# jdhuang-csm/hybrid-drt

Hardware: AMD Instinct MI355X
Metric: DRT fits/sec (256 freq x 512 tau, batched) (higher is better)
Workload: dtype f64

## Files before the change

### hybrid-drt_amd/_ffi.py

```python
from __future__ import annotations

import ctypes as C
import os
import sys
import threading

import numpy as np

_HERE = os.path.dirname(os.path.abspath(__file__))
LIB_PATH = os.environ.get("HIPDRT_LIB", os.path.join(_HERE, "libhipdrt.so"))

MODE_INTERP, MODE_TRAPZ = 0, 1
RESPONSE_POT, RESPONSE_EXPDECAY = 0, 1
QP_OPTIMAL, QP_MAXITER, QP_SINGULAR_LATE, QP_SINGULAR, QP_ABORTED = 0, 1, 2, -1, -2
PREDICT_NOT_PD = -3


class HipDrtError(RuntimeError):
    pass


class QpOpts(C.Structure):
    _fields_ = [("abstol", C.c_double), ("reltol", C.c_double), ("feastol", C.c_double), ("maxiters", C.c_int)]

# ... 148 lines not shown


SIGNATURES = {
    "hipdrt_create": [C.c_int, C.POINTER(_vp)],
    "hipdrt_destroy": [_vp],
    "hipdrt_last_error": [],
    "hipdrt_stream": [_vp],
    "hipdrt_synchronize": [_vp],
    "hipdrt_device_info": [_vp, C.c_char_p, C.c_int, _ip, C.POINTER(C.c_longlong)],
    "hipdrt_impedance_lookup": [_vp, C.c_double, C.c_int, C.c_int, _dp, _dp, _dp, _dp],
    "hipdrt_impedance_matrix": [_vp, C.c_int, C.c_int, _dp, C.c_int, _dp, C.c_int, C.c_int, C.c_int, C.c_double,
                                C.c_int, _dp, _dp, _dp, _dp, C.c_int, _dp, _dp],
    "hipdrt_impedance_matrix_dev": [_vp, C.c_int, C.c_int, _dp, C.c_int, _dp, C.c_int, C.c_int, C.c_int, C.c_double,
                                    C.c_int, _dp, _dp, _dp, _dp, C.c_int, _vp, _vp, C.c_int, C.POINTER(C.c_float)],
    "hipdrt_phasor_z_matrix": [_vp, _dp, C.c_int, _dp, C.c_int, C.c_double, _dp, _dp],
    "hipdrt_phasor_v_matrix": [_vp, _dp, C.c_int, _dp, C.c_int, C.c_double, _dp, _dp, C.c_int, _dp, _dp],
    "hipdrt_chrono_var_matrix": [_vp, _dp, C.c_int, _ip, C.c_int, C.c_double, C.c_int, _dp],
    "hipdrt_response_lookup": [_vp, C.c_double, C.c_int, C.c_int, _dp, _dp],
    "hipdrt_response_matrix": [_vp, _dp, C.c_int, _dp, C.c_int, _dp, _dp, C.c_int, C.c_int, C.c_double, C.c_int, _dp, _dp,
                               C.c_int, _dp, _dp],
    "hipdrt_plan_bytes_per_spectrum": [C.c_int, C.c_int, C.c_int, C.POINTER(C.c_longlong)],
    "hipdrt_response_matrix_variant": [_vp, _dp, C.c_int, _dp, C.c_int, _dp, _dp, _dp, C.c_int, C.c_int, C.c_double, C.c_int,
                                       _dp, _dp],
    "hipdrt_nonuniform_gaussian_filter1d": [_vp, _dp, C.c_int, _dp, _ip, C.c_int, _ip, _dp, C.c_int, _dp, _dp, C.c_longlong,
                                            _ip, _ip, _dp],
    "hipdrt_penalty_matrices": [_vp, _dp, C.c_int, C.c_double, C.c_int, _dp, _dp, _dp],
    "hipdrt_eis_var_matrix": [_vp, _dp, C.c_int, C.c_double, C.c_double, C.c_int, _dp],
    "hipdrt_qp_batch": [_vp, C.c_int, C.c_int, C.c_int, _dp, _dp, C.c_int, _dp, C.POINTER(QpOpts), _dp, _ip, _dp, _ip],
    "hipdrt_qp_profile": [_vp, C.POINTER(C.c_ulonglong), C.c_int, C.c_int],
    "hipdrt_debug_qp_occupancy": [_vp, C.c_int, C.c_int],
    "hipdrt_debug_qp_group": [_vp, C.c_int],
    "hipdrt_debug_exact_zero_shortcuts": [_vp, C.c_int],
    "hipdrt_debug_qp_waves": [_vp, C.c_int],
    "hipdrt_debug_stream_pool": [_vp, C.c_int, C.POINTER(C.c_void_p), _ip, _ip, _ip],
    "hipdrt_debug_gram_l2": [_vp, C.POINTER(DebugGramArgs)],
    "hipdrt_debug_pack_p": [_vp, C.c_int, C.c_int, _dp, C.c_int, _dp],
    "hipdrt_debug_hyper_step": [_vp, C.POINTER(DebugHyperArgs)],
    "hipdrt_debug_hyper_form": [_vp, C.c_int, C.c_int, C.c_int, C.c_int, C.c_int, _ip, C.POINTER(C.c_longlong)],
    "hipdrt_debug_kk_stats": [_vp, C.c_int, C.c_int, _dp, _dp, _dp, C.POINTER(KkOpts), _dp, _ip, _dp, _ip, _ip],
    "hipdrt_default_kk_opts": [C.POINTER(KkOpts)],
    "hipdrt_plan_kk_screen": [_vp, C.POINTER(KkOpts), C.c_int, _dp, _dp, _dp, _dp, _dp, _ip, _dp, _ip, _ip],
    "hipdrt_func_eval_matrix": [_vp, _dp, C.c_int, _dp, C.c_int, C.c_double, C.c_int, _dp],
    "hipdrt_plan_set_tau_basis": [_vp, _dp, C.c_int, C.c_double],
    "hipdrt_plan_predict_drt": [_vp, _dp, C.c_int, C.c_int, C.c_int, C.c_int, C.c_double, C.c_double, _dp, _dp, _dp, _ip],
    "hipdrt_plan_predict_z": [_vp, _dp, C.c_int, C.c_int, _dp, _dp, _ip],
    "hipdrt_plan_predict_resistances": [_vp, _dp, _dp, _dp, C.c_int],
    "hipdrt_plan_set_predict_desc": [_vp, C.POINTER(PredictDesc)],
    "hipdrt_plan_predict_response": [_vp, C.POINTER(ResponseArgs), _dp, _ip],
    "hipdrt_plan_predict_z_model": [_vp, C.POINTER(ZModelArgs), _dp, _dp, _ip],
    "hipdrt_plan_predict_dop": [_vp, _dp, C.c_int, _dp, C.c_double, _dp, C.c_double, C.c_int, _dp, _ip],
    "hipdrt_debug_response": [_vp, C.POINTER(DebugResponseArgs)],
    "hipdrt_peak_opts_default": [C.POINTER(PeakOpts)],
    "hipdrt_plan_find_peaks": [_vp, _dp, C.c_int, C.POINTER(PeakOpts), _dp, _ip, _ip, _dp, _dp, _dp, _ip, _ip, _ip, _dp, _dp, _dp,
                               _ip],
    "hipdrt_debug_find_peaks": [_vp, C.c_int, C.c_int, _dp, _dp, _dp, _dp, C.POINTER(PeakOpts), _ip, _ip, _dp, _dp, _dp, _ip, _ip,
                                _ip, _dp, _dp, _dp],
    "hipdrt_peak_resolve_opts_default": [C.POINTER(PeakResolveOpts)],
    "hipdrt_plan_resolve_peaks": [_vp, C.POINTER(PeakResolveIn), C.POINTER(PeakResolveOpts), C.POINTER(PeakResolveOut)],
    "hipdrt_plan_integrate_drt": [_vp, _dp, C.c_int, C.c_int, C.c_int, C.c_int, _dp, _ip, _ip, C.c_int, _dp, _ip],
    "hipdrt_debug_peak_resolve": [_vp, C.POINTER(DebugPeakResolveArgs)],
    "hipdrt_plan_score_candidates": [_vp, C.POINTER(CandidatesIn), C.POINTER(CandidatesOut)],
    "hipdrt_debug_candidate_llh": [_vp, C.c_int, C.c_int, C.c_int, C.c_int, _dp, C.c_int, _dp, _dp, _dp, _dp, _dp, _dp],
    "hipdrt_debug_candidate_form": [_vp, C.c_int],
    "hipdrt_plan_pfrt_bytes_per_spectrum": [C.c_int, C.c_int, C.POINTER(C.c_longlong)],
    "hipdrt_plan_pfrt_begin": [_vp, C.c_int],
    "hipdrt_plan_pfrt_record": [_vp],
# ... 431 lines not shown
        opts = opts if opts is not None else default_fit_opts()
        B, nf, ntau = z.shape[0], freq.size, tau.size
        n = ntau + int(opts.fit_ohmic) + int(opts.fit_inductance)
        out = {"x": np.empty((B, n)), "fit_x": np.empty((B, ntau)), "R_inf": np.empty(B), "inductance": np.empty(B),
               "weights": np.empty((B, 2 * nf)), "coefficient_scale": np.empty(B), "rho": np.empty((B, 3)),
               "q_vector": np.empty((B, n)), "outer_iters": np.empty(B, dtype=np.int32),
               "status": np.empty(B, dtype=np.int32)}
        _check(self._lib.hipdrt_fit_eis_batch(self._h, B, _p(freq), nf, _p(z_re), _p(z_im), _p(tau), ntau, float(epsilon),
                                              MODE_INTERP, int(bool(toeplitz_a)), int(bool(toeplitz_m)), wt_re.size,
                                              int(ny), _p(wt_re), _p(wt_im), _p(lre), _p(lim), C.byref(opts),
                                              _p(out["x"]), _p(out["fit_x"]), _p(out["R_inf"]), _p(out["inductance"]),
                                              _p(out["weights"]), _p(out["coefficient_scale"]), _p(out["rho"]),
                                              _p(out["q_vector"]), _pi(out["outer_iters"]), _pi(out["status"])))
        return out

    def device_alloc(self, nbytes):
        ptr = _vp()
        _check(self._lib.hipdrt_device_alloc(self._h, int(nbytes), C.byref(ptr)))
        return ptr.value

    def device_free(self, ptr):
        _check(self._lib.hipdrt_device_free(self._h, _vp(ptr)))

    def device_synchronize(self):
        _check(self._lib.hipdrt_device_synchronize(self._h))

    def debug_qp_group(self, members):
        _check(self._lib.hipdrt_debug_qp_group(self._h, int(members)))
        self._qp_group_override = int(members)

    def debug_qp_waves(self, waves):
        _check(self._lib.hipdrt_debug_qp_waves(self._h, int(waves)))

    def debug_stream_pool(self):
        size = C.c_int(0)
        _check(self._lib.hipdrt_debug_stream_pool(self._h, 0, None, None, None, C.byref(size)))
        n = size.value
        st, ho, ru = (C.c_void_p * n)(), (C.c_int * n)(), (C.c_int * n)()
        _check(self._lib.hipdrt_debug_stream_pool(self._h, n, st, ho, ru, C.byref(size)))
        return [st[i] for i in range(n)], [ho[i] for i in range(n)], [ru[i] for i in range(n)]

    def debug_exact_zero_shortcuts(self, on):
        _check(self._lib.hipdrt_debug_exact_zero_shortcuts(self._h, int(bool(on))))

    def debug_gram_l2(self, A, w, y=None, l1=None, l1_scalar=0.0, l2=None, mk=None, s=None, rho=None, dfac=(0.0, 0.0, 0.0),
                      ns=0, sym=False, toep=False, toep_maxd=-1, spec_zero=False, dop_start=0, dop_size=0, dop_rho=None,
                      dop_dfac=(0.0, 0.0, 0.0), active=None, n=None, P=None, Ppk=None, q=None):
        A, w = _f64(A), _f64(w)
        B, m = w.shape
        a = DebugGramArgs()
        a.B, a.m, a.lda = B, m, A.shape[-1]
        a.n = n = A.shape[-1] if n is None else int(n)
        a.a_batched = int(A.ndim == 3)
        if A.shape[-2] != m or (A.ndim == 3 and A.shape[0] != B):
            raise ValueError("A does not match w")
        keep = [A, w]

        def arr(v, shape, what):
            if v is None:
                return None
            v = _f64(v)
            if v.shape != tuple(shape):
                raise ValueError(f"{what}: shape {v.shape}, expected {tuple(shape)}")
            keep.append(v)
            return _p(v)

# ... 958 lines not shown
```

### hybrid-drt_amd/csrc/common.hpp

```cpp
#pragma once
#include <hip/hip_runtime.h>

#include <cstdio>
#include <string>
#include <vector>

#include "../../include/hipdrt.h"
#include "../../include/hipdrt_debug.h"

namespace hipdrt {

void set_error(const std::string& msg);

#define HIPDRT_CHECK(expr)                                                                     \
    do {                                                                                       \
        hipError_t _e = (expr);                                                                \
        if (_e != hipSuccess) {                                                                \
            hipdrt::set_error(std::string(#expr) + ": " + hipGetErrorString(_e) + " (" +       \
                              __FILE__ + ":" + std::to_string(__LINE__) + ")");                \
            return HIPDRT_E_HIP;                                                               \
        }                                                                                      \
    } while (0)

#define HIPDRT_REQUIRE(cond, msg)                                                              \
// ... 30 lines not shown
        if (!src.p) return;
        p = static_cast<char*>(src.p) + offset;
        bytes = n;
        own = false;
    }
    template <class T>
    T* as() const { return static_cast<T*>(p); }
    double* d() const { return static_cast<double*>(p); }
    int* i() const { return static_cast<int*>(p); }
};

inline int round_up(int v, int m) { return (v + m - 1) / m * m; }

inline int set_lds_limit(const void* f, size_t bytes, const char* what) {
    const hipError_t e = hipFuncSetAttribute(f, hipFuncAttributeMaxDynamicSharedMemorySize, (int)bytes);
    if (e != hipSuccess) { set_error(std::string("hipFuncSetAttribute(") + what + "): " + hipGetErrorString(e)); return HIPDRT_E_HIP; }
    return HIPDRT_OK;
}

}

struct hipdrt_ctx {
    int device = 0;
    hipStream_t stream = nullptr;
    int pool_idx = -1;
    int num_cu = 0;
    size_t hbm_bytes = 0;
    std::string arch;
    int plans = 0;
    bool released = false;
    int qp_force_group = -1;
    int zero_shortcuts = 1;
    int qp_waves = -1;
    int cand_form = -1;
    float predict_ms[2] = {0.f, 0.f};
};

namespace hipdrt {

void ensure_stream_pool(int device);

void launch_lookup(hipStream_t st, double eps, int ngrid, int ny, const double* wt_re, const double* wt_im,
                   double* z_re, double* z_im);
void launch_lookup_slopes(hipStream_t st, int ngrid, const double* xp, const double* fp, double* slopes);
void launch_impedance_matrix(hipStream_t st, int B, int freq_batched, const double* freq, int nf, const double* tau,
                             int ntau, int mode, int toeplitz, double eps, int ngrid, const double* lut6, int ny,
                             double* a_re, double* a_im, double* cr_scratch);
void launch_phasor_z(hipStream_t st, const double* freq, int nf, const double* nu, int nnu, double eps, double* zre,
                     double* zim);
void launch_phasor_v(hipStream_t st, const double* times, int nt, const double* nu, int nnu, double eps,
                     const double* step_times, const double* step_sizes, int nsteps, double* rm, double* layered);
void launch_chrono_vmm(hipStream_t st, const double* tt, int nt, const int* seg, int nseg, double eps, int uniform,
                       double* vmm);
void launch_response_lookup(hipStream_t st, double eps, int ngrid, int ny, const double* td, double* v);
void launch_response_matrix(hipStream_t st, const double* times, int nt, const double* tau, int ntau,
                            const double* step_times, const double* step_sizes, int nsteps, int mode, double eps,
                            int ngrid, const double* lut3, int ny, double* a, double* layered);
void launch_response_variant(hipStream_t st, const double* times, int nt, const double* tau, int ntau,
                             const double* step_times, const double* step_sizes, const double* tau_rise, int nsteps,
                             int variant, double eps, int ny, double* a, double* layered);
void launch_nonuniform_gauss(hipStream_t st, const double* y, int n, const double* sigma, const int* seg_of, const int* seg,
                             const double* nodes, int K, const double* node_delta, const double* weights, const int* woff,
                             const int* radius, double* out);
void launch_penalty(hipStream_t st, const double* ln_tau, int n, double eps, int toeplitz, double* m0, double* m1,
                    double* m2, int ld, int pad);
void launch_eis_vmm(hipStream_t st, const double* freq, int nf, double vmm_eps, double reim_cor, int uniform,
// ... 282 lines not shown
    int* status;
};
void launch_cand_compact(hipStream_t st, const CandPeakArgs& a);

struct QpArgs {
    int B, n;
    const double* P;
    long long p_stride;
    int ldp;
    const double* Ppk;
    long long ppk_stride;
    int nchp;
    const double* q;
    const double* h;
    long long h_stride;
    double* L;
    int ldl;
    long long l_stride;
    double* x;
    int* iters;
    double* pcost;
    int* status;
    const int* active;
    const int* order = nullptr;
    int* iters_accum;
    double* state;
    int state_ld;
    long long state_stride;
    hipdrt_qp_opts opts;
    int G = 0;
    int* gsync = nullptr;
    int redo_aborted = 0;
    int waves = 0;
};
int launch_qp(hipStream_t st, const QpArgs& a);
int qp_group_size(int B, int n, int force = -1);
size_t qp_gsync_ints();
int launch_dist_var(hipStream_t st, int B, int n, const double* Ppk, long long ppk_stride, const double* Bex, int nex,
                    double* L, long long l_stride, double* out, long long out_stride, int* status);
size_t dist_var_scratch_doubles(int n, int nex);
void launch_rows_outer(hipStream_t st, const double* Y, int nch, int ncol, int nex, int nrow, double scale, double* out, int ld);
void launch_pack_rows(hipStream_t st, int nrow, int ncol, int col_offset, const double* M, int ldm, int ntile_rows,
                      double* tiles, int nchp);
void launch_lpt_order(hipStream_t st, int B, const int* iters, const int* active, int* order);
size_t qp_scratch_ld(int n);
size_t qp_scratch_doubles(int n, int G = 0);
inline int qp_state_ld(int n) { return round_up(n, 32) + 32; }
inline size_t qp_state_doubles(int n) { return (size_t)17 * qp_state_ld(n); }
int qp_profile_read(unsigned long long* out, int n, int reset);
int hyper_profile_read(unsigned long long* out, int n, int reset);
int qp_occupancy(int threads, int n);

}
```

### hybrid-drt_amd/csrc/debug.hip

```cpp
#include <cmath>
#include <cstring>

#include "plan.hpp"

namespace {
struct Guarded {
    static constexpr size_t G = 128;
    static constexpr unsigned char MARK = 0xA5;
    DevBuf buf;
    void* host = nullptr;
    size_t bytes = 0;
    const char* name = "";
    std::vector<unsigned char> stage;
    int up(const char* what, void* h, size_t nbytes, hipStream_t st) {
        name = what; host = h; bytes = nbytes;
        stage.assign(nbytes + 2 * G, MARK);
        if (h) std::memcpy(stage.data() + G, h, nbytes);
        HIPDRT_CHECK(buf.alloc(stage.size()));
        HIPDRT_CHECK(hipMemcpyAsync(buf.p, stage.data(), stage.size(), hipMemcpyHostToDevice, st));
        return 0;
    }
    double* dd() const { return reinterpret_cast<double*>(static_cast<unsigned char*>(buf.p) + G); }
    int fetch(hipStream_t st) { HIPDRT_CHECK(hipMemcpyAsync(stage.data(), buf.p, stage.size(), hipMemcpyDeviceToHost, st)); return 0; }
    int check() {
// ... 9 lines not shown
struct GuardedOuts {
    static constexpr int MAX = 17;
    Guarded g[MAX];
    int n = 0;
    template <class T>
    int want(const char* name, T* host, size_t count, T*& field, hipStream_t st) {
        if (!host) return 0;
        HIPDRT_REQUIRE(n < MAX, "internal: more outputs than GuardedOuts holds");
        TRY(g[n].up(name, host, count * sizeof(T), st));
        field = reinterpret_cast<T*>(g[n++].dd());
        return 0;
    }
    int back(hipStream_t st) {
        for (int i = 0; i < n; ++i) TRY(g[i].fetch(st));
        HIPDRT_CHECK(hipStreamSynchronize(st));
        for (int i = 0; i < n; ++i) TRY(g[i].check());
        return 0;
    }
};
}

extern "C" {

int hipdrt_debug_qp_group(hipdrt_ctx* ctx, int members) try {
    HIPDRT_REQUIRE(ctx, "NULL pointer");
    ctx->qp_force_group = members;
    return HIPDRT_OK;
} HIPDRT_CATCH

int hipdrt_debug_qp_waves(hipdrt_ctx* ctx, int waves) try {
    HIPDRT_REQUIRE(ctx, "NULL pointer");
    HIPDRT_REQUIRE(waves == -1 || waves == 4 || waves == 8, "waves: 4, 8 or -1");
    ctx->qp_waves = waves;
    return HIPDRT_OK;
} HIPDRT_CATCH

int hipdrt_debug_exact_zero_shortcuts(hipdrt_ctx* ctx, int on) try {
    HIPDRT_REQUIRE(ctx, "NULL pointer");
    ctx->zero_shortcuts = on ? 1 : 0;
    return HIPDRT_OK;
} HIPDRT_CATCH

int hipdrt_debug_qp_occupancy(hipdrt_ctx* ctx, int threads, int n) try {
    if (!ctx || hipSetDevice(ctx->device) != hipSuccess) return -1;
    return qp_occupancy(threads, n);
} HIPDRT_CATCH

int hipdrt_qp_profile(hipdrt_ctx* ctx, unsigned long long* cycles, int n, int reset) try {
    HIPDRT_REQUIRE(ctx && cycles, "NULL pointer");
    TRY(enter(ctx));
    HIPDRT_CHECK(hipStreamSynchronize(ctx->stream));
    return qp_profile_read(cycles, n, reset) < 0 ? HIPDRT_E_HIP : HIPDRT_OK;
} HIPDRT_CATCH

int hipdrt_debug_gram_l2(hipdrt_ctx* ctx, const hipdrt_debug_gram_args* a) try {
    HIPDRT_REQUIRE(ctx && a && a->A && a->w, "NULL pointer");
    const int B = a->B, m = a->m, n = a->n;
    HIPDRT_REQUIRE(B >= 1 && B <= 4096 && m >= 1 && m <= 8192 && n >= 1 && n <= 4096, "1 <= B <= 4096, 1 <= m <= 8192, 1 <= n <= 4096");
    HIPDRT_REQUIRE(a->lda >= n, "lda >= n");
    HIPDRT_REQUIRE(a->P || a->Ppk, "at least one of P / Ppk");
    HIPDRT_REQUIRE(!a->P || a->ldp >= n, "ldp >= n");
    HIPDRT_REQUIRE(!a->y || a->q, "y without q");
    const bool hyper = a->s != nullptr;
    if (hyper) {
        HIPDRT_REQUIRE(a->mk[0] && a->mk[1] && a->mk[2], "hyper-parameter form: three penalty matrices");
        HIPDRT_REQUIRE(a->ldm >= n, "ldm >= n");
// ... 501 lines not shown
```

### hybrid-drt_amd/csrc/operators.hip

```cpp
#include <cmath>

#include "plan.hpp"

namespace hipdrt {
hipdrt_qp_opts default_qp_opts() { return hipdrt_qp_opts{1e-7, 1e-6, 1e-7, 100}; }

int func_eval_dev(hipStream_t st, const double* basis_dev, int nb, const double* ev_dev, int ne, double eps, int order, double fac,
                  double* out_dev, int ld) {
    const double c1 = -2.0 * std::pow(eps, 2.0), c2 = 4.0 * std::pow(eps, 4.0);
    launch_func_eval(st, basis_dev, nb, ev_dev, ne, eps, order, c1, c2, fac, out_dev, ld);
    LAUNCH_OK();
    return HIPDRT_OK;
}
}

extern "C" {

int hipdrt_impedance_lookup(hipdrt_ctx* ctx, double epsilon, int ngrid, int ny, const double* wt_re,
                            const double* wt_im, double* z_re, double* z_im) try {
    HIPDRT_REQUIRE(ctx && wt_re && wt_im && z_re && z_im, "NULL pointer");
    HIPDRT_REQUIRE(ngrid >= 2 && ny >= 2 && ny <= 6000, "ngrid >= 2, 2 <= ny <= 6000");
    hipStream_t st; TRY(enter(ctx, &st));
    DevBuf dwr, dwi, dzr, dzi;
    const size_t gb = (size_t)ngrid * sizeof(double);
// ... 271 lines not shown

int hipdrt_eis_var_matrix(hipdrt_ctx* ctx, const double* freq, int nf, double vmm_epsilon, double reim_cor,
                          int uniform, double* vmm) try {
    HIPDRT_REQUIRE(ctx && freq && vmm, "NULL pointer");
    HIPDRT_REQUIRE(nf >= 1, "nf >= 1");
    hipStream_t st; TRY(enter(ctx, &st));
    DevBuf df, dv;
    const size_t bytes = (size_t)4 * nf * nf * sizeof(double);
    TRY(upload(df, freq, (size_t)nf * sizeof(double), st));
    HIPDRT_CHECK(dv.alloc(bytes));
    launch_eis_vmm(st, df.d(), nf, vmm_epsilon, reim_cor, uniform, dv.d());
    LAUNCH_OK();
    HIPDRT_CHECK(hipMemcpyAsync(vmm, dv.p, bytes, hipMemcpyDeviceToHost, st));
    HIPDRT_CHECK(hipStreamSynchronize(st));
    return HIPDRT_OK;
} HIPDRT_CATCH

int hipdrt_qp_batch(hipdrt_ctx* ctx, int B, int n, int p_batched, const double* P, const double* q, int h_batched,
                    const double* h, const hipdrt_qp_opts* opts, double* x, int* iters, double* pcost, int* status) try {
    HIPDRT_REQUIRE(ctx && P && q && h && x && status, "NULL pointer");
    HIPDRT_REQUIRE(B >= 1 && n >= 1 && n <= 4096, "B >= 1, 1 <= n <= 4096");
    hipStream_t st; TRY(enter(ctx, &st));
    DevBuf dP, dq, dh, dL, dx, dit, dpc, dst, dstate, dPpk, dgs;
    const int ldl = (int)qp_scratch_ld(n);
    const int G = qp_group_size(B, n, ctx->qp_force_group);
    const int ldp = round_up(n, 2);
    const size_t nmat = (size_t)(p_batched ? B : 1);
    HIPDRT_CHECK(dP.alloc(nmat * n * ldp * sizeof(double)));
    if (ldp != n) HIPDRT_CHECK(hipMemsetAsync(dP.p, 0, dP.bytes, st));
    HIPDRT_CHECK(hipMemcpy2DAsync(dP.p, (size_t)ldp * sizeof(double), P, (size_t)n * sizeof(double),
                                  (size_t)n * sizeof(double), nmat * n, hipMemcpyHostToDevice, st));
    TRY(upload(dq, q, (size_t)B * n * sizeof(double), st));
    TRY(upload(dh, h, (size_t)(h_batched ? B : 1) * n * sizeof(double), st));
    HIPDRT_CHECK(dL.alloc((size_t)B * qp_scratch_doubles(n, G) * sizeof(double)));
    HIPDRT_CHECK(dx.alloc((size_t)B * n * sizeof(double)));
    HIPDRT_CHECK(dit.alloc((size_t)B * sizeof(int)));
    HIPDRT_CHECK(dpc.alloc((size_t)B * sizeof(double)));
    HIPDRT_CHECK(dst.alloc((size_t)B * sizeof(int)));
    QpArgs a{};
    a.B = B; a.n = n; a.P = dP.d(); a.p_stride = p_batched ? (long long)n * ldp : 0; a.ldp = ldp;
    a.q = dq.d(); a.h = dh.d(); a.h_stride = h_batched ? n : 0;
    a.L = dL.d(); a.ldl = ldl; a.l_stride = (long long)qp_scratch_doubles(n, G);
    a.x = dx.d(); a.iters = dit.i(); a.pcost = dpc.d(); a.status = dst.i();
    a.active = nullptr; a.iters_accum = nullptr;
    a.G = G;
    a.waves = ctx->qp_waves;
    if (G >= 1) {
        HIPDRT_CHECK(dgs.alloc((size_t)B * qp_gsync_ints() * sizeof(int)));
        a.gsync = dgs.i();
    }
    HIPDRT_CHECK(dPpk.alloc(nmat * qp_ppk_doubles(n) * sizeof(double)));
    launch_pack_p(st, (int)nmat, n, dP.d(), ldp, (long long)n * ldp, dPpk.d(), (long long)qp_ppk_doubles(n), qp_nchp(n));
    a.Ppk = dPpk.d(); a.ppk_stride = p_batched ? (long long)qp_ppk_doubles(n) : 0; a.nchp = qp_nchp(n);
    HIPDRT_CHECK(dstate.alloc((size_t)B * (G > 1 ? G : 1) * qp_state_doubles(n) * sizeof(double)));
    a.state = dstate.d(); a.state_ld = qp_state_ld(n); a.state_stride = (long long)qp_state_doubles(n);
    a.opts = opts ? *opts : default_qp_opts();
    TRY(launch_qp(st, a));
    HIPDRT_CHECK(hipMemcpyAsync(x, dx.p, (size_t)B * n * sizeof(double), hipMemcpyDeviceToHost, st));
    if (iters) HIPDRT_CHECK(hipMemcpyAsync(iters, dit.p, (size_t)B * sizeof(int), hipMemcpyDeviceToHost, st));
    if (pcost) HIPDRT_CHECK(hipMemcpyAsync(pcost, dpc.p, (size_t)B * sizeof(double), hipMemcpyDeviceToHost, st));
    HIPDRT_CHECK(hipMemcpyAsync(status, dst.p, (size_t)B * sizeof(int), hipMemcpyDeviceToHost, st));
    HIPDRT_CHECK(hipStreamSynchronize(st));
    return HIPDRT_OK;
} HIPDRT_CATCH

int hipdrt_weighted_gram(hipdrt_ctx* ctx, int B, int m, int n, const double* A, const double* w, const double* b,
                         int l2_batched, const double* l2, const double* l1, double* P, double* q) try {
    HIPDRT_REQUIRE(ctx && A && w && b && P && q, "NULL pointer");
    HIPDRT_REQUIRE(B >= 1 && m >= 1 && n >= 1, "B, m, n >= 1");
    hipStream_t st; TRY(enter(ctx, &st));
    DevBuf dA, dw, db, dl2, dl1, dP, dq;
    TRY(upload(dA, A, (size_t)m * n * sizeof(double), st));
    TRY(upload(dw, w, (size_t)B * m * sizeof(double), st));
    TRY(upload(db, b, (size_t)B * m * sizeof(double), st));
    if (l2) TRY(upload(dl2, l2, (size_t)(l2_batched ? B : 1) * n * n * sizeof(double), st));
    if (l1) TRY(upload(dl1, l1, (size_t)n * sizeof(double), st));
    HIPDRT_CHECK(dP.alloc((size_t)B * n * n * sizeof(double)));
    HIPDRT_CHECK(dq.alloc((size_t)B * n * sizeof(double)));
    launch_weighted_gram(st, B, m, n, dA.d(), n, dw.d(), db.d(), l2 ? dl2.d() : nullptr,
// ... 27 lines not shown
```

### hybrid-drt_amd/csrc/plan.hip

```cpp
#include <cmath>
#include <cstring>

#include "plan.hpp"

struct SpecDims { size_t n, m, nf; int qp_G; };
struct PerSpectrumBuf {
    DevBuf hipdrt_plan::*buf;
    size_t (*bytes)(const SpecDims&);
    bool lazy;
};
static const PerSpectrumBuf kPerSpectrum[] = {
    {&hipdrt_plan::z_re, [](const SpecDims& d) { return d.nf * sizeof(double); }},
    {&hipdrt_plan::z_im, [](const SpecDims& d) { return d.nf * sizeof(double); }},
    {&hipdrt_plan::rv, [](const SpecDims& d) { return d.m * sizeof(double); }},
    {&hipdrt_plan::w, [](const SpecDims& d) { return d.m * sizeof(double); }},
    {&hipdrt_plan::est_w, [](const SpecDims& d) { return d.m * sizeof(double); }},
    {&hipdrt_plan::x, [](const SpecDims& d) { return d.n * sizeof(double); }},
    {&hipdrt_plan::x_in, [](const SpecDims& d) { return d.n * sizeof(double); }},
    {&hipdrt_plan::q, [](const SpecDims& d) { return d.n * sizeof(double); }},
    {&hipdrt_plan::s, [](const SpecDims& d) { return 3 * d.n * sizeof(double); }},
    {&hipdrt_plan::rho, [](const SpecDims&) { return 3 * sizeof(double); }},
    {&hipdrt_plan::xmx, [](const SpecDims&) { return 3 * sizeof(double); }},
    {&hipdrt_plan::coef_scale, [](const SpecDims&) { return sizeof(double); }},
    {&hipdrt_plan::var_floor, [](const SpecDims&) { return sizeof(double); }},
    {&hipdrt_plan::pcost, [](const SpecDims&) { return sizeof(double); }},
    {&hipdrt_plan::active, [](const SpecDims&) { return sizeof(int); }},
    {&hipdrt_plan::outer_iters, [](const SpecDims&) { return sizeof(int); }},
    {&hipdrt_plan::fit_status, [](const SpecDims&) { return sizeof(int); }},
    {&hipdrt_plan::qp_iters_total, [](const SpecDims&) { return sizeof(int); }},
    {&hipdrt_plan::qp_status, [](const SpecDims&) { return sizeof(int); }},
    {&hipdrt_plan::qp_iters, [](const SpecDims&) { return sizeof(int); }},
    {&hipdrt_plan::L, [](const SpecDims& d) { return qp_scratch_doubles((int)d.n, d.qp_G) * sizeof(double); }},
    {&hipdrt_plan::qpstate, [](const SpecDims& d) { return (d.qp_G > 1 ? d.qp_G : 1) * qp_state_doubles((int)d.n) * sizeof(double); }},
    {&hipdrt_plan::gsync, [](const SpecDims&) { return qp_gsync_ints() * sizeof(int); }},
    {&hipdrt_plan::Ppk, [](const SpecDims& d) { return qp_ppk_doubles((int)d.n) * sizeof(double); }},
    {&hipdrt_plan::order, [](const SpecDims&) { return sizeof(int); }},
    {&hipdrt_plan::premv, [](const SpecDims& d) { return 3 * d.m * sizeof(double); }, true},
};

static SpecDims spec_dims(const hipdrt_plan* p) {
    return {(size_t)p->n, (size_t)p->m, (size_t)(p->nf > 0 ? p->nf : 1), p->qp_G};
}

namespace hipdrt {
int make_view(hipdrt_plan* p, hipdrt_subfit& sf, int idx, int b0, int nb) {
    hipdrt_plan& v = sf.view;
    sf.ctx = *p->ctx;
    sf.ctx.plans = 0; sf.ctx.released = false; sf.ctx.pool_idx = -1;
    v.ctx = &sf.ctx;
    static_cast<PlanShape&>(v) = *p;
    v.capacity = nb; v.B = nb; v.subbatches = 1;
    auto whole = [](DevBuf& d, const DevBuf& s_) { d.alias(s_, 0, s_.bytes); };
    whole(v.freq, p->freq); whole(v.tau, p->tau); whole(v.ln_tau, p->ln_tau); whole(v.wt_re, p->wt_re); whole(v.wt_im, p->wt_im);
    whole(v.lut6, p->lut6); whole(v.a_re, p->a_re); whole(v.a_im, p->a_im); whole(v.cr, p->cr); whole(v.rm, p->rm);
    for (int k = 0; k < 3; ++k) whole(v.mk[k], p->mk[k]);
    whole(v.vmm, p->vmm); whole(v.h, p->h); whole(v.l1, p->l1); whole(v.h_init, p->h_init); whole(v.vmm_base, p->vmm_base);
    whole(v.Ptmp, p->Ptmp);
    const SpecDims d = spec_dims(p);
    for (const PerSpectrumBuf& e : kPerSpectrum) {
        const size_t per = e.bytes(d);
        (v.*e.buf).alias(p->*e.buf, (size_t)b0 * per, (size_t)nb * per);
    }
    v.n_active.alias(p->n_active_sub, (size_t)idx * sizeof(int), sizeof(int));
    return HIPDRT_OK;
}

int plan_hist_reserve(hipdrt_plan* p, int rows) {
    if (rows < 1) rows = 1;
    if (p->hist_b >= 0 && p->hist_cap < rows) {
        p->hist_cap = rows;
        HIPDRT_CHECK(p->hist_x.alloc((size_t)p->hist_cap * p->n * sizeof(double)));
        HIPDRT_CHECK(p->hist_w.alloc((size_t)p->hist_cap * p->m * sizeof(double)));
        HIPDRT_CHECK(p->hist_rho.alloc((size_t)p->hist_cap * 3 * sizeof(double)));
        HIPDRT_CHECK(p->hist_qp.alloc((size_t)(p->hist_cap + 1) * sizeof(int)));
// ... 20 lines not shown
    o->eis_vmm_epsilon = 0.25; o->eis_reim_cor = 0.25;
    o->xtol = 1e-2; o->max_iter = 50; o->nonneg = 1; o->scale_data = 1; o->fit_ohmic = 1; o->fit_inductance = 1;
    o->update_scale = 0; o->eff_hp = 1;
    o->eis_error_uniform = 0;
    o->outlier_p = -1.0; o->iw_alpha = -1.0; o->iw_beta = -1.0;
    o->qp = default_qp_opts();
}

static int plan_build_matrices(hipdrt_plan* p, bool build_lookup) {
    hipStream_t st = p->ctx->stream;
    if (p->mode == HIPDRT_MODE_INTERP && build_lookup) {
        double* base = p->lut6.d();
        launch_lookup(st, p->eps, p->ngrid, p->ny, p->wt_re.d(), p->wt_im.d(), base + p->ngrid, base + 4 * (size_t)p->ngrid);
        LAUNCH_OK();
    }
    if (p->mode == HIPDRT_MODE_INTERP) {
        double* base = p->lut6.d();
        launch_lookup_slopes(st, p->ngrid, base, base + p->ngrid, base + 2 * (size_t)p->ngrid);
        launch_lookup_slopes(st, p->ngrid, base + 3 * (size_t)p->ngrid, base + 4 * (size_t)p->ngrid, base + 5 * (size_t)p->ngrid);
    }
    launch_impedance_matrix(st, 1, 0, p->freq.d(), p->nf, p->tau.d(), p->ntau, p->mode, p->toeplitz_a, p->eps, p->ngrid,
                            p->lut6.d(), p->ny, p->a_re.d(), p->a_im.d(), p->cr.d());
    LAUNCH_OK();
    FitState fs = p->state();
    launch_assemble_rm(st, fs, p->a_re.d(), p->a_im.d(), p->freq.d(), p->rm.d(), p->idx_rinf, p->idx_induc);
    LAUNCH_OK();
    return 0;
}

static int plan_alloc_batch(hipdrt_plan* p) {
    const size_t cap = (size_t)p->capacity;
    const int n = p->n, m = p->m;
    p->qp_G = qp_group_size(p->capacity, n, p->ctx->qp_force_group);
    HIPDRT_REQUIRE(p->qp_G >= 0, "n too large for the QP kernels");
    const SpecDims d = spec_dims(p);
    for (const PerSpectrumBuf& e : kPerSpectrum)
        if (!e.lazy) HIPDRT_CHECK((p->*e.buf).alloc(cap * e.bytes(d)));
    HIPDRT_CHECK(p->n_active.alloc(sizeof(int)));
    HIPDRT_CHECK(p->Ptmp.alloc((size_t)n * p->ldp * sizeof(double)));
    if (p->opts.outlier_p > 0.0) {
        HIPDRT_CHECK(p->vmm_base.alloc((size_t)m * m * sizeof(double)));
        HIPDRT_CHECK(p->outlier_t.alloc(cap * m * sizeof(double)));
    }
    HIPDRT_CHECK(p->hist_rows.alloc(sizeof(int)));
    return 0;
}

static int plan_toep_reach(hipdrt_plan* p) {
    p->toep_maxd = -1;
    if (!p->toeplitz_m) return HIPDRT_OK;
    const int nd = p->n - p->ns;
    std::vector<double> row(nd);
    int reach = 0;
    for (int k = 0; k < 3; ++k) {
        HIPDRT_CHECK(hipMemcpy(row.data(), p->mk[k].d() + (size_t)p->ns * p->ldm + p->ns, (size_t)nd * sizeof(double), hipMemcpyDeviceToHost));
        for (int d = nd - 1; d > reach; --d)
            if (row[d] != 0.0) { reach = d; break; }
    }
    p->toep_maxd = reach;
    p->spec_zero = 1;
    if (p->ns > 0) {
        std::vector<double> cols((size_t)nd * p->ns), rows((size_t)p->ns * nd);
        for (int k = 0; k < 3 && p->spec_zero; ++k) {
            HIPDRT_CHECK(hipMemcpy2D(cols.data(), (size_t)p->ns * sizeof(double), p->mk[k].d() + (size_t)p->ns * p->ldm,
                                     (size_t)p->ldm * sizeof(double), (size_t)p->ns * sizeof(double), nd, hipMemcpyDeviceToHost));
            HIPDRT_CHECK(hipMemcpy2D(rows.data(), (size_t)nd * sizeof(double), p->mk[k].d() + p->ns, (size_t)p->ldm * sizeof(double),
// ... 369 lines not shown
```

### hybrid-drt_amd/csrc/plan.hpp

```cpp
#pragma once
#include <memory>
#include <mutex>
#include <new>
#include <stdexcept>

#include "common.hpp"
#include "pfrt_store.hpp"

using namespace hipdrt;

#define TRY(expr) do { int _rc = (expr); if (_rc) return _rc; } while (0)
#define LAUNCH_OK() HIPDRT_CHECK(hipGetLastError())

#define HIPDRT_CATCH                                                                                              \
    catch (const std::bad_alloc&) { hipdrt::set_error("out of host memory"); return HIPDRT_E_HIP; }                \
    catch (const std::exception& e) { hipdrt::set_error(std::string("internal error: ") + e.what()); return HIPDRT_E_HIP; } \
    catch (...) { hipdrt::set_error("internal error"); return HIPDRT_E_HIP; }

inline int enter(hipdrt_ctx* ctx, hipStream_t* st = nullptr) {
    HIPDRT_CHECK(hipSetDevice(ctx->device)); (void)hipGetLastError();
    if (st) *st = ctx->stream;
    return HIPDRT_OK;
}

// ... 34 lines not shown
    if (nf < 2) return 1;
    const int dir = f[0] > f[1] ? 1 : -1;
    for (int i = 0; i + 1 < nf; ++i)
        if (!(dir > 0 ? f[i] > f[i + 1] : f[i] < f[i + 1])) return 0;
    return dir;
}

namespace hipdrt {
void pool_borrow(int device, int k, int* idx, hipStream_t* st);
void pool_return(int device, int k, const int* idx);
int pool_size(int device);
struct LoopOnContextStream {
    hipdrt_ctx* c;
    explicit LoopOnContextStream(hipdrt_ctx* c_);
    ~LoopOnContextStream();
};
extern std::mutex g_life;
void free_ctx(hipdrt_ctx* ctx);

hipdrt_qp_opts default_qp_opts();
int func_eval_dev(hipStream_t st, const double* basis_dev, int nb, const double* ev_dev, int ne, double eps, int order,
                  double fac, double* out_dev, int ld);
}

struct PlanShape {
    int nf = 0, ntau = 0, n = 0, m = 0, ns = 0, ngrid = 0, ny = 0, mode = 0, toeplitz_a = 0, toeplitz_m = 0;
    int idx_rinf = -1, idx_induc = -1;
    int ldrm = 0, ldm = 0, ldp = 0, ldl = 0;
    double eps = 0;
    hipdrt_fit_opts opts{};
    int toep_maxd = -1;
    int spec_zero = 0;
    int qp_G = 0;
};

struct hipdrt_plan : PlanShape {
    hipdrt_ctx* ctx = nullptr;
    int freq_order = 0;
    int capacity = 0, B = 0;
    int prepared = 0;
    int prepped = 0;
    hipdrt_prepared_desc desc{};
    long long rm_stride = 0;
    DevBuf vz_strength, dop_rho, dop_xmx, hist_dop_rho, outlier_t, vz_entry;
    double weight_factor = 1.0;
    int wrow_batched = 0;
    int wrow_late = 0;
    DevBuf wrow, w_eff, h_init, wfac;
    bool has_weight_factors() const { return weight_factor != 1.0 || wrow.p != nullptr; }
    DevBuf freq, tau, ln_tau, wt_re, wt_im, lut6, a_re, a_im, cr, rm, mk[3], vmm, h, l1;
    DevBuf z_re, z_im, rv, w, est_w, x, x_in, q, s, rho, xmx, coef_scale, var_floor;
    DevBuf active, outer_iters, fit_status, qp_iters_total, qp_status, qp_iters, n_active, pcost;
    DevBuf premv;
    DevBuf L, Ptmp, qpstate, Ppk, order, vmm_base, gsync;
    DevBuf basis_ln_tau;
    int basis_nb = 0;
    double basis_eps = 0;
    int pd_set = 0, pd_idx_rinf = -1, pd_idx_induc = -1, pd_idx_cinv = -1;
    double pd_inductance_scale = 0, pd_capacitance_scale = 0;
    DevBuf pd_dop_scale, pd_vb_scale, pd_cs, pd_rss, pd_sro;
    void qp_layout(int B, QpArgs& qa) const {
        int G = qp_group_size(B, n, ctx ? ctx->qp_force_group : -1);
        const size_t have_l = L.bytes / sizeof(double), have_s = qpstate.bytes / sizeof(double);
        if (G >= 1 && G != qp_G) {
            const bool fits = gsync.p && (size_t)B * qp_scratch_doubles(n, G) <= have_l &&
                              (size_t)B * G * qp_state_doubles(n) <= have_s && (size_t)B * qp_gsync_ints() * sizeof(int) <= gsync.bytes;
            if (!fits) G = qp_G;
        } else if (G < 1) {
            G = qp_G;
        }
        qa.G = G; qa.gsync = gsync.i(); qa.l_stride = (long long)qp_scratch_doubles(n, G);
        qa.waves = ctx ? ctx->qp_waves : -1;
    }
    int hist_b = -1, hist_cap = 0;
    DevBuf hist_x, hist_w, hist_rho, hist_qp, hist_rows;
    int pf_max = 0, pf_steps = 0;
    DevBuf pf_x, pf_rho, pf_dop_rho, pf_s, pf_rss, pf_slw, pf_status;
    hipdrt::PfrtStoreLayout pf_layout() const { return {(size_t)capacity, (size_t)n}; }
    float t_ms[5] = {0, 0, 0, 0, 0};
    int launches[5] = {0, 0, 0, 0, 0};
    int subbatches = 0;
    std::vector<std::unique_ptr<struct hipdrt_subfit>> subs;
    DevBuf n_active_sub;
    hipdrt_plan() = default;
    ~hipdrt_plan();

    FitState state() const {
        FitState st{};
        st.nf = nf; st.m = m; st.n = n; st.ns = ns; st.ldrm = ldrm; st.ldm = ldm; st.toeplitz_m = toeplitz_m;
        st.toep_reach = (toeplitz_m && !(ctx && !ctx->zero_shortcuts)) ? toep_maxd : -1;
        st.opts = opts; st.continue_mode = 0; st.min_iter = 1;
        st.basis_area = prepared ? desc.basis_area : (eps > 0 ? 1.7724538509055159 / eps : 0.0);
        st.prepared = prepared; st.desc = desc; st.rm_stride = rm_stride; st.rm_rw = rm.d();
        st.vz_strength = vz_strength.d(); st.vz_entry = nullptr; st.dop_rho = dop_rho.d(); st.dop_xmx = dop_xmx.d();
        st.hist_dop_rho = hist_dop_rho.d(); st.outlier_t = outlier_t.d();
        st.rm = rm.d(); st.vmm = vmm.d(); st.vmm_iw = vmm_base.p ? vmm_base.d() : vmm.d();
        for (int k = 0; k < 3; ++k) st.mk[k] = mk[k].d();
        st.z_re = z_re.d(); st.z_im = z_im.d();
        st.rv = rv.d(); st.w = w.d(); st.est_w = est_w.d();
        st.x = x.d(); st.x_in = x_in.d(); st.s = s.d(); st.rho = rho.d(); st.xmx = xmx.d();
        st.coef_scale = coef_scale.d(); st.var_floor = var_floor.d();
        st.active = active.i(); st.outer_iters = outer_iters.i(); st.fit_status = fit_status.i();
        st.qp_iters_total = qp_iters_total.i(); st.qp_status = qp_status.i(); st.qp_iters = qp_iters.i();
        st.n_active = n_active.i();
// ... 55 lines not shown
```

### hybrid-drt_amd/csrc/qp.hip

```cpp
#include <atomic>
#include <mutex>
#include <cstdlib>
#include <cstdio>

#include "qp_common.hpp"
#include "qp_resident.hpp"
#include "qp_group.hpp"

namespace hipdrt {

size_t qp_scratch_ld(int n) { return (size_t)round_up(n, 16); }

size_t qp_scratch_doubles(int n, int G) {
    if (G >= 1) return group_scratch_doubles(n, G);
    return n <= RNP_MAX ? resident_l_doubles(n) : resident_gu_doubles(n);
}
size_t qp_gsync_ints() { return GRP_WORDS; }

int device_cus() {
    static const int cus = [] {
        int dev = 0, v = 0;
        if (hipGetDevice(&dev) != hipSuccess ||
            hipDeviceGetAttribute(&v, hipDeviceAttributeMultiprocessorCount, dev) != hipSuccess || v <= 0) v = 256;
        return v;
    }();
    return cus;
}

int qp_group_size(int B, int n, int force) {
    if (n > GRP_NMAX) return -1;
    if (force == 0 && n <= 2048) return 0;
    if (force >= 1) {
        int G = force;
        const int ntr = (n + 15) / 16, rounds = (B + 7) / 8;
        if (G > 32 / rounds) G = 32 / rounds;
        if (G > ntr / 2) G = ntr / 2;
        return G >= 1 ? G : 1;
    }
    const bool few = B * 16 <= device_cus();
    if (n <= 2048 && !(few && n > 256)) return 0;
    const int ntr = (n + 15) / 16, rounds = (B + 7) / 8;
    int G = ntr / 4;
    if (G > 32 / rounds) G = 32 / rounds;
    if (G > GRP_MAXG) G = GRP_MAXG;
    return G >= 2 ? G : 1;
}

#ifdef HIPDRT_GRP_TIMELINE
// ... 32 lines not shown
    for (int i = threadIdx.x; i < B; i += blockDim.x) keys[i] = (active && !active[i]) ? -1 : iters[i];
    __syncthreads();
    const int t = blockIdx.x * blockDim.x + threadIdx.x, b = t >> 4, part = t & 15;
    int rank = 0;
    if (b < B) {
        const int kb = keys[b];
        for (int j = part; j < B; j += 16) {
            const int kj = keys[j];
            rank += (kj > kb) || (kj == kb && j < b);
        }
    }
#pragma unroll
    for (int o = 8; o >= 1; o >>= 1) rank += __shfl_xor(rank, o, 16);
    if (b < B && part == 0) order[rank] = b;
}

void launch_lpt_order(hipStream_t st, int B, const int* iters, const int* active, int* order) {
    const int blocks = (B * 16 + 255) / 256;
    hipLaunchKernelGGL(lpt_order_kernel, dim3(blocks), dim3(256), (size_t)B * sizeof(int), st, B, iters, active, order);
}

template <typename K, typename... A>
static int launch_lds(K kernel, const char* what, dim3 grid, dim3 block, size_t lds, hipStream_t st, A... args) {
    if (int rc = set_lds_limit(reinterpret_cast<const void*>(kernel), lds, what)) return rc;
    hipLaunchKernelGGL(kernel, grid, block, lds, st, args...);
    const hipError_t e = hipGetLastError();
    if (e != hipSuccess) { set_error(std::string(what) + " launch: " + hipGetErrorString(e)); return HIPDRT_E_HIP; }
    return HIPDRT_OK;
}

static int launch_qp_resident(hipStream_t st, const QpArgs& a) {
    const int NP = round_up(a.n, 32);
    if (!a.Ppk) { set_error("qp resident: packed copy of P missing"); return HIPDRT_E_INVALID; }
    const bool gu = a.n > RNP_MAX;
    if (!gu && a.waves == 4)
        return launch_lds(qp_kernel_resident<false, 256, 1, 2>, "qp fat", dim3(a.B), dim3(256), qp_resident_lds_bytes<false, 256, 2>(NP),
                          st, a, NP);
    if (gu) return launch_lds(qp_kernel_resident<true>, "qp resident", dim3(a.B), dim3(RT), qp_resident_lds_bytes<true>(NP), st, a, NP);
    return launch_lds(qp_kernel_resident<false>, "qp resident", dim3(a.B), dim3(RT), qp_resident_lds_bytes<false>(NP), st, a, NP);
}

int launch_dist_var(hipStream_t st, int B, int n, const double* Ppk, long long ppk_stride, const double* Bex, int nex,
                    double* L, long long l_stride, double* out, long long out_stride, int* status) {
    if (n > GRP_NMAX) { set_error("posterior variance: n > 4096 not supported"); return HIPDRT_E_INVALID; }
    const int NP = round_up(n, 32);
    CovArgs a;
    a.B = B; a.n = n; a.Ppk = Ppk; a.ppk_stride = ppk_stride; a.nchp = qp_nchp(n); a.Bex = Bex; a.nex = nex;
    a.L = L; a.l_stride = l_stride; a.out = out; a.out_stride = out_stride; a.status = status;
    if (n > RNP_MAX) return launch_lds(cov_kernel_resident<true>, "cov", dim3(B), dim3(RT), cov_lds_bytes<true>(NP), st, a, NP);
    return launch_lds(cov_kernel_resident<false>, "cov", dim3(B), dim3(RT), cov_lds_bytes<false>(NP), st, a, NP);
}

size_t dist_var_scratch_doubles(int n, int nex) {
    const size_t nch = (size_t)round_up(n, 32) / 16;
    return (nch + (size_t)nex) * nch * TSZ + (n > RNP_MAX ? (size_t)round_up(n, 32) * PLD : 0);
}

int qp_occupancy(int threads, int n) {
    const int NP = round_up(n, 32);
    int nb = -1;
    hipError_t e;
    if (threads != 512) return -1;
    if (n > RNP_MAX) {
        e = hipOccupancyMaxActiveBlocksPerMultiprocessor(&nb, qp_kernel_resident<true, 512>, 512, qp_resident_lds_bytes<true>(NP));
    } else {
        (void)hipFuncSetAttribute(reinterpret_cast<const void*>(qp_kernel_resident<false, 512>), hipFuncAttributeMaxDynamicSharedMemorySize, (int)qp_resident_lds_bytes<false>(NP));
        e = hipOccupancyMaxActiveBlocksPerMultiprocessor(&nb, qp_kernel_resident<false, 512>, 512, qp_resident_lds_bytes<false>(NP));
    }
    return e == hipSuccess ? nb : -1;
}

static int launch_qp_group(hipStream_t st, const QpArgs& a, int G) {
    const int NP = round_up(a.n, 32);
    if (!a.Ppk || !a.gsync) { set_error("qp group: packed copy of P or sync words missing"); return HIPDRT_E_INVALID; }
    hipError_t e = hipMemsetAsync(a.gsync, 0, (size_t)a.B * GRP_WORDS * sizeof(int), st);
    if (e != hipSuccess) { set_error(std::string("qp group sync reset: ") + hipGetErrorString(e)); return HIPDRT_E_HIP; }
    const int blocks = 8 * G * ((a.B + 7) / 8);
    static std::mutex mtx;
    static hipEvent_t last[64] = {};
    int dev = 0;
    (void)hipGetDevice(&dev);
    std::lock_guard<std::mutex> lock(mtx);
    hipEvent_t& ev = last[dev & 63];
    if (G > 1) {
        if (ev) {
            e = hipStreamWaitEvent(st, ev, 0);
            if (e != hipSuccess) { set_error(std::string("qp group chain: ") + hipGetErrorString(e)); return HIPDRT_E_HIP; }
        } else {
            e = hipEventCreateWithFlags(&ev, hipEventDisableTiming);
            if (e != hipSuccess) { ev = nullptr; set_error(std::string("qp group event: ") + hipGetErrorString(e)); return HIPDRT_E_HIP; }
        }
    }
    if (int rc = launch_lds(qp_kernel_group, "qp group", dim3(blocks), dim3(512), group_lds_bytes(NP), st, a, NP, G)) return rc;
    if (G > 1) {
        e = hipEventRecord(ev, st);
        if (e != hipSuccess) { set_error(std::string("qp group record: ") + hipGetErrorString(e)); return HIPDRT_E_HIP; }
    }
    return HIPDRT_OK;
}

static std::atomic<bool> g_group_spread[64];

// ... 40 lines not shown
```

### hybrid-drt_amd/csrc/qp_common.hpp

```cpp
#pragma once
#include "common.hpp"

namespace hipdrt {

typedef double v4d __attribute__((ext_vector_type(4)));

#ifdef HIPDRT_QP_PROFILE
static constexpr int QP_PROF_SLOTS = 48;
__device__ unsigned long long g_qp_prof[QP_PROF_SLOTS];
static constexpr int QP_TL_J = 16, QP_TL_K = 8;
__device__ unsigned long long g_qp_tl[8 * QP_TL_J * QP_TL_K];
__device__ unsigned long long g_qp_tl_sum[8 * QP_TL_J * QP_TL_K + 1];
__device__ unsigned long long g_qp_tl_ref;
#define TL_START() do { if (blockIdx.x == 0) { g_qp_tl_ref = __builtin_amdgcn_s_memtime(); atomicAdd(&g_qp_tl_sum[8 * QP_TL_J * QP_TL_K], 1ull); } } while (0)
#define TL(w, J, k) do { if ((threadIdx.x & 63) == 0 && blockIdx.x == 0 && (J) < QP_TL_J) { \
    const unsigned long long _tn = __builtin_amdgcn_s_memtime(); \
    g_qp_tl[((w) * QP_TL_J + (J)) * QP_TL_K + (k)] = _tn; \
    atomicAdd(&g_qp_tl_sum[((w) * QP_TL_J + (J)) * QP_TL_K + (k)], _tn - g_qp_tl_ref); } } while (0)
#define PROF_DECL unsigned long long _pt = __builtin_amdgcn_s_memtime();
#define PROF(slot) do { if (threadIdx.x == 0 && blockIdx.x == 0) { unsigned long long _n = __builtin_amdgcn_s_memtime(); \
    atomicAdd(&g_qp_prof[slot], _n - _pt); _pt = _n; } else { _pt = 0; } } while (0)
#define PROF2(slot, slot2) do { if (threadIdx.x == 0 && blockIdx.x == 0) { unsigned long long _n = __builtin_amdgcn_s_memtime(); \
    atomicAdd(&g_qp_prof[slot], _n - _pt); atomicAdd(&g_qp_prof[slot2], _n - _pt); _pt = _n; } else { _pt = 0; } } while (0)
#define PROFW(slot) do { if ((threadIdx.x & 63) == 0 && blockIdx.x == 0) { unsigned long long _n = __builtin_amdgcn_s_memtime(); \
    atomicAdd(&g_qp_prof[slot], _n - _pt); _pt = _n; } else { _pt = 0; } } while (0)
#else
static constexpr int QP_PROF_SLOTS = 48;
#define PROF_DECL
#define PROF(slot)
#define PROF2(slot, slot2)
#define PROFW(slot)
#define TL(w, J, k)
#define TL_START()
#endif

static constexpr int NB = 32;
static constexpr int PLD = 33;

__device__ __forceinline__ unsigned opaque_u32(unsigned v) {
    asm volatile("" : "+v"(v));
    return v;
}

__device__ __forceinline__ void lds_barrier() {
    asm volatile("s_waitcnt lgkmcnt(0)\n\ts_barrier" ::: "memory");
}

static __device__ __forceinline__ int lds_peek32(const void* p) {
    int v;
    asm volatile("ds_read_b32 %0, %1\n\ts_waitcnt lgkmcnt(0)" : "=v"(v) : "v"((unsigned)(size_t)p) : "memory");
    return __builtin_amdgcn_readfirstlane(v);
}
static __device__ __forceinline__ int lds_peek8(const void* p) {
    int v;
    asm volatile("ds_read_u8 %0, %1\n\ts_waitcnt lgkmcnt(0)" : "=v"(v) : "v"((unsigned)(size_t)p) : "memory");
    return __builtin_amdgcn_readfirstlane(v);
}

typedef double v2d __attribute__((ext_vector_type(2)));

static __device__ __forceinline__ v2d gload16(const char* sbase, unsigned voff) {
    v2d d;
    asm volatile("global_load_dwordx4 %0, %1, %2" : "=v"(d) : "v"(voff), "s"(sbase) : "memory");
    return d;
}
template <int OFF>
static __device__ __forceinline__ v2d gload16v(const void* p) {
    v2d d;
    asm volatile("global_load_dwordx4 %0, %1, off offset:%2" : "=v"(d) : "v"(p), "n"(OFF) : "memory");
    return d;
// ... 54 lines not shown

__device__ __forceinline__ double uni(double v) {
    int lo = __double2loint(v), hi = __double2hiint(v);
    lo = __builtin_amdgcn_readfirstlane(lo);
    hi = __builtin_amdgcn_readfirstlane(hi);
    return __hiloint2double(hi, lo);
}

__device__ __forceinline__ double wsum(double v) {
    v += dpp_mov_d<0xB1>(v);
    v += dpp_mov_d<0x4E>(v);
    v += dpp_mov_d<0x124>(v);
    v += dpp_mov_d<0x128>(v);
    return (bcast_lane(v, 0) + bcast_lane(v, 16)) + (bcast_lane(v, 32) + bcast_lane(v, 48));
}
__device__ __forceinline__ double wmax(double v) {
    v = fmax(v, dpp_mov_d<0xB1>(v));
    v = fmax(v, dpp_mov_d<0x4E>(v));
    v = fmax(v, dpp_mov_d<0x124>(v));
    v = fmax(v, dpp_mov_d<0x128>(v));
    return fmax(fmax(bcast_lane(v, 0), bcast_lane(v, 16)), fmax(bcast_lane(v, 32), bcast_lane(v, 48)));
}

template <int NW, int SLOTS = 4, int VT = 1>
struct Reducer {
    static_assert(SLOTS == 2 || SLOTS == 4, "");
    static constexpr int NWV = NW * VT;
    double* buf;
    int slot;
    __device__ Reducer(double* b) : buf(b), slot(0) {}
    template <int N>
    __device__ __forceinline__ void sum(double (&v)[VT][N]) {
        static_assert(N <= 4, "");
        double* s = buf + (slot & (SLOTS - 1)) * NWV * 4;
        ++slot;
#pragma unroll
        for (int t = 0; t < VT; ++t)
#pragma unroll
            for (int i = 0; i < N; ++i) v[t][i] = wsum(v[t][i]);
        if ((threadIdx.x & 63) == 0) {
#pragma unroll
            for (int t = 0; t < VT; ++t)
#pragma unroll
                for (int i = 0; i < N; ++i) s[((threadIdx.x >> 6) + NW * t) * 4 + i] = v[t][i];
        }
        __syncthreads();
#pragma unroll
        for (int i = 0; i < N; ++i) {
            double t = 0.0;
#pragma unroll
            for (int w = 0; w < NWV; ++w) t += s[w * 4 + i];
            v[0][i] = t;
        }
    }
    template <int N>
    __device__ __forceinline__ void max(double (&v)[VT][N]) {
        static_assert(N <= 4, "");
        double* s = buf + (slot & (SLOTS - 1)) * NWV * 4;
        ++slot;
#pragma unroll
        for (int t = 0; t < VT; ++t)
#pragma unroll
            for (int i = 0; i < N; ++i) v[t][i] = wmax(v[t][i]);
        if ((threadIdx.x & 63) == 0) {
#pragma unroll
            for (int t = 0; t < VT; ++t)
#pragma unroll
                for (int i = 0; i < N; ++i) s[((threadIdx.x >> 6) + NW * t) * 4 + i] = v[t][i];
        }
        __syncthreads();
#pragma unroll
        for (int i = 0; i < N; ++i) {
            double t = s[i];
#pragma unroll
            for (int w = 1; w < NWV; ++w) t = fmax(t, s[w * 4 + i]);
            v[0][i] = t;
        }
    }
};


struct IpmSmem {
    double* vec;
    double* dvec;
    double* red;
};

template <int THREADS, int EPT, class Ops, int VT = 1>
__device__ __forceinline__ void ipm_solve(const QpArgs& a, int b, Ops& ops, const IpmSmem& sm, int slot = -1,
                                          bool leader = true) {
    constexpr int NW = THREADS / 64;
    constexpr int EUNR = EPT <= 4 ? EPT : 2;
    const int n = a.n;
    const unsigned tid = threadIdx.x;
    const double* qg = a.q + (size_t)b * n;
    const double* hg = a.h + (size_t)b * a.h_stride;
    Reducer<NW, Ops::kRedSlots, VT> red(sm.red);
#ifdef HIPDRT_QP_MATVEC
    constexpr bool kRecurPx = false;
#else
    constexpr bool kRecurPx = true;
#endif
    constexpr double kDriftTol = 8.0;
    constexpr double kCancUlps = 64.0;
    double drift = 0.0, canc = 0.0;
    bool refresh = false;

    double* const S_ = a.state + (size_t)(slot >= 0 ? slot : b) * a.state_stride;
    const int sld = a.state_ld;
#define SV(k) (S_ + (size_t)(k) * sld)
    double* const x = SV(0); double* const z = SV(1); double* const s = SV(2); double* const d = SV(3);
    double* const di = SV(4); double* const lm = SV(5); double* const qv = SV(6); double* const hv = SV(7);
    double* const rx = SV(8); double* const rz = SV(9); double* const dx = SV(10); double* const ds = SV(11);
    double* const dz = SV(12); double* const ws3 = SV(13); double* const zz = SV(14); double* const sv = SV(15);
    double* const px = SV(16);
#define FOR_E _Pragma("unroll") for (unsigned v_ = 0; v_ < (unsigned)VT; ++v_) \
        _Pragma("unroll EUNR") for (unsigned e_ = 0, i = opaque_u32(tid) + v_ * THREADS; e_ < (unsigned)EPT; ++e_, i += THREADS * VT)
#define VALID (i < (unsigned)n)
    FOR_E if (VALID) { qv[i] = qg[i]; hv[i] = hg[i]; x[i] = z[i] = 0.0; s[i] = lm[i] = 1.0; d[i] = di[i] = 1.0; }

    double nq[VT][2] = {};
    FOR_E if (VALID) { nq[v_][0] += qv[i] * qv[i]; nq[v_][1] += hv[i] * hv[i]; }
    red.sum(nq);
    const double resx0 = uni(fmax(1.0, sqrt(nq[0][0])));
    const double resz0 = uni(fmax(1.0, sqrt(nq[0][1])));

    PROF_DECL
#ifdef HIPDRT_QP_PROFILE
    const unsigned long long _rt0 = __builtin_amdgcn_s_memrealtime();
#endif
    int status = HIPDRT_QP_MAXITER, iters = 0;
    double pcost = 0.0, gap = 0.0;

    bool start = true;
    for (;;) {
        if (!start) {
            const bool direct = !kRecurPx || refresh;
            if (direct) {
                __syncthreads();
                FOR_E if (VALID) sm.vec[i] = x[i];
                __syncthreads();
                { PROF_DECL
                ops.matvec();
                __syncthreads();
                PROF(9); }
                if (kRecurPx) {
                    FOR_E if (VALID) px[i] = sm.dvec[i];
                    refresh = false;
                    canc = 0.0;
                }
            }
            double t4[VT][4] = {}, zr[VT][1] = {};
            FOR_E {
                if (VALID) {
                    const double px_ = kRecurPx ? px[i] : sm.dvec[i], q_ = qv[i], x_ = x[i], z_ = z[i], s_ = s[i], h_ = hv[i];
                    double r = px_ + q_;
                    t4[v_][0] += x_ * r;
                    t4[v_][1] += x_ * q_;
                    r -= z_;
                    t4[v_][2] += r * r;
                    const double rzz = s_ - h_ - x_;
                    t4[v_][3] += rzz * rzz;
                    zr[v_][0] += z_ * rzz;
                    rx[i] = r;
                    rz[i] = rzz;
                }
            }
            red.sum(t4);
            red.sum(zr);
            const double f0 = 0.5 * (t4[0][0] + t4[0][1]);
            const double resx = sqrt(t4[0][2]), resz = sqrt(t4[0][3]);
            pcost = uni(f0);
            const double dcost = f0 + zr[0][0] - gap;
            bool has_rel = false;
            double relgap = 0.0;
            if (pcost < 0.0) { relgap = gap / -pcost; has_rel = true; }
            else if (dcost > 0.0) { relgap = gap / dcost; has_rel = true; }
// ... 7 lines not shown
            }
            if (conv) { status = HIPDRT_QP_OPTIMAL; break; }
            if (iters == a.opts.maxiters) { status = HIPDRT_QP_MAXITER; break; }
            if (iters == 0) {
                FOR_E if (VALID) { const double s_ = s[i], z_ = z[i], d_ = sqrt(s_ / z_); d[i] = d_; di[i] = 1.0 / d_; lm[i] = sqrt(s_ * z_); }
            }
        }
        const double mu = uni(gap / (double)n);
        double sigma = 0.0, step = 1.0;
        const int nsolve = start ? 1 : 2;
        auto set_rhs = [&](int pc) {
            FOR_E {
                if (VALID) {
                    if (start) {
                        sm.vec[i] = -qv[i] - hv[i];
                    } else {
                        const double lm_ = lm[i], rz_ = rz[i], d_ = d[i], di_ = di[i], rx_ = rx[i];
                        double t = (pc == 1) ? (-ws3[i] - lm_ * lm_) : (-(lm_ * lm_));
                        t += sigma * mu;
                        const double sv_ = t / lm_;
                        const double bz = -rz_ - d_ * sv_;
                        const double zz_ = bz * di_;
                        sv[i] = sv_;
                        zz[i] = zz_;
                        sm.vec[i] = -rx_ - di_ * zz_;
                    }
                }
            }
        };
        __syncthreads();
        FOR_E if (VALID) sm.dvec[i] = di[i] * di[i];
        set_rhs(0);
        __syncthreads();
        if (!ops.factor()) {
            status = (start || iters == 0) ? HIPDRT_QP_SINGULAR : HIPDRT_QP_SINGULAR_LATE;
            break;
        }

#pragma nounroll
        for (int pc = 0; pc < nsolve; ++pc) {
            if (pc == 0) {
                ops.backward();
            } else {
                set_rhs(pc);
                __syncthreads();
                ops.solve();
            }
            if (start) {
                double st[VT][2] = {}, mx[VT][2];
                for (int t_ = 0; t_ < VT; ++t_) mx[t_][0] = mx[t_][1] = -INFINITY;
                FOR_E {
                    if (VALID) {
                        const double x_ = sm.vec[i], q_ = qv[i], h_ = hv[i];
                        const double z_ = -x_ - h_, s_ = -z_;
                        st[v_][0] += s_ * s_; st[v_][1] += z_ * z_;
                        mx[v_][0] = fmax(mx[v_][0], -s_); mx[v_][1] = fmax(mx[v_][1], -z_);
                        x[i] = x_;
                        if (kRecurPx) px[i] = (-q_ - h_) - x_;
                        z[i] = z_;
                        s[i] = s_;
                    }
                }
                red.sum(st);
                red.max(mx);
                if (kRecurPx) {
                    double mm[VT][2] = {};
                    FOR_E if (VALID) { const double ax = fabs(x[i]); mm[v_][0] = fmax(mm[v_][0], ax); mm[v_][1] = fmax(mm[v_][1], fabs(qv[i] + hv[i]) + ax); }
                    red.max(mm);
                    drift = uni(mm[0][0]);
                    canc = uni(mm[0][1]);
                }
                const double nrms = sqrt(st[0][0]), nrmz = sqrt(st[0][1]);
                if (mx[0][0] >= -1e-8 * fmax(nrms, 1.0)) {
                    FOR_E if (VALID) s[i] += 1.0 + mx[0][0];
                }
                if (mx[0][1] >= -1e-8 * fmax(nrmz, 1.0)) {
                    FOR_E if (VALID) z[i] += 1.0 + mx[0][1];
                }
                double gp[VT][1] = {};
// ... 62 lines not shown
                s[i] = lmn * dn;
                z[i] = lmn * din;
            }
        }
        red.sum(g2);
        gap = uni(g2[0][0]);
        if (kRecurPx) {
            red.max(mm);
            drift = uni(drift + mm[0][0]);
            canc = uni(canc + mm[0][2]);
            if (drift > kDriftTol * mm[0][1]) { refresh = true; drift = uni(mm[0][1]); }
        }
        ++iters;
    }

    PROF(10);
#ifdef HIPDRT_QP_PROFILE
    if (threadIdx.x == 0 && blockIdx.x == 0) atomicAdd(&g_qp_prof[13], __builtin_amdgcn_s_memrealtime() - _rt0);
#endif
    if (leader) {
        FOR_E if (VALID) a.x[(size_t)b * n + i] = x[i];
    }
    if (tid == 0 && leader) {
#ifdef HIPDRT_QP_PROFILE
        if (blockIdx.x == 0) atomicAdd(&g_qp_prof[11], (unsigned long long)(iters + 1));
#endif
        if (a.iters) a.iters[b] = iters;
        if (a.pcost) a.pcost[b] = pcost;
        a.status[b] = status;
        if (a.iters_accum) a.iters_accum[b] += iters;
    }
#undef FOR_E
#undef VALID
#undef SV
}

}
```

### hybrid-drt_amd/csrc/qp_group.hpp

```cpp
#pragma once
#include "qp_resident.hpp"

namespace hipdrt {

#ifdef HIPDRT_GRP_TIMELINE
__device__ unsigned long long g_grp_tl[32 * 8 * 10 + 32];
#define TS_DECL unsigned long long ts_[10] = {0, 0, 0, 0, 0, 0, 0, 0, 0, 0}; const bool ts_on_ = (fidx == 3 && jb == HIPDRT_GRP_TIMELINE);
#define TS(e) do { if (ts_on_) ts_[e] = __builtin_amdgcn_s_memtime(); } while (0)
#define TS_PRINT() do { if (ts_on_ && (threadIdx.x & 63) == 0 && g < 32) { const int w_ = threadIdx.x >> 6; for (int e_ = 0; e_ < 10; ++e_) g_grp_tl[(g * 8 + w_) * 10 + e_] = ts_[e_]; if (w_ == 1) g_grp_tl[2560 + g] = la_owner(jb); } } while (0)
#else
#define TS_DECL
#define TS(e)
#define TS_PRINT()
#endif

static constexpr int GRP_NMAX = 4096;
static constexpr int GRP_OWN = 512;
static constexpr int GRP_MAXG = 32;
#ifndef HIPDRT_GRP_LA_RING
#define HIPDRT_GRP_LA_RING 4
#endif
#ifndef HIPDRT_GRP_ROW_RING
#define HIPDRT_GRP_ROW_RING 4
#endif
// ... 340 lines not shown
            const v4d d22 = init_tile(1, 1, ntr, fo, li, kq);
            stage_dsc(d11);
            img21[lane] = d21;
            img21[64 + lane] = d22;
        }
        __syncthreads();
        bool ok;
        if (wv == 0) ok = factor_chain();
        else if (wv == 1) ok = factor_lookahead();
        else ok = factor_rows(wv);
        if (ok) group_sync();
        return ok;
    }

    __device__ __forceinline__ bool factor_chain() {
        const int lane = fresh_lane(), li = lane & 15, kq = lane >> 4;
        const int fo = li * 4 + kq;
        const int nblk = (n + NB - 1) / NB;
        double* U = sm.U;
        v4d* const img21 = reinterpret_cast<v4d*>(sm.img);
        v4d* const img22 = img21 + 64;
        for (int jb = 0; jb < nblk; ++jb) {
            const int j0 = jb * NB;
            PROF_DECL
            TS_DECL
            TS(0);
            for (int spins = 0; lds_peek32(&sm.flag[1]) < jb;) {
                __builtin_amdgcn_s_sleep(1);
                trap_if(++spins > kSpinLimit);
            }
            asm volatile("" ::: "memory");
            PROF(2);
            TS(1);
            bool ok = cholinv16_dsc(j0, 0);
            TS(2);
            const v4d d21 = img21[lane];
            v4d d22 = img22[lane];
            v4d x21 = (v4d){0, 0, 0, 0};
#pragma unroll
            for (int s_ = 0; s_ < 4; ++s_)
                x21 = __builtin_amdgcn_mfma_f64_16x16x4f64(-U[(size_t)(j0 + li) * PLD + 4 * s_ + kq], d21[s_], x21, 0, 0, 0);
#pragma unroll
            for (int rg = 0; rg < 4; ++rg) sm.t21[li * DLD + kq + 4 * rg] = x21[rg];
            {
                double2* d0 = const_cast<double2*>(tile2(2 * jb + 1, 2 * jb)) + fo;
                d0[0] = make_double2(x21[0], x21[1]);
                d0[64] = make_double2(x21[2], x21[3]);
            }
            __builtin_amdgcn_wave_barrier();
#pragma unroll
            for (int s_ = 0; s_ < 4; ++s_)
                d22 = __builtin_amdgcn_mfma_f64_16x16x4f64(sm.t21[li * DLD + 4 * s_ + kq], x21[s_], d22, 0, 0, 0);
            ok = cholinv16(d22, j0 + 16, 16) && ok;
            PROF(12);
            TS(5);
            if (lane == 0) sm.flag[0] = ok ? 0 : 1;
            __syncthreads();
            PROF(1);
            TS(6);
            if (sm.flag[0]) return false;
            v4d y = (v4d){0, 0, 0, 0};
#pragma unroll
            for (int s_ = 0; s_ < 4; ++s_)
                y = __builtin_amdgcn_mfma_f64_16x16x4f64(sm.t21[li * DLD + 4 * s_ + kq],
                                                         U[(size_t)(j0 + 4 * s_ + kq) * PLD + li], y, 0, 0, 0);
            v4d w21 = (v4d){0, 0, 0, 0};
#pragma unroll
            for (int s_ = 0; s_ < 4; ++s_)
                w21 = __builtin_amdgcn_mfma_f64_16x16x4f64(-U[(size_t)(j0 + 16 + li) * PLD + 16 + 4 * s_ + kq], y[s_], w21, 0, 0, 0);
#pragma unroll
            for (int rg = 0; rg < 4; ++rg) U[(size_t)(j0 + 16 + kq + 4 * rg) * PLD + li] = w21[rg];
            __builtin_amdgcn_wave_barrier();
            const int r = lane & 31;
            const double* Mr = U + (size_t)(j0 + r) * PLD;
            double s0 = 0.0, s1 = 0.0, s2 = 0.0, s3 = 0.0;
#pragma unroll
            for (int c = 0; c < NB; c += 4) {
                s0 += Mr[c] * sm.vec[j0 + c];
                s1 += Mr[c + 1] * sm.vec[j0 + c + 1];
                s2 += Mr[c + 2] * sm.vec[j0 + c + 2];
                s3 += Mr[c + 3] * sm.vec[j0 + c + 3];
            }
            const double yv = (s0 + s1) + (s2 + s3);
            __builtin_amdgcn_wave_barrier();
            if (lane < NB) sm.vec[j0 + lane] = yv;
            TS(8);
            lds_barrier();
            PROF(3);
            TS(7);
            TS_PRINT();
        }
        return true;
    }

    __device__ __forceinline__ bool factor_lookahead() {
        const int lane = fresh_lane(), li = lane & 15, kq = lane >> 4;
        const int fo = li * 4 + kq;
        const int nblk = (n + NB - 1) / NB;
        const int ntr = (n + 15) >> 4;
        double* U = sm.U;
        v4d* const img21 = reinterpret_cast<v4d*>(sm.img);
        v4d* const img22 = img21 + 64;
        int laown = 0;
        for (int jb = 0; jb < nblk; ++jb) {
            const int j0 = jb * NB;
            const int tb = j0 >> 4;
            const int R2 = tb + 2, R3 = tb + 3;
// ... 74 lines not shown
                        v2d t_[14];
#pragma unroll
                        for (int q = 0; q < 7; ++q) {
                            t_[2 * q] = gload16_sc1(src + q * 2048, vo);
                            t_[2 * q + 1] = gload16_sc1(src + q * 2048 + 16, vo);
                        }
                        vm_wait<0>();
#pragma unroll
                        for (int q = 0; q < 14; ++q) asm volatile("" : "+v"(t_[q]));
                        auto cat = [&](int q) { return (v4d){t_[2 * q].x, t_[2 * q].y, t_[2 * q + 1].x, t_[2 * q + 1].y}; };
                        p20 = cat(0); p21 = cat(1); p30 = cat(2); p31 = cat(3); e11 = cat(4); e21 = cat(5); e22 = cat(6);
                        if (lane < 32) {
                            unsigned long long* rp_ = reinterpret_cast<unsigned long long*>(labuf + (size_t)jb * GRP_LA_SLOT + 7 * 256 + lane);
                            const unsigned long long bits = __hip_atomic_load(rp_, __ATOMIC_RELAXED, __HIP_MEMORY_SCOPE_AGENT);
                            sm.vec[R2 * 16 + lane] = __longlong_as_double((long long)bits);
                        }
                        TS(4);
                    }
                    if (!v3) {
                        p30 = (v4d){0, 0, 0, 0}; p31 = (v4d){0, 0, 0, 0}; e21 = (v4d){0, 0, 0, 0};
                        e22 = init_tile(R3, R3, ntr, fo, li, kq);
                    }
                }
            }
            TS(5);
            __syncthreads();
            PROFW(23);
            TS(6);
            if (sm.flag[0]) return false;
            if (v2) {
                double wn1[4], l21[4], wn2[4];
#pragma unroll
                for (int s_ = 0; s_ < 4; ++s_) {
                    wn1[s_] = -U[(size_t)(j0 + li) * PLD + 4 * s_ + kq];
                    l21[s_] = sm.t21[li * DLD + 4 * s_ + kq];
                    wn2[s_] = -U[(size_t)(j0 + 16 + li) * PLD + 16 + 4 * s_ + kq];
                }
                v4d x20 = (v4d){0, 0, 0, 0}, x30 = x20, x21_ = x20, x31 = x20;
#pragma unroll
                for (int s_ = 0; s_ < 4; ++s_) {
                    x20 = __builtin_amdgcn_mfma_f64_16x16x4f64(wn1[s_], p20[s_], x20, 0, 0, 0);
                    x30 = __builtin_amdgcn_mfma_f64_16x16x4f64(wn1[s_], p30[s_], x30, 0, 0, 0);
                }
#pragma unroll
                for (int s_ = 0; s_ < 4; ++s_) {
                    p21 = __builtin_amdgcn_mfma_f64_16x16x4f64(l21[s_], x20[s_], p21, 0, 0, 0);
                    p31 = __builtin_amdgcn_mfma_f64_16x16x4f64(l21[s_], x30[s_], p31, 0, 0, 0);
                }
#pragma unroll
                for (int s_ = 0; s_ < 4; ++s_) {
                    x21_ = __builtin_amdgcn_mfma_f64_16x16x4f64(wn2[s_], p21[s_], x21_, 0, 0, 0);
                    x31 = __builtin_amdgcn_mfma_f64_16x16x4f64(wn2[s_], p31[s_], x31, 0, 0, 0);
                }
                {
                    double2* d0 = const_cast<double2*>(tile2(R2, 2 * jb)) + fo;
                    d0[0] = make_double2(x20[0], x20[1]);   d0[64] = make_double2(x20[2], x20[3]);
                    d0[128] = make_double2(x21_[0], x21_[1]); d0[192] = make_double2(x21_[2], x21_[3]);
                }
                if (v3) {
                    double2* d0 = const_cast<double2*>(tile2(R3, 2 * jb)) + fo;
                    d0[0] = make_double2(x30[0], x30[1]);   d0[64] = make_double2(x30[2], x30[3]);
                    d0[128] = make_double2(x31[0], x31[1]); d0[192] = make_double2(x31[2], x31[3]);
                }
#pragma unroll
                for (int s_ = 0; s_ < 4; ++s_) {
                    e11 = __builtin_amdgcn_mfma_f64_16x16x4f64(x20[s_], x20[s_], e11, 0, 0, 0);
                    e21 = __builtin_amdgcn_mfma_f64_16x16x4f64(x20[s_], x30[s_], e21, 0, 0, 0);
                    e22 = __builtin_amdgcn_mfma_f64_16x16x4f64(x30[s_], x30[s_], e22, 0, 0, 0);
                }
// ... 61 lines not shown
#pragma unroll 1
            for (int ps = 0; ps < npass; ++ps) {
                int T[GRP_RMAXT];
                bool act[GRP_RMAXT];
#pragma unroll
                for (int u = 0; u < GRP_RMAXT; ++u) {
                    const int t_ = pop_row(mask, tb);
                    T[u] = t_ >= 0 ? t_ : nch;
                    act[u] = t_ >= 0;
                }
                v4d acc[GRP_RMAXT][2];
#pragma unroll
                for (int u = 0; u < GRP_RMAXT; ++u)
#pragma unroll
                    for (int ct = 0; ct < 2; ++ct)
                        acc[u][ct] = act[u] ? init_tile(T[u], tb + ct, ntr, fo, li, kq) : (v4d){0, 0, 0, 0};
                TS(9);
                if (jb > 0 && act[0]) {
                    if (act[GRP_RMAXT - 1]) ring_rows<GRP_RMAXT>(jb, ntr, lane, T, act, acc);
                    else ring_rows<1>(jb, ntr, lane, T, act, acc);
                }
                if (ps == 0) {
                    if (wv == 2) PROFW(28);
                    TS(5);
                    __syncthreads();
                    if (wv == 2) PROFW(29);
                    TS(6);
                    if (sm.flag[0]) return false;
                }
                if (act[0]) {
                    double wn1[4], l21[4], wn2[4];
#pragma unroll
                    for (int s_ = 0; s_ < 4; ++s_) {
                        wn1[s_] = -U[(size_t)(j0 + li) * PLD + 4 * s_ + kq];
                        wn2[s_] = -U[(size_t)(j0 + 16 + li) * PLD + 16 + 4 * s_ + kq];
                    }
                    if (ps == 0) {
#pragma unroll
                        for (int s_ = 0; s_ < 4; ++s_) l21[s_] = sm.t21[li * DLD + 4 * s_ + kq];
                    } else {
                        const double2* t_ = tile2(tb + 1, 2 * jb) + fo;
                        const double2 h0 = t_[0], h1 = t_[64];
                        l21[0] = h0.x; l21[1] = h0.y; l21[2] = h1.x; l21[3] = h1.y;
                    }
                    v4d x1[GRP_RMAXT], x2[GRP_RMAXT];
#pragma unroll
                    for (int u = 0; u < GRP_RMAXT; ++u) { x1[u] = (v4d){0, 0, 0, 0}; x2[u] = (v4d){0, 0, 0, 0}; }
#pragma unroll
                    for (int s_ = 0; s_ < 4; ++s_)
#pragma unroll
                        for (int u = 0; u < GRP_RMAXT; ++u)
                            x1[u] = __builtin_amdgcn_mfma_f64_16x16x4f64(wn1[s_], acc[u][0][s_], x1[u], 0, 0, 0);
#pragma unroll
                    for (int s_ = 0; s_ < 4; ++s_)
#pragma unroll
                        for (int u = 0; u < GRP_RMAXT; ++u)
                            acc[u][1] = __builtin_amdgcn_mfma_f64_16x16x4f64(l21[s_], x1[u][s_], acc[u][1], 0, 0, 0);
#pragma unroll
                    for (int s_ = 0; s_ < 4; ++s_)
#pragma unroll
                        for (int u = 0; u < GRP_RMAXT; ++u)
                            x2[u] = __builtin_amdgcn_mfma_f64_16x16x4f64(wn2[s_], acc[u][1][s_], x2[u], 0, 0, 0);
#pragma unroll
                    for (int u = 0; u < GRP_RMAXT; ++u) {
                        if (act[u]) {
                            double2* d0 = const_cast<double2*>(tile2(T[u], 2 * jb)) + fo;
                            d0[0] = make_double2(x1[u][0], x1[u][1]);
                            d0[64] = make_double2(x1[u][2], x1[u][3]);
                            d0[128] = make_double2(x2[u][0], x2[u][1]);
                            d0[192] = make_double2(x2[u][2], x2[u][3]);
                        }
                    }
                    if (ps == 0) lds_barrier();
#pragma unroll
                    for (int u = 0; u < GRP_RMAXT; ++u)
                        if (act[u] && T[u] < nch) fwd_update(x1[u], x2[u], T[u], j0, li, kq);
                } else if (ps == 0) {
                    lds_barrier();
                }
            }
            if (wv == 2) PROFW(30);
            TS(7);
            TS_PRINT();
        }
        return true;
    }
};

static constexpr int GRP_FIXED = 4 * 8 * 4 + 2 * 16 * 17 + 8 + 512 + 2 * GRP_OWN / 8 + 7 * 256 + 8;
static size_t group_lds_bytes(int NP) { return (size_t)(GRP_FIXED + 2 * (NP + 64)) * sizeof(double); }

static size_t group_scratch_doubles(int n, int G) {
    const size_t NP = (size_t)round_up(n, 32);
    return NP * NP + (size_t)G * NP * PLD + (NP / NB) * (size_t)GRP_LA_SLOT;
}

__global__ __launch_bounds__(512, 2) void qp_kernel_group(QpArgs a, int NP, int G) {
    constexpr int RT = 512;
    const int s_ = blockIdx.x & 7, rg = blockIdx.x >> 3;
    const int b = 8 * (rg / G) + s_, g = rg % G;
    if (b >= a.B) return;
    if (a.active && !a.active[b]) return;
    if (a.redo_aborted && a.status[b] != HIPDRT_QP_ABORTED) return;
    extern __shared__ double smem[];
    OpsGroup ops;
    ops.G = G; ops.g = g;
    ops.gs = a.gsync + (size_t)b * GRP_WORDS;
    ops.abort_status = a.status + b;
    ops.L = a.L + (size_t)b * a.l_stride; ops.nch = NP / 16; ops.n = a.n;
    ops.Ppk = a.Ppk + (size_t)b * a.ppk_stride; ops.nchp = a.nchp;
    ops.sm.red = smem;
    ops.sm.t21 = ops.sm.red + 4 * 8 * 4;
    ops.sm.dsc = ops.sm.t21 + 16 * 17;
    ops.sm.flag = reinterpret_cast<int*>(ops.sm.dsc + 16 * 17);
    ops.sm.img = ops.sm.dsc + 16 * 17 + 8;
    ops.owner = reinterpret_cast<unsigned char*>(ops.sm.img + 512);
    ops.rowdone = ops.owner + GRP_OWN;
    ops.latile = ops.sm.img + 512 + 2 * GRP_OWN / 8;
    ops.lacnt = reinterpret_cast<int*>(ops.latile + 7 * 256);
    ops.sm.vec = ops.latile + 7 * 256 + 8;
    ops.sm.dvec = ops.sm.vec + NP + 64;
    ops.sm.U = ops.L + (size_t)NP * NP + (size_t)g * NP * PLD;
    ops.labuf = ops.L + (size_t)NP * NP + (size_t)G * NP * PLD;
    ops.build_owner();
    for (int i = threadIdx.x; i < NP * PLD; i += RT) ops.sm.U[i] = 0.0;
    for (int i = threadIdx.x; i < NP + 64; i += RT) { ops.sm.vec[i] = 0.0; ops.sm.dvec[i] = 0.0; }
    if (G > 1) {
        int& xcc_mask = ops.sm.flag[2];
        if (threadIdx.x == 0) {
            const unsigned xcc = __builtin_amdgcn_s_getreg(20 | (0 << 6) | ((4 - 1) << 11)) & 15u;
            __hip_atomic_fetch_or(&ops.gs[1], 1 << xcc, __ATOMIC_RELAXED, __HIP_MEMORY_SCOPE_AGENT);
            int seen = __hip_atomic_fetch_add(&ops.gs[0], 1, __ATOMIC_ACQ_REL, __HIP_MEMORY_SCOPE_AGENT) + 1;
            int spins = 0;
            while (!(seen & kNotResident) && seen < G) {
                __builtin_amdgcn_s_sleep(2);
                if (++spins > OpsGroup::kRendezvousLimit) {
                    int expected = seen;
                    if (__hip_atomic_compare_exchange_strong(&ops.gs[0], &expected, seen | kNotResident, __ATOMIC_RELAXED,
                                                             __ATOMIC_RELAXED, __HIP_MEMORY_SCOPE_AGENT)) {
                        seen |= kNotResident;
                        break;
                    }
                    seen = expected;
                    continue;
                }
                seen = __hip_atomic_load(&ops.gs[0], __ATOMIC_ACQUIRE, __HIP_MEMORY_SCOPE_AGENT);
            }
            xcc_mask = (seen & kNotResident) ? kNotResident
                                             : __hip_atomic_load(&ops.gs[1], __ATOMIC_RELAXED, __HIP_MEMORY_SCOPE_AGENT);
        }
        __syncthreads();
        if (__builtin_popcount(xcc_mask) != 1 || (xcc_mask & kNotResident)) {
            if (g == 0 && threadIdx.x == 0) {
                a.status[b] = HIPDRT_QP_ABORTED;
                ops.gs[4] = (xcc_mask & kNotResident) ? 2 : 1;
            }
            return;
        }
// ... 8 lines not shown
```

### hybrid-drt_amd/csrc/qp_resident.hpp

```cpp
#pragma once
#include "qp_common.hpp"


namespace hipdrt {

static constexpr int RT = 512;
static constexpr int RNW = RT / 64;
static constexpr int RMAXT = 4;
static constexpr int kSweepCap = 5;
static constexpr int kLa1Load = 14;
static constexpr int kLa2Load = 22;
static constexpr int RNP_MAX = 528;
static constexpr int TSZ = 256;
static constexpr int DLD = 17;

template <bool GU, int RTT = 512, bool P64 = false, int VT = 1>
struct ResSmemT {
    double* U;
    double* vec;
    double* dvec;
    double* red;
    double* t21;
    double* dsc;
    double* img;
    int* flag;
    unsigned char* sched;

    static constexpr int VEC = GU ? (P64 ? 2048 + 32 + 32 : 4096 + 32 + 32) : 528 + 16 + 32;
    static constexpr int DVEC = P64 ? VEC - 32 : VEC;
    static constexpr int SROW = GU ? 128 : 32;
    static constexpr int SCHED = GU ? 64 * 128 / 8 : (P64 ? 9 * 32 / 8 : 17 * 32 / 8 + 4);
    static constexpr int RED = (P64 ? 2 : 4) * (RTT / 64) * VT * 4;
    static constexpr int T21 = P64 ? 2 * 256 : 16 * 17;
    static constexpr int FIXED = RED + T21 + 16 * 17 + 8 + 512 + SCHED + VEC + DVEC;
    __device__ __forceinline__ void carve(double* smem) {
        red = smem;
        t21 = red + RED;
        dsc = t21 + T21;
        flag = reinterpret_cast<int*>(dsc + 16 * 17);
        img = dsc + 16 * 17 + 8;
        sched = reinterpret_cast<unsigned char*>(img + 512);
        vec = img + 512 + SCHED;
        dvec = vec + VEC;
        U = dvec + DVEC;
    }
};
static_assert((ResSmemT<false, 512, true>::FIXED + 544 * 33) * 8 <= 160 * 1024, "n = 514 must fit one CU's LDS");
static_assert((ResSmemT<false, 256, true, 2>::FIXED + 544 * 33) * 8 <= 160 * 1024, "n = 514 must fit one CU's LDS (fat form)");
static_assert((ResSmemT<false, 512, true>::RED + ResSmemT<false, 512, true>::T21 + 16 * 17 + 8) % 4 == 0, "img must be 32-byte aligned");

template <bool GU, int RTT = 512, bool P64 = false, int VT = 1>
struct OpsResidentT {
    static constexpr int RT = RTT, RNW = RTT / 64;
    static_assert(!P64 || RTT == 512 || RTT == 256, "factor64 is written for eight wavefronts, or four fat ones");
    using Smem = ResSmemT<GU, RTT, P64, VT>;
    static constexpr int kVT = VT;
    static constexpr int kRedSlots = P64 ? 2 : 4;
    double* L; int nch; int n; Smem sm;
    const double* Ppk; int nchp;
    int nex = 0; const double* Bex = nullptr;

    __device__ __forceinline__ const double2* tile2(int t, int c) const {
        return reinterpret_cast<const double2*>(L) + (size_t)((t * nch + c) * (TSZ / 2));
    }

    static __device__ __forceinline__ int fresh_lane() {
        int l;
        asm volatile("v_mbcnt_lo_u32_b32 %0, -1, 0\n\tv_mbcnt_hi_u32_b32 %0, -1, %0" : "=v"(l));
        return l;
    }

    __device__ __forceinline__ void stage_dsc(const v4d& at) const {
        const int lane = fresh_lane(), li = lane & 15, kq = lane >> 4;
#pragma unroll
        for (int rg = 0; rg < 4; ++rg) sm.dsc[li * DLD + kq + 4 * rg] = -at[rg];
    }
    __device__ __forceinline__ bool cholinv16(const v4d& at, int r0, int c0) const {
        stage_dsc(at);
        __builtin_amdgcn_wave_barrier();
        return cholinv16_dsc(r0, c0);
    }
    __device__ __forceinline__ bool cholinv16_dsc(int r0, int c0) const { return cholinv16_blocked(r0, c0); }
    static __device__ __forceinline__ double rsq_pivot(double x) {
        const double y0 = __builtin_amdgcn_rsq(x);
        const double e = __builtin_fma(y0 * -x, y0, 1.0);
        return __builtin_fma(y0 * e, __builtin_fma(e, 0.375, 0.5), y0);
    }
    __device__ __forceinline__ bool cholinv16_blocked(int r0, int c0) const {
        const int lane = fresh_lane(), li = lane & 15, kq = lane >> 4;
        const double* D = sm.dsc;
        v4d aA, aW;
#pragma unroll
        for (int rg = 0; rg < 4; ++rg) {
            const int i = kq + 4 * rg;
            aA[rg] = D[(i > li ? i : li) * DLD + (i > li ? li : i)];
            aW[rg] = (i == li) ? 1.0 : 0.0;
        }
        double pmin = 1.0, plast = 0.0;
#pragma unroll
        for (int k = 0; k < 4; ++k) {
            const double tA = aA[k], tW = aW[k];
            auto dg = [&](int a_, int b_) { return bcast_lane(tA, 4 * k + b_ + 16 * a_); };
            const double d00 = dg(0, 0), d10 = dg(1, 0), d20 = dg(2, 0), d30 = dg(3, 0);
            const double d11 = dg(1, 1), d21 = dg(2, 1), d31 = dg(3, 1), d22 = dg(2, 2), d32 = dg(3, 2), d33 = dg(3, 3);
            const double i0 = rsq_pivot(d00);
            const double l10 = d10 * i0, l20 = d20 * i0, l30 = d30 * i0;
            const double p1 = d11 - l10 * l10;
            const double i1 = rsq_pivot(p1);
            const double l21 = (d21 - l20 * l10) * i1, l31 = (d31 - l30 * l10) * i1;
            const double p2 = d22 - l20 * l20 - l21 * l21;
            const double i2 = rsq_pivot(p2);
            const double l32 = (d32 - l30 * l20 - l31 * l21) * i2;
            const double p3 = d33 - l30 * l30 - l31 * l31 - l32 * l32;
            const double i3 = rsq_pivot(p3);
            pmin = fmin(fmin(pmin, fmin(d00, p1)), fmin(p2, p3));
            plast = p3;
            const double w10 = -(l10 * i0) * i1;
            const double w21 = -(l21 * i1) * i2, w20 = -(l20 * i0 + l21 * w10) * i2;
            const double w32 = -(l32 * i2) * i3, w31 = -(l31 * i1 + l32 * w21) * i3, w30 = -(l30 * i0 + l31 * w10 + l32 * w20) * i3;
            const double c0_ = li == 0 ? i0 : li == 1 ? w10 : li == 2 ? w20 : w30;
            const double c1_ = li == 1 ? i1 : li == 2 ? w21 : w31;
            const double c2_ = li == 2 ? i2 : w32;
            double wsel = kq == 0 ? c0_ : kq == 1 ? c1_ : kq == 2 ? c2_ : i3;
            wsel = (li < 4 && kq <= li) ? wsel : 0.0;
            const v4d z4 = (v4d){0, 0, 0, 0};
            const v4d X = __builtin_amdgcn_mfma_f64_16x16x4f64(wsel, tA, z4, 0, 0, 0);
            const v4d Y = __builtin_amdgcn_mfma_f64_16x16x4f64(wsel, tW, z4, 0, 0, 0);
            sm.U[(size_t)(r0 + 4 * k + kq) * PLD + c0 + li] = (li <= 4 * k + kq) ? Y[0] : 0.0;
            if (k < 3) {
                const double pan = (li > 4 * k + 3) ? -X[0] : 0.0;
                aA = __builtin_amdgcn_mfma_f64_16x16x4f64(pan, X[0], aA, 0, 0, 0);
                aW = __builtin_amdgcn_mfma_f64_16x16x4f64(pan, Y[0], aW, 0, 0, 0);
            }
        }
        __builtin_amdgcn_wave_barrier();
        return pmin > 0.0 && plast == plast;
    }

    struct TileSrc { double2 d0, d1; };
    __device__ __forceinline__ TileSrc tile_src(int T, int Cc, int ntr, int fo) const {
        TileSrc r_;
        r_.d0 = make_double2(0.0, 0.0); r_.d1 = r_.d0;
        if (T >= nch) {
            const double2* tile = reinterpret_cast<const double2*>(Bex + ((size_t)(T - nch) * nchp + Cc) * 256);
            r_.d0 = tile[fo]; r_.d1 = tile[64 + fo];
        } else if (T < ntr) {
            const double2* tile = reinterpret_cast<const double2*>(Ppk + ((size_t)T * nchp + Cc) * 256);
            r_.d0 = tile[fo]; r_.d1 = tile[64 + fo];
        }
        return r_;
    }
    __device__ __forceinline__ v4d tile_image(const TileSrc& r_, int T, int Cc, int li, int kq) const {
        v4d a_ = (v4d){-r_.d0.x, -r_.d0.y, -r_.d1.x, -r_.d1.y};
        if (T == Cc) {
            const int row = T * 16 + li;
            const double dg = row < n ? sm.dvec[row] : 1.0;
#pragma unroll
            for (int rg = 0; rg < 4; ++rg)
                if (kq + 4 * rg == li) a_[rg] -= dg;
        }
        return a_;
// ... 24 lines not shown
            default: vm_wait<28>(); break;
        }
    }

    __device__ __forceinline__ bool factor() {
        if constexpr (P64) return factor64();
        const int tid = opaque_u32(threadIdx.x), lane = tid & 63, wv = __builtin_amdgcn_readfirstlane(tid >> 6);
        const int ntr = (n + 15) >> 4;
        if (wv == 1) {
            const int li = lane & 15, kq = lane >> 4, fo = li * 4 + kq;
            v4d* const img21 = reinterpret_cast<v4d*>(sm.img);
            const v4d d11 = init_tile(0, 0, ntr, fo, li, kq);
            const v4d d21 = init_tile(1, 0, ntr, fo, li, kq);
            const v4d d22 = init_tile(1, 1, ntr, fo, li, kq);
            stage_dsc(d11);
            img21[lane] = d21;
            img21[64 + lane] = d22;
        }
        __syncthreads();
        if (wv == 0) return factor_chain();
        if (wv == 1) return factor_lookahead();
        return factor_rows(wv);
    }

    __device__ __forceinline__ bool factor_chain() {
        const int lane = fresh_lane(), li = lane & 15, kq = lane >> 4;
        const int nblk = (n + NB - 1) / NB;
        double* U = sm.U;
        v4d* const img21 = reinterpret_cast<v4d*>(sm.img);
        v4d* const img22 = img21 + 64;
        for (int jb = 0; jb < nblk; ++jb) {
            const int j0 = jb * NB;
            PROF_DECL
            bool ok = cholinv16_dsc(j0, 0);
            PROF(12);
            const v4d d21 = img21[lane];
            v4d d22 = img22[lane];
            v4d x21 = (v4d){0, 0, 0, 0};
#pragma unroll
            for (int s_ = 0; s_ < 4; ++s_)
                x21 = __builtin_amdgcn_mfma_f64_16x16x4f64(-U[(size_t)(j0 + li) * PLD + 4 * s_ + kq], d21[s_], x21, 0, 0, 0);
#pragma unroll
            for (int rg = 0; rg < 4; ++rg) sm.t21[li * DLD + kq + 4 * rg] = x21[rg];
            __builtin_amdgcn_wave_barrier();
#pragma unroll
            for (int s_ = 0; s_ < 4; ++s_)
                d22 = __builtin_amdgcn_mfma_f64_16x16x4f64(sm.t21[li * DLD + 4 * s_ + kq], x21[s_], d22, 0, 0, 0);
            PROF(14);
            ok = cholinv16(d22, j0 + 16, 16) && ok;
            PROF(15);
            if (lane == 0) sm.flag[0] = ok ? 0 : 1;
            __syncthreads();
            PROF2(1, 16 + (jb < 31 ? jb : 31));
            if (sm.flag[0]) return false;
            v4d y = (v4d){0, 0, 0, 0};
#pragma unroll
            for (int s_ = 0; s_ < 4; ++s_)
                y = __builtin_amdgcn_mfma_f64_16x16x4f64(sm.t21[li * DLD + 4 * s_ + kq],
                                                         U[(size_t)(j0 + 4 * s_ + kq) * PLD + li], y, 0, 0, 0);
            v4d w21 = (v4d){0, 0, 0, 0};
#pragma unroll
            for (int s_ = 0; s_ < 4; ++s_)
                w21 = __builtin_amdgcn_mfma_f64_16x16x4f64(-U[(size_t)(j0 + 16 + li) * PLD + 16 + 4 * s_ + kq], y[s_], w21, 0, 0, 0);
#pragma unroll
            for (int rg = 0; rg < 4; ++rg) U[(size_t)(j0 + 16 + kq + 4 * rg) * PLD + li] = w21[rg];
            PROF(3);
            __syncthreads();
            PROF(4);
        }
        return true;
    }

    __device__ __forceinline__ bool factor_lookahead() {
        const int lane = fresh_lane(), li = lane & 15, kq = lane >> 4;
        const int fo = li * 4 + kq;
        const int nblk = (n + NB - 1) / NB;
        const int ntr = (n + 15) >> 4;
        double* U = sm.U;
        v4d* const img21 = reinterpret_cast<v4d*>(sm.img);
        v4d* const img22 = img21 + 64;
        TileSrc pre[7];
        bool have_pre = false;
        for (int jb = 0; jb < nblk; ++jb) {
            const int j0 = jb * NB;
            const int tb = j0 >> 4;
            const int nc = 2 * jb;
            const int R2 = tb + 2, R3 = tb + 3;
            const bool v2 = R2 < ntr, v3 = R3 < ntr;
            v4d p20, p21, p30, p31, e11, e21, e22;
            if (v2) {
                if (have_pre) {
                    p20 = tile_image(pre[0], R2, tb, li, kq);      p21 = tile_image(pre[1], R2, tb + 1, li, kq);
                    p30 = tile_image(pre[2], R3, tb, li, kq);      p31 = tile_image(pre[3], R3, tb + 1, li, kq);
                    e11 = tile_image(pre[4], R2, R2, li, kq);      e21 = tile_image(pre[5], R3, R2, li, kq);
                    e22 = tile_image(pre[6], R3, R3, li, kq);
                } else {
                    p20 = init_tile(R2, tb, ntr, fo, li, kq);      p21 = init_tile(R2, tb + 1, ntr, fo, li, kq);
                    p30 = init_tile(R3, tb, ntr, fo, li, kq);      p31 = init_tile(R3, tb + 1, ntr, fo, li, kq);
// ... 23 lines not shown
                        e21 = __builtin_amdgcn_mfma_f64_16x16x4f64(A2, A3, e21, 0, 0, 0);           \
                        e22 = __builtin_amdgcn_mfma_f64_16x16x4f64(A3, A3, e22, 0, 0, 0);           \
                    }
                    auto multf = [&](const Frag& f_) {
                        HIPDRT_STEP7(f_.b0.x, f_.b1.x, f_.a2.x, f_.a3.x)
                        HIPDRT_STEP7(f_.b0.y, f_.b1.y, f_.a2.y, f_.a3.y)
                        __builtin_amdgcn_sched_barrier(0);
                    };
#undef HIPDRT_STEP7
                    asm volatile("s_waitcnt vmcnt(0)" ::: "memory");
                    __builtin_amdgcn_sched_barrier(0);
                    Frag f0, f1, f2, f3;
                    loadf(f0, 0); loadf(f1, 1); loadf(f2, 2);
                    for (int k2 = 0; k2 < nk2; k2 += 4) {
                        loadf(f3, k2 + 3); vm_wait<12>(); multf(f0);
                        loadf(f0, k2 + 4); vm_wait<12>(); multf(f1);
                        loadf(f1, k2 + 5); vm_wait<12>(); multf(f2);
                        loadf(f2, k2 + 6); vm_wait<12>(); multf(f3);
                    }
                    vm_wait<0>();
                    if (!v3) {
                        p30 = (v4d){0, 0, 0, 0}; p31 = (v4d){0, 0, 0, 0}; e21 = (v4d){0, 0, 0, 0};
                        e22 = init_tile(R3, R3, ntr, fo, li, kq);
                    }
                }
            }
            __syncthreads();
            if (sm.flag[0]) return false;
            have_pre = false;
            if (v2) {
                double wn1[4], l21[4], wn2[4];
#pragma unroll
                for (int s_ = 0; s_ < 4; ++s_) {
                    wn1[s_] = -U[(size_t)(j0 + li) * PLD + 4 * s_ + kq];
                    l21[s_] = sm.t21[li * DLD + 4 * s_ + kq];
                    wn2[s_] = -U[(size_t)(j0 + 16 + li) * PLD + 16 + 4 * s_ + kq];
                }
                v4d x20 = (v4d){0, 0, 0, 0}, x30 = x20, x21_ = x20, x31 = x20;
#pragma unroll
                for (int s_ = 0; s_ < 4; ++s_) {
                    x20 = __builtin_amdgcn_mfma_f64_16x16x4f64(wn1[s_], p20[s_], x20, 0, 0, 0);
                    x30 = __builtin_amdgcn_mfma_f64_16x16x4f64(wn1[s_], p30[s_], x30, 0, 0, 0);
                }
#pragma unroll
                for (int s_ = 0; s_ < 4; ++s_) {
                    p21 = __builtin_amdgcn_mfma_f64_16x16x4f64(l21[s_], x20[s_], p21, 0, 0, 0);
                    p31 = __builtin_amdgcn_mfma_f64_16x16x4f64(l21[s_], x30[s_], p31, 0, 0, 0);
                }
#pragma unroll
                for (int s_ = 0; s_ < 4; ++s_) {
                    x21_ = __builtin_amdgcn_mfma_f64_16x16x4f64(wn2[s_], p21[s_], x21_, 0, 0, 0);
                    x31 = __builtin_amdgcn_mfma_f64_16x16x4f64(wn2[s_], p31[s_], x31, 0, 0, 0);
                }
                {
                    double2* d0 = const_cast<double2*>(tile2(R2, 2 * jb)) + fo;
                    d0[0] = make_double2(x20[0], x20[1]);   d0[64] = make_double2(x20[2], x20[3]);
                    d0[128] = make_double2(x21_[0], x21_[1]); d0[192] = make_double2(x21_[2], x21_[3]);
                }
                if (v3) {
                    double2* d0 = const_cast<double2*>(tile2(R3, 2 * jb)) + fo;
                    d0[0] = make_double2(x30[0], x30[1]);   d0[64] = make_double2(x30[2], x30[3]);
                    d0[128] = make_double2(x31[0], x31[1]); d0[192] = make_double2(x31[2], x31[3]);
                }
                if (R2 + 2 < ntr) {
                    const int N2 = R2 + 2, N3 = R3 + 2;
                    pre[0] = tile_src(N2, R2, ntr, fo); pre[1] = tile_src(N2, R3, ntr, fo);
                    pre[2] = tile_src(N3, R2, ntr, fo); pre[3] = tile_src(N3, R3, ntr, fo);
                    pre[4] = tile_src(N2, N2, ntr, fo); pre[5] = tile_src(N3, N2, ntr, fo);
                    pre[6] = tile_src(N3, N3, ntr, fo);
// ... 102 lines not shown
                            }
                        }
#pragma unroll
                        for (int u = 0; u < RMAXT; ++u) {
                            if (act[u]) {
                                acc[u][0] = __builtin_amdgcn_mfma_f64_16x16x4f64(b_.b0.y, a_.a[u].y, acc[u][0], 0, 0, 0);
                                if (two) acc[u][1] = __builtin_amdgcn_mfma_f64_16x16x4f64(b_.b1.y, a_.a[u].y, acc[u][1], 0, 0, 0);
                            }
                        }
                        __builtin_amdgcn_sched_barrier(0);
                    };
                    SlA a0, a1, a2, a3;
                    asm volatile("s_waitcnt vmcnt(0)" ::: "memory");
                    __builtin_amdgcn_sched_barrier(0);
                    SlB b0, b1;
                    loadB(b0, 0); loadA(a0, 0); loadA(a1, 1); loadA(a2, 2);
                    for (int k2 = 0; k2 < nk2; k2 += 4) {
                        loadB(b1, k2 + 1); loadA(a3, k2 + 3); vm_wait<2 * RMAXT + 2>(); mult(a0, b0);
                        loadB(b0, k2 + 2); loadA(a0, k2 + 4); vm_wait<2 * RMAXT + 2>(); mult(a1, b1);
                        loadB(b1, k2 + 3); loadA(a1, k2 + 5); vm_wait<2 * RMAXT + 2>(); mult(a2, b0);
                        loadB(b0, k2 + 4); loadA(a2, k2 + 6); vm_wait<2 * RMAXT + 2>(); mult(a3, b1);
                    }
                    vm_wait<0>();
                }
                if (ps == 0) {
                    __syncthreads();
                    if (sm.flag[0]) return false;
                    have_pre = false;
                }
                if (act[0]) {
                    double wn1[4], l21[4], wn2[4];
#pragma unroll
                    for (int s_ = 0; s_ < 4; ++s_) {
                        wn1[s_] = -U[(size_t)(j0 + li) * PLD + 4 * s_ + kq];
                        l21[s_] = sm.t21[li * DLD + 4 * s_ + kq];
                        wn2[s_] = -U[(size_t)(j0 + 16 + li) * PLD + 16 + 4 * s_ + kq];
                    }
                    v4d x1[RMAXT], x2[RMAXT];
#pragma unroll
                    for (int u = 0; u < RMAXT; ++u) { x1[u] = (v4d){0, 0, 0, 0}; x2[u] = (v4d){0, 0, 0, 0}; }
#pragma unroll
                    for (int s_ = 0; s_ < 4; ++s_)
#pragma unroll
                        for (int u = 0; u < RMAXT; ++u)
                            x1[u] = __builtin_amdgcn_mfma_f64_16x16x4f64(wn1[s_], acc[u][0][s_], x1[u], 0, 0, 0);
#pragma unroll
                    for (int s_ = 0; s_ < 4; ++s_)
#pragma unroll
                        for (int u = 0; u < RMAXT; ++u)
                            acc[u][1] = __builtin_amdgcn_mfma_f64_16x16x4f64(l21[s_], x1[u][s_], acc[u][1], 0, 0, 0);
#pragma unroll
                    for (int s_ = 0; s_ < 4; ++s_)
#pragma unroll
                        for (int u = 0; u < RMAXT; ++u)
                            x2[u] = __builtin_amdgcn_mfma_f64_16x16x4f64(wn2[s_], acc[u][1][s_], x2[u], 0, 0, 0);
#pragma unroll
                    for (int u = 0; u < RMAXT; ++u) {
                        if (act[u]) {
                            double2* d0 = const_cast<double2*>(tile2(T[u], 2 * jb)) + fo;
                            d0[0] = make_double2(x1[u][0], x1[u][1]);
                            d0[64] = make_double2(x1[u][2], x1[u][3]);
                            d0[128] = make_double2(x2[u][0], x2[u][1]);
                            d0[192] = make_double2(x2[u][2], x2[u][3]);
                        }
                    }
                    if (ps == npass - 1 && jb + 1 < nblk) {
                        int Tn[RMAXT];
                        bool an[RMAXT];
                        first_rows(jb + 1, wv, ntr, Tn, an);
// ... 49 lines not shown
                continue;
            }
            const int cap = RM * (nsq > 6 * RM ? (nsq + 6 * RM - 1) / (6 * RM) : 1);
            int l0 = (tA + 2 < ntr) ? kLa1Load * nk2 + 48 : 0;
            int l1 = (tA + 4 < ntr) ? kLa2Load * nk2 + 96 : 0, l2 = 0, l3 = 0;
            int c2 = 0, c3 = 0, c4 = 0, c5 = 0, c6 = 0, c7 = 0;
            for (int r = 0; r < nsq; ++r) {
                const int w2 = c2 <= c6 ? 2 : 6, n2 = c2 <= c6 ? c2 : c6;
                const int w3 = c3 <= c7 ? 3 : 7, n3 = c3 <= c7 ? c3 : c7;
                int best = -1, bl = 0x7fffffff;
                if (c4 < cap && l0 < bl) { best = 4; bl = l0; }
                if (n2 < cap && l2 < bl) { best = w2; bl = l2; }
                if (n3 < cap && l3 < bl) { best = w3; bl = l3; }
                if (c5 < cap && l1 < bl) { best = 5; bl = l1; }
                sm.sched[J * SROW + r] = (unsigned char)best;
                if (best == 4) { ++c4; l0 += c; }
                else if (best == 5) { ++c5; l1 += c; }
                else if (best == 2) { ++c2; l2 += c; }
                else if (best == 6) { ++c6; l2 += c; }
                else if (best == 3) { ++c3; l3 += c; }
                else { ++c7; l3 += c; }
            }
        }
    }

    __device__ __forceinline__ void load_l21(double (&l21)[4], int which, int lane) const {
#pragma unroll
        for (int s_ = 0; s_ < 4; ++s_) l21[s_] = sm.t21[which * 256 + s_ * 64 + lane];
    }
    __device__ __forceinline__ void load_wn(double (&wn1)[4], double (&wn2)[4], int j0, int li, int kq) const {
        const double* U = sm.U;
#pragma unroll
        for (int s_ = 0; s_ < 4; ++s_) {
            wn1[s_] = -U[(size_t)(j0 + li) * PLD + 4 * s_ + kq];
            wn2[s_] = -U[(size_t)(j0 + 16 + li) * PLD + 16 + 4 * s_ + kq];
        }
    }
    __device__ __forceinline__ void wait_y(int word) const {
        int spins = 0;
        while (lds_peek32(&sm.flag[2]) < word) {
            __builtin_amdgcn_s_sleep(1);
            if (++spins > (1 << 22)) __builtin_trap();
        }
    }
    __device__ __forceinline__ void publish_a(int J_, int lane) {
        if (lane == 0) __hip_atomic_store(&sm.flag[1], J_ + 1, __ATOMIC_RELEASE, __HIP_MEMORY_SCOPE_WORKGROUP);
    }
    __device__ __forceinline__ void wait_a(int J_) const {
        int spins = 0;
        while (lds_peek32(&sm.flag[1]) < J_ + 1) {
            __builtin_amdgcn_s_sleep(1);
            if (++spins > (1 << 22)) __builtin_trap();
        }
    }
    __device__ __forceinline__ void arrive_b(int lane) {
        if (lane == 0) __hip_atomic_fetch_add(&sm.flag[3], 1, __ATOMIC_RELEASE, __HIP_MEMORY_SCOPE_WORKGROUP);
    }
    __device__ __forceinline__ void wait_b(int J_) const {
        int spins = 0;
        while (lds_peek32(&sm.flag[3]) < NARR * (J_ + 1)) {
            __builtin_amdgcn_s_sleep(1);
            if (++spins > (1 << 22)) __builtin_trap();
        }
    }
    struct BFrag { v2d f[2][2][2]; };
    __device__ __forceinline__ void load_bfrag(BFrag& b_, int tA, bool v3, int fo) const {
#pragma unroll
        for (int r = 0; r < 2; ++r)
#pragma unroll
            for (int k = 0; k < 2; ++k) {
                const double2* p = tile2((r == 1 && !v3) ? tA + 2 : tA + 2 + r, tA + k) + fo;
                const double2 d0 = p[0], d1 = p[64];
                b_.f[r][k][0] = (v2d){d0.x, d0.y};
                b_.f[r][k][1] = (v2d){d1.x, d1.y};
            }
    }
    static __device__ __forceinline__ void upd_b_step(v4d& acc, const BFrag& b_, int r, const v4d& xa, const v4d& xb, int st) {
        const int k = st >> 2, h = (st >> 1) & 1;
        const double bo = (st & 1) ? b_.f[r][k][h].y : b_.f[r][k][h].x;
        const double xo = k ? xb[st & 3] : xa[st & 3];
        acc = __builtin_amdgcn_mfma_f64_16x16x4f64(bo, xo, acc, 0, 0, 0);
    }
    __device__ __forceinline__ void store_pair(int T, int c, const v4d& x1, const v4d& x2, int fo) const {
        double2* d0 = const_cast<double2*>(tile2(T, c)) + fo;
        d0[0] = make_double2(x1[0], x1[1]);   d0[64] = make_double2(x1[2], x1[3]);
        d0[128] = make_double2(x2[0], x2[1]); d0[192] = make_double2(x2[2], x2[3]);
    }
    __device__ __forceinline__ void finish_block(const v4d& x21, int j0, int lane, int li, int kq) {
        double* U = sm.U;
        v4d y = (v4d){0, 0, 0, 0};
#pragma unroll
        for (int s_ = 0; s_ < 4; ++s_)
            y = __builtin_amdgcn_mfma_f64_16x16x4f64(x21[s_], U[(size_t)(j0 + 4 * s_ + kq) * PLD + li], y, 0, 0, 0);
        v4d w21 = (v4d){0, 0, 0, 0};
#pragma unroll
        for (int s_ = 0; s_ < 4; ++s_)
            w21 = __builtin_amdgcn_mfma_f64_16x16x4f64(-U[(size_t)(j0 + 16 + li) * PLD + 16 + 4 * s_ + kq], y[s_], w21, 0, 0, 0);
#pragma unroll
        for (int rg = 0; rg < 4; ++rg) U[(size_t)(j0 + 16 + kq + 4 * rg) * PLD + li] = w21[rg];
        __builtin_amdgcn_wave_barrier();
        const int r = lane & 31;
        const double* Mr = U + (size_t)(j0 + r) * PLD;
        double s0 = 0.0, s1 = 0.0, s2 = 0.0, s3 = 0.0;
#pragma unroll
        for (int c = 0; c < NB; c += 4) {
            s0 += Mr[c] * sm.vec[j0 + c];
            s1 += Mr[c + 1] * sm.vec[j0 + c + 1];
            s2 += Mr[c + 2] * sm.vec[j0 + c + 2];
            s3 += Mr[c + 3] * sm.vec[j0 + c + 3];
        }
        const double yv = (s0 + s1) + (s2 + s3);
        __builtin_amdgcn_wave_barrier();
        if (lane < NB) sm.vec[j0 + lane] = yv;
        __builtin_amdgcn_wave_barrier();
    }

    __device__ __forceinline__ bool factor64() {
        const int tid = opaque_u32(threadIdx.x), lane = tid & 63, wv = __builtin_amdgcn_readfirstlane(tid >> 6);
        const int ntr = (n + 15) >> 4;
        if (wv == 1) {
            const int li = lane & 15, kq = lane >> 4, fo = li * 4 + kq;
            v4d* const img21 = reinterpret_cast<v4d*>(sm.img);
            const v4d d11 = init_tile(0, 0, ntr, fo, li, kq);
            const v4d d21 = init_tile(1, 0, ntr, fo, li, kq);
            const v4d d22 = init_tile(1, 1, ntr, fo, li, kq);
            stage_dsc(d11);
            img21[lane] = d21;
            img21[64 + lane] = d22;
            if (lane == 0) { sm.flag[1] = 0; sm.flag[2] = 0; sm.flag[3] = 0; TL_START(); }
        }
        __syncthreads();
        const bool ok = wv == 0 ? f64_chain() : (wv == 1 ? f64_look2() : f64_rows(wv));
        __syncthreads();
        return ok;
    }

    __device__ __forceinline__ bool f64_chain() {
        const int lane = fresh_lane(), li = lane & 15, kq = lane >> 4;
        const int fo = li * 4 + kq;
        const int nblk = (n + NB - 1) / NB, nsup = (nblk + 1) >> 1;
        const int ntr = (n + 15) >> 4;
        double* U = sm.U;
// ... 28 lines not shown
                e22 = __builtin_amdgcn_mfma_f64_16x16x4f64(A3, A3, e22, 0, 0, 0);                   \
            }
            auto multf = [&](const Frag& f_) {
                HIPDRT_STEP7(f_.b0.x, f_.b1.x, f_.a2.x, f_.a3.x)
                HIPDRT_STEP7(f_.b0.y, f_.b1.y, f_.a2.y, f_.a3.y)
                __builtin_amdgcn_sched_barrier(0);
            };
#undef HIPDRT_STEP7
            asm volatile("s_waitcnt vmcnt(0)" ::: "memory");
            __builtin_amdgcn_sched_barrier(0);
            Frag f0, f1, f2, f3;
            loadf(f0, k_lo); loadf(f1, k_lo + 1); loadf(f2, k_lo + 2);
            int k2 = k_lo;
            for (; k2 < k_hi; k2 += 4) {
                if (poll && lds_peek32(&sm.flag[3]) >= arrived) break;
                loadf(f3, k2 + 3); vm_wait<12>(); multf(f0);
                loadf(f0, k2 + 4); vm_wait<12>(); multf(f1);
                loadf(f1, k2 + 5); vm_wait<12>(); multf(f2);
                loadf(f2, k2 + 6); vm_wait<12>(); multf(f3);
            }
            vm_wait<0>();
            return k2;
        };
        for (int J = 0; J < nsup; ++J) {
            const int j0a = J * 64, j0b = j0a + NB, tA = 4 * J;
            const bool hasb = (2 * J + 1) < nblk;
            const int R2 = tA + 2, R3 = tA + 3;
            const bool v3 = R3 < ntr;
            PROF_DECL
#ifdef HIPDRT_QP_PROFILE
            const unsigned long long _jt0 = __builtin_amdgcn_s_memtime();
#endif
            TL(0, J, 0);
            bool ok = cholinv16_dsc(j0a, 0);
            PROF(12);
            {
                const v4d d21 = img21[lane];
                v4d d22 = img22[lane];
                v4d x21 = (v4d){0, 0, 0, 0};
#pragma unroll
                for (int s_ = 0; s_ < 4; ++s_)
                    x21 = __builtin_amdgcn_mfma_f64_16x16x4f64(-U[(size_t)(j0a + li) * PLD + 4 * s_ + kq], d21[s_], x21, 0, 0, 0);
#pragma unroll
                for (int rg = 0; rg < 4; ++rg) sm.t21[rg * 64 + lane] = x21[rg];
#pragma unroll
                for (int s_ = 0; s_ < 4; ++s_)
                    d22 = __builtin_amdgcn_mfma_f64_16x16x4f64(x21[s_], x21[s_], d22, 0, 0, 0);
                PROF(14);
                ok = cholinv16(d22, j0a + 16, 16) && ok;
                PROF(15);
                TL(0, J, 4);
            }
            v4d x20 = (v4d){0, 0, 0, 0}, x30 = x20, x21_ = x20, x31 = x20;
            if (hasb) {
                if (!la_ready) {
                    p20 = init_tile(R2, tA, ntr, fo, li, kq);      p21 = init_tile(R2, tA + 1, ntr, fo, li, kq);
                    p30 = init_tile(R3, tA, ntr, fo, li, kq);      p31 = init_tile(R3, tA + 1, ntr, fo, li, kq);
                    e11 = init_tile(R2, R2, ntr, fo, li, kq);      e21 = init_tile(R3, R2, ntr, fo, li, kq);
                    e22 = init_tile(R3, R3, ntr, fo, li, kq);
                    la_done = 0;
                }
                if (J > 0) {
                    if (la_done < 8 * J) la1_ring(J, la_done, 8 * J, false, 0);
                    if (!v3) {
                        p30 = (v4d){0, 0, 0, 0}; p31 = (v4d){0, 0, 0, 0}; e21 = (v4d){0, 0, 0, 0};
                        e22 = init_tile(R3, R3, ntr, fo, li, kq);
                    }
                }
                PROF(40);
                TL(0, J, 5);
                double wn1[4], l21[4], wn2[4];
                load_wn(wn1, wn2, j0a, li, kq);
                load_l21(l21, 0, lane);
#pragma unroll
                for (int s_ = 0; s_ < 4; ++s_) {
                    x20 = __builtin_amdgcn_mfma_f64_16x16x4f64(wn1[s_], p20[s_], x20, 0, 0, 0);
                    x30 = __builtin_amdgcn_mfma_f64_16x16x4f64(wn1[s_], p30[s_], x30, 0, 0, 0);
                }
#pragma unroll
                for (int s_ = 0; s_ < 4; ++s_) {
                    p21 = __builtin_amdgcn_mfma_f64_16x16x4f64(l21[s_], x20[s_], p21, 0, 0, 0);
                    p31 = __builtin_amdgcn_mfma_f64_16x16x4f64(l21[s_], x30[s_], p31, 0, 0, 0);
                }
#pragma unroll
                for (int s_ = 0; s_ < 4; ++s_) {
                    x21_ = __builtin_amdgcn_mfma_f64_16x16x4f64(wn2[s_], p21[s_], x21_, 0, 0, 0);
                    x31 = __builtin_amdgcn_mfma_f64_16x16x4f64(wn2[s_], p31[s_], x31, 0, 0, 0);
                }
                store_pair(R2, tA, x20, x21_, fo);
                if (v3) store_pair(R3, tA, x30, x31, fo);
#pragma unroll
                for (int s_ = 0; s_ < 4; ++s_) {
                    e11 = __builtin_amdgcn_mfma_f64_16x16x4f64(x20[s_], x20[s_], e11, 0, 0, 0);
                    e21 = __builtin_amdgcn_mfma_f64_16x16x4f64(x20[s_], x30[s_], e21, 0, 0, 0);
                    e22 = __builtin_amdgcn_mfma_f64_16x16x4f64(x30[s_], x30[s_], e22, 0, 0, 0);
                }
#pragma unroll
                for (int s_ = 0; s_ < 4; ++s_) {
                    e11 = __builtin_amdgcn_mfma_f64_16x16x4f64(x21_[s_], x21_[s_], e11, 0, 0, 0);
                    e21 = __builtin_amdgcn_mfma_f64_16x16x4f64(x21_[s_], x31[s_], e21, 0, 0, 0);
                    e22 = __builtin_amdgcn_mfma_f64_16x16x4f64(x31[s_], x31[s_], e22, 0, 0, 0);
                }
                PROF(41);
                TL(0, J, 6);
                ok = cholinv16(e11, j0b, 0) && ok;
                v4d xb = (v4d){0, 0, 0, 0};
#pragma unroll
                for (int s_ = 0; s_ < 4; ++s_)
                    xb = __builtin_amdgcn_mfma_f64_16x16x4f64(-U[(size_t)(j0b + li) * PLD + 4 * s_ + kq], e21[s_], xb, 0, 0, 0);
#pragma unroll
                for (int rg = 0; rg < 4; ++rg) sm.t21[256 + rg * 64 + lane] = xb[rg];
#pragma unroll
                for (int s_ = 0; s_ < 4; ++s_)
                    e22 = __builtin_amdgcn_mfma_f64_16x16x4f64(xb[s_], xb[s_], e22, 0, 0, 0);
                ok = cholinv16(e22, j0b + 16, 16) && ok;
                PROF(42);
            }
            if (lane == 0) sm.flag[0] = ok ? 0 : 1;
            TL(0, J, 1);
            if constexpr (kFat) {
                publish_a(J, lane);
                if (!ok) return false;
            } else {
                __syncthreads();
            }
            TL(0, J, 2);
            PROF(1);
#ifdef HIPDRT_QP_PROFILE
            const unsigned long long _ta = __builtin_amdgcn_s_memtime();
            unsigned long long _tarr = _ta;
#define HIPDRT_PROF_ARRIVED() do { _tarr = __builtin_amdgcn_s_memtime(); } while (0)
#else
#define HIPDRT_PROF_ARRIVED()
#endif
            if (sm.flag[0]) return false;
            {
                double l21[4];
                load_l21(l21, 0, lane);
                finish_block((v4d){l21[0], l21[1], l21[2], l21[3]}, j0a, lane, li, kq);
                if (lane == 0) sm.flag[2] = 2 * J + 1;
                if (hasb) {
                    fwd_update(x20, x21_, R2, j0a, li, kq);
                    if (v3) fwd_update(x30, x31, R3, j0a, li, kq);
                    __builtin_amdgcn_wave_barrier();
                    load_l21(l21, 1, lane);
                    finish_block((v4d){l21[0], l21[1], l21[2], l21[3]}, j0b, lane, li, kq);
                    if (lane == 0) sm.flag[2] = 2 * J + 2;
                }
// ... 479 lines not shown
    struct UrgentBuf { v2d t[2][4]; };

    __device__ __forceinline__ void fwd_tile(const v2d (&t)[4], const double (&ya)[4], const double (&yb)[4], int T, int l4, int g4) {
        double pv = 0.0;
#pragma unroll
        for (int q = 0; q < 4; ++q) pv += t[q].x * ya[q] + t[q].y * yb[q];
        pv = quad_sum(pv);
        if (l4 == 0) {
            const int row = T * 16 + g4;
            if (row < n) sm.vec[row] -= pv;
        }
    }
    __device__ __forceinline__ void bwd_chunk(const v2d (&t)[4], double x0, double x1, int c, int lane, int l4) {
        const double s0 = t[0].x * x0 + t[2].x * x1;
        const double s1 = t[0].y * x0 + t[2].y * x1;
        const double s2 = t[1].x * x0 + t[3].x * x1;
        const double s3 = t[1].y * x0 + t[3].y * x1;
        const double f = colsum4(s0, s1, s2, s3, lane);
        if ((lane & 12) == 0) sm.vec[c * 16 + l4 + 4 * (lane >> 4)] -= f;
    }

    __device__ __forceinline__ void forward() {
        const int tid = opaque_u32(threadIdx.x), lane = tid & 63, wv = __builtin_amdgcn_readfirstlane(tid >> 6);
        const int nblk = (n + NB - 1) / NB;
        const int ntr = (n + 15) >> 4;
        double* vec = sm.vec;
        const double* U = sm.U;
        PROF_DECL
        if (wv == 0) {
            const int r = lane & 31;
            double mr[NB];
            if (GU) {
#pragma unroll
                for (int c = 0; c < NB; ++c) mr[c] = U[(size_t)r * PLD + c];
            }
            const int l4 = lane & 3, g4 = lane >> 2;
            auto ucount = [&](int jb) {
                const int k = jb < nblk ? ntr - (2 * jb + 2) : 0;
                return k < 0 ? 0 : (k < 2 ? k : 2);
            };
            auto upre = [&](UrgentBuf& B_, int jb) {
                const int nv = ucount(jb);
#pragma unroll
                for (int u = 0; u < 2; ++u) {
                    if (u < nv) {
                        const double2* p = tile2(2 * jb + 2 + u, 2 * jb) + lane;
                        B_.t[u][0] = gload16v<0>(p); B_.t[u][1] = gload16v<1024>(p);
                        B_.t[u][2] = gload16v<2048>(p); B_.t[u][3] = gload16v<3072>(p);
                    }
                }
            };
            auto urgent = [&](UrgentBuf& B_, int jb) {
                const int j0 = jb * NB, nv = ucount(jb);
                vm_wait_tiles(ucount(jb + 1));
                if (nv > 0) {
                    double ya[4], yb[4];
#pragma unroll
                    for (int q = 0; q < 4; ++q) { ya[q] = vec[j0 + 8 * q + l4]; yb[q] = vec[j0 + 8 * q + l4 + 4]; }
#pragma unroll
                    for (int u = 0; u < 2; ++u)
                        if (u < nv) fwd_tile(B_.t[u], ya, yb, 2 * jb + 2 + u, l4, g4);
                }
                upre(B_, jb + 2);
            };
            UrgentBuf ua, ub;
            upre(ua, 0);
            upre(ub, 1);
            auto dstep = [&](int jb) {
                const int j0 = jb * NB;
                const double* Mr = U + (size_t)(j0 + r) * PLD;
                PROF(6);
                double s0 = 0.0, s1 = 0.0, s2 = 0.0, s3 = 0.0;
#pragma unroll
                for (int c = 0; c < NB; c += 4) {
                    s0 += (GU ? mr[c] : Mr[c]) * vec[j0 + c];
                    s1 += (GU ? mr[c + 1] : Mr[c + 1]) * vec[j0 + c + 1];
                    s2 += (GU ? mr[c + 2] : Mr[c + 2]) * vec[j0 + c + 2];
                    s3 += (GU ? mr[c + 3] : Mr[c + 3]) * vec[j0 + c + 3];
                }
                const double y = (s0 + s1) + (s2 + s3);
                __builtin_amdgcn_wave_barrier();
                if (lane < NB) vec[j0 + lane] = y;
                lds_barrier();
                PROF(5);
                if (GU && jb + 1 < nblk) {
#pragma unroll
                    for (int c = 0; c < NB; ++c) mr[c] = Mr[(size_t)NB * PLD + c];
                }
            };
            for (int jb = 0; jb < nblk; jb += 2) {
                dstep(jb);
                urgent(ua, jb);
                if (jb + 1 < nblk) { dstep(jb + 1); urgent(ub, jb + 1); }
            }
            vm_wait<0>();
            lds_barrier();
        } else {
            const int l4 = lane & 3, g4 = lane >> 2, tw_ = wv - 1;
            const unsigned voff = (unsigned)lane * 16u;
            auto fcount = [&](int jb) {
                const int tbelow = jb < nblk ? ntr - (2 * jb + 4) : 0;
                const int k = tbelow - tw_ > 0 ? (tbelow - tw_ + SW_TW - 1) / SW_TW : 0;
                return k < SW_FT ? k : SW_FT;
            };
            auto fpre1 = [&](SweepBuf& B_, int jb, int nv, int u) {
                if (u < nv) {
                    const char* p = uniform_ptr(tile2(2 * jb + 4 + tw_ + u * SW_TW, 2 * jb));
#pragma unroll
                    for (int q = 0; q < 4; ++q) B_.t[u][q] = gload16(p + q * 1024, voff);
                }
            };
            auto fpre = [&](SweepBuf& B_, int jb) {
                const int nv = fcount(jb);
#pragma unroll
                for (int u = 0; u < SW_FT; ++u) fpre1(B_, jb, nv, u);
            };
            auto fstep = [&](SweepBuf& B_, int jb) {
                const int j0 = jb * NB, tb = 2 * jb, tbelow = ntr - (tb + 4);
                PROFW(44);
                lds_barrier();
// ... 31 lines not shown
                                const int tt = tt0 + j * SW_TW;
                                if (tt < tbelow) fwd_tile(t_[j], ya, yb, tb + 4 + tt, l4, g4);
                            }
                        }
                    }
                }
            };
            {
                SweepBuf fa, fb;
                fpre(fa, 0);
                fpre(fb, 1);
                for (int jb = 0; jb < nblk; jb += 2) {
                    fstep(fa, jb);
                    if (jb + 1 < nblk) fstep(fb, jb + 1);
                }
                vm_wait<0>();
                lds_barrier();
            }
        }
    }

    __device__ __forceinline__ void backward() {
        const int tid = opaque_u32(threadIdx.x), lane = tid & 63, wv = __builtin_amdgcn_readfirstlane(tid >> 6);
        const int nblk = (n + NB - 1) / NB;
        const int ntr = (n + 15) >> 4;
        double* vec = sm.vec;
        const double* U = sm.U;
        PROF_DECL
        if (wv == 0) {
            const int r = lane & 31;
            double mc[NB];
            if (GU) {
#pragma unroll
                for (int q = 0; q < NB; ++q) mc[q] = U[((size_t)(nblk - 1) * NB + q) * PLD + r];
            }
            const int l4 = lane & 3, g4 = lane >> 2;
            auto ucount = [&](int jb) { return jb > 0 ? 2 : 0; };
            auto upre = [&](UrgentBuf& B_, int jb) {
                if (jb > 0) {
                    const int tb = 2 * jb;
                    const bool two = (tb + 1) < ntr;
#pragma unroll
                    for (int u = 0; u < 2; ++u) {
                        const int c = 2 * jb - 2 + u;
                        const double2* p0 = tile2(tb, c) + lane;
                        const double2* p1 = tile2(two ? tb + 1 : tb, c) + lane;
                        B_.t[u][0] = gload16v<0>(p0); B_.t[u][1] = gload16v<1024>(p0);
                        B_.t[u][2] = gload16v<0>(p1); B_.t[u][3] = gload16v<1024>(p1);
                    }
                }
            };
            auto urgent = [&](UrgentBuf& B_, int jb) {
                const int j0 = jb * NB, tb = 2 * jb;
                const bool two = (tb + 1) < ntr;
                vm_wait_tiles(ucount(jb - 1));
                if (jb > 0) {
                    const double x0 = vec[j0 + g4];
                    const double x1 = two ? vec[j0 + 16 + g4] : 0.0;
#pragma unroll
                    for (int u = 0; u < 2; ++u) bwd_chunk(B_.t[u], x0, x1, 2 * jb - 2 + u, lane, l4);
                }
                upre(B_, jb - 2);
            };
            UrgentBuf ua, ub;
            upre(ua, nblk - 1);
            upre(ub, nblk - 2);
            auto dstep = [&](int jb) {
                const int j0 = jb * NB;
                const double* Mc = U + (size_t)j0 * PLD + r;
                PROF(8);
                double s0 = 0.0, s1 = 0.0, s2 = 0.0, s3 = 0.0;
#pragma unroll
                for (int q = 0; q < NB; q += 4) {
                    s0 += (GU ? mc[q] : Mc[(size_t)q * PLD]) * vec[j0 + q];
                    s1 += (GU ? mc[q + 1] : Mc[(size_t)(q + 1) * PLD]) * vec[j0 + q + 1];
                    s2 += (GU ? mc[q + 2] : Mc[(size_t)(q + 2) * PLD]) * vec[j0 + q + 2];
                    s3 += (GU ? mc[q + 3] : Mc[(size_t)(q + 3) * PLD]) * vec[j0 + q + 3];
                }
                const double xv = (s0 + s1) + (s2 + s3);
                __builtin_amdgcn_wave_barrier();
                if (lane < NB) vec[j0 + lane] = xv;
                lds_barrier();
                PROF(7);
                if (GU && jb > 0) {
#pragma unroll
                    for (int q = 0; q < NB; ++q) mc[q] = U[((size_t)(j0 - NB) + q) * PLD + r];
                }
            };
            for (int jb = nblk - 1; jb >= 0; jb -= 2) {
                dstep(jb);
                urgent(ua, jb);
                if (jb - 1 >= 0) { dstep(jb - 1); urgent(ub, jb - 1); }
            }
            vm_wait<0>();
            lds_barrier();
        } else {
            const int l4 = lane & 3, g4 = lane >> 2, tw_ = wv - 1;
            const unsigned voff = (unsigned)lane * 16u;
            auto bcount = [&](int jb) {
                const int nc = jb > 0 ? 2 * jb - 2 : 0;
                const int k = nc - tw_ > 0 ? (nc - tw_ + SW_TW - 1) / SW_TW : 0;
                return k < SW_BC ? k : SW_BC;
            };
            auto bpre1 = [&](SweepBuf& B_, int jb, int nv, int u) {
                if (u < nv) {
                    const int tb = 2 * jb, c = tw_ + u * SW_TW;
                    const bool two = (tb + 1) < ntr;
                    const char* p0 = uniform_ptr(tile2(tb, c));
                    const char* p1 = uniform_ptr(tile2(two ? tb + 1 : tb, c));
                    B_.t[u][0] = gload16(p0, voff); B_.t[u][1] = gload16(p0 + 1024, voff);
                    B_.t[u][2] = gload16(p1, voff); B_.t[u][3] = gload16(p1 + 1024, voff);
                }
            };
            auto bpre = [&](SweepBuf& B_, int jb) {
                const int nv = bcount(jb);
#pragma unroll
                for (int u = 0; u < SW_BC; ++u) bpre1(B_, jb, nv, u);
            };
            auto bstep = [&](SweepBuf& B_, int jb) {
// ... 126 lines not shown
#pragma unroll
            for (int w = 0; w < RNWV; ++w) s_ += sm.U[(size_t)w * NPd + i];
            sm.dvec[i] = s_;
        }
        __syncthreads();
        for (int i = tid; i < RNWV * NPd; i += RT) sm.U[i] = 0.0;
    }
};

struct CovArgs {
    int B, n;
    const double* Ppk; long long ppk_stride; int nchp;
    const double* Bex; int nex;
    double* L; long long l_stride;
    double* out; long long out_stride;
    int* status;
};

template <bool GU>
__device__ __forceinline__ double* resident_u_ptr(double* Lb, int NP) { return Lb + (size_t)NP * NP; }

template <bool GU, int RTT = 512>
__global__ __launch_bounds__(RTT) void cov_kernel_resident(CovArgs a, int NP) {
    constexpr int RT = RTT, RNW = RTT / 64;
    const int b = blockIdx.x;
    extern __shared__ double smem[];
    OpsResidentT<GU, RTT> ops;
    ops.L = a.L + (size_t)b * a.l_stride; ops.nch = NP / 16; ops.n = a.n;
    ops.Ppk = a.Ppk + (size_t)b * a.ppk_stride; ops.nchp = a.nchp;
    ops.nex = a.nex; ops.Bex = a.Bex;
    constexpr int VEC = ResSmemT<GU, RTT>::VEC;
    ops.sm.carve(smem);
    if (GU) ops.sm.U = ops.L + (size_t)(NP / 16 + a.nex) * (NP / 16) * TSZ;
    for (int i = threadIdx.x; i < NP * PLD; i += RT) ops.sm.U[i] = 0.0;
    for (int i = threadIdx.x; i < VEC; i += RT) { ops.sm.vec[i] = 0.0; ops.sm.dvec[i] = 0.0; }
    __syncthreads();
    const bool ok = ops.factor();
    double* out = a.out + (size_t)b * a.out_stride;
    if (threadIdx.x == 0) a.status[b] = ok ? 0 : -1;
    const int lane = threadIdx.x & 63, wv = threadIdx.x >> 6, l4 = lane & 3, g4 = lane >> 2;
    const int nblk = (a.n + NB - 1) / NB;
    for (int e = wv; e < a.nex; e += RNW) {
        double s_ = 0.0;
        if (ok) {
            for (int c = 0; c < 2 * nblk; ++c) {
                const double2* t = ops.tile2(ops.nch + e, c) + lane;
                const double2 d0 = t[0], d1 = t[64];
                s_ += d0.x * d0.x + d0.y * d0.y + d1.x * d1.x + d1.y * d1.y;
            }
            s_ = quad_sum(s_);
        } else {
            s_ = __builtin_nan("");
        }
        if (l4 == 0) out[e * 16 + g4] = s_;
    }
}

template <bool GU, int RTT = 512, int WPS = 2, int VT = 1>
__global__ __launch_bounds__(RTT, WPS) void qp_kernel_resident(QpArgs a, int NP) {
    constexpr int RT = RTT;
    const int b = a.order ? a.order[blockIdx.x] : blockIdx.x;
    if (a.active && !a.active[b]) return;
    extern __shared__ double smem[];
    OpsResidentT<GU, RTT, true, VT> ops;
    ops.L = a.L + (size_t)b * a.l_stride; ops.nch = NP / 16; ops.n = a.n;
    ops.Ppk = a.Ppk ? a.Ppk + (size_t)b * a.ppk_stride : nullptr; ops.nchp = a.nchp;
    ops.sm.carve(smem);
    if (GU) ops.sm.U = resident_u_ptr<GU>(ops.L, NP);
    ops.build_schedule64();
    for (int i = threadIdx.x; i < NP * PLD; i += RT) ops.sm.U[i] = 0.0;
    for (int i = threadIdx.x; i < NP + 32; i += RT) ops.sm.vec[i] = 0.0;
    __syncthreads();
    IpmSmem is{ops.sm.vec, ops.sm.dvec, ops.sm.red};
    constexpr int VTH = RT * VT;
    ipm_solve<RT, GU ? (2048 + VTH - 1) / VTH : (RNP_MAX + VTH - 1) / VTH, decltype(ops), VT>(a, b, ops, is);
}

template <bool GU, int RTT = 512, int VT = 1>
static size_t qp_resident_lds_bytes(int NP) {
    return ((GU ? 0 : (size_t)NP * PLD) + ResSmemT<GU, RTT, true, VT>::FIXED) * sizeof(double);
}
template <bool GU>
static size_t cov_lds_bytes(int NP) {
    return ((GU ? 0 : (size_t)NP * PLD) + ResSmemT<GU, 512, false>::FIXED) * sizeof(double);
}
static size_t resident_gu_doubles(int n) {
    const size_t NP = (size_t)round_up(n, 32);
    return NP * NP + NP * PLD;
}

static size_t resident_l_doubles(int n) {
    const size_t nt = (size_t)round_up(n, 32) / 16;
    return nt * nt * TSZ;
}

}
```

### include/hipdrt_debug.h

```cpp
#ifndef HIPDRT_DEBUG_H
#define HIPDRT_DEBUG_H

#include "hipdrt.h"

#ifdef __cplusplus
extern "C" {
#endif

int hipdrt_qp_profile(hipdrt_ctx* ctx, unsigned long long* cycles, int n, int reset);
int hipdrt_debug_qp_occupancy(hipdrt_ctx* ctx, int threads, int n);
int hipdrt_debug_qp_group(hipdrt_ctx* ctx, int members);
int hipdrt_debug_qp_waves(hipdrt_ctx* ctx, int waves);
int hipdrt_debug_exact_zero_shortcuts(hipdrt_ctx* ctx, int on);
int hipdrt_debug_stream_pool(hipdrt_ctx* ctx, int cap, void** streams, int* holders, int* running, int* size);

typedef struct hipdrt_debug_gram_args {
    int B, m, n;
    const double* A;
    int a_batched, lda;
    const double* w;
    const double* y;
    const double* l1;
    double l1_scalar;
    const double* l2;
    int l2_batched, ldl2;
    const double* mk[3];
    int ldm;
    const double* s;
    const double* rho;
    double dfac[3];
    int ns, sym, toep, toep_maxd, spec_zero;
    int dop_start, dop_size;
    const double* dop_rho;
    double dop_dfac[3];
    const int* active;
    double* P;
    int ldp;
    double* Ppk;
    double* q;
} hipdrt_debug_gram_args;
int hipdrt_debug_gram_l2(hipdrt_ctx* ctx, const hipdrt_debug_gram_args* a);
int hipdrt_debug_pack_p(hipdrt_ctx* ctx, int B, int n, const double* P, int ldp, double* Ppk);

typedef struct hipdrt_debug_hyper_args {
    int B, m, n, ns, ldrm, ldm;
// ... 92 lines not shown
```

Measured before the change: 2752.

## Pack LDS-resident U factor blocks without upper-right zeros and move IPM vectors into LDS

Introduces a ULayout abstraction so that the LDS-resident Cholesky factor U stores each 32x32 block without its upper-right 16x16 zero quadrant, shrinking LDS per block. The freed LDS holds several IPM state vectors (d, di, lm, rx, rz, zz, sv, ws3), which were previously in global state memory. The triangular solves, cholinv16 and the zeroing loops are rewritten to use the new indexing. The change also adds a debug toggle to force U into global memory and some profiling spans. The aim is lower LDS footprint and fewer global-memory accesses in the QP solver, at the cost of more complex indexing.

Measured after the change: 2774, median of 6. Within noise of the previous version (+0.8%).

```diff
diff --git a/hybrid-drt_amd/_ffi.py b/hybrid-drt_amd/_ffi.py
--- a/hybrid-drt_amd/_ffi.py
+++ b/hybrid-drt_amd/_ffi.py
@@ -204,6 +204,8 @@
     "hipdrt_debug_qp_group": [_vp, C.c_int],
     "hipdrt_debug_exact_zero_shortcuts": [_vp, C.c_int],
     "hipdrt_debug_qp_waves": [_vp, C.c_int],
+    "hipdrt_debug_qp_u_outside": [_vp, C.c_int],
+    "hipdrt_debug_qp_u_layout": [_vp, C.c_int, C.c_int, _ip, C.POINTER(C.c_longlong), C.POINTER(C.c_longlong)],
     "hipdrt_debug_stream_pool": [_vp, C.c_int, C.POINTER(C.c_void_p), _ip, _ip, _ip],
     "hipdrt_debug_gram_l2": [_vp, C.POINTER(DebugGramArgs)],
     "hipdrt_debug_pack_p": [_vp, C.c_int, C.c_int, _dp, C.c_int, _dp],
@@ -701,6 +703,9 @@
     def debug_qp_waves(self, waves):
         _check(self._lib.hipdrt_debug_qp_waves(self._h, int(waves)))
 
+    def debug_qp_u_outside(self, on):
+        _check(self._lib.hipdrt_debug_qp_u_outside(self._h, int(bool(on))))
+
     def debug_stream_pool(self):
         size = C.c_int(0)
         _check(self._lib.hipdrt_debug_stream_pool(self._h, 0, None, None, None, C.byref(size)))
diff --git a/hybrid-drt_amd/csrc/common.hpp b/hybrid-drt_amd/csrc/common.hpp
--- a/hybrid-drt_amd/csrc/common.hpp
+++ b/hybrid-drt_amd/csrc/common.hpp
@@ -86,6 +86,7 @@
     int qp_force_group = -1;
     int zero_shortcuts = 1;
     int qp_waves = -1;
+    int qp_u_outside = 0;
     int cand_form = -1;
     float predict_ms[2] = {0.f, 0.f};
 };
@@ -434,6 +435,7 @@
     int* gsync = nullptr;
     int redo_aborted = 0;
     int waves = 0;
+    int u_outside = 0;
 };
 int launch_qp(hipStream_t st, const QpArgs& a);
 int qp_group_size(int B, int n, int force = -1);
@@ -446,11 +448,12 @@
                       double* tiles, int nchp);
 void launch_lpt_order(hipStream_t st, int B, const int* iters, const int* active, int* order);
 size_t qp_scratch_ld(int n);
-size_t qp_scratch_doubles(int n, int G = 0);
+size_t qp_scratch_doubles(int n, int G = 0, int u_outside = 0);
 inline int qp_state_ld(int n) { return round_up(n, 32) + 32; }
 inline size_t qp_state_doubles(int n) { return (size_t)17 * qp_state_ld(n); }
 int qp_profile_read(unsigned long long* out, int n, int reset);
 int hyper_profile_read(unsigned long long* out, int n, int reset);
 int qp_occupancy(int threads, int n);
+void qp_u_layout(int n, int u_outside, int* offsets, long long* vec_offsets, long long* info);
 
 }
diff --git a/hybrid-drt_amd/csrc/debug.hip b/hybrid-drt_amd/csrc/debug.hip
--- a/hybrid-drt_amd/csrc/debug.hip
+++ b/hybrid-drt_amd/csrc/debug.hip
@@ -65,6 +65,20 @@
     HIPDRT_REQUIRE(ctx, "NULL pointer");
     HIPDRT_REQUIRE(waves == -1 || waves == 4 || waves == 8, "waves: 4, 8 or -1");
     ctx->qp_waves = waves;
+    return HIPDRT_OK;
+} HIPDRT_CATCH
+
+int hipdrt_debug_qp_u_outside(hipdrt_ctx* ctx, int on) try {
+    HIPDRT_REQUIRE(ctx, "NULL pointer");
+    ctx->qp_u_outside = on ? 1 : 0;
+    return HIPDRT_OK;
+} HIPDRT_CATCH
+
+int hipdrt_debug_qp_u_layout(hipdrt_ctx* ctx, int n, int u_outside, int* offsets, long long* vec_offsets, long long* info) try {
+    (void)ctx;
+    HIPDRT_REQUIRE(offsets && vec_offsets && info, "NULL pointer");
+    HIPDRT_REQUIRE(n >= 1 && n <= 2048, "1 <= n <= 2048");
+    qp_u_layout(n, u_outside, offsets, vec_offsets, info);
     return HIPDRT_OK;
 } HIPDRT_CATCH
 
diff --git a/hybrid-drt_amd/csrc/operators.hip b/hybrid-drt_amd/csrc/operators.hip
--- a/hybrid-drt_amd/csrc/operators.hip
+++ b/hybrid-drt_amd/csrc/operators.hip
@@ -327,7 +327,7 @@
                                   (size_t)n * sizeof(double), nmat * n, hipMemcpyHostToDevice, st));
     TRY(upload(dq, q, (size_t)B * n * sizeof(double), st));
     TRY(upload(dh, h, (size_t)(h_batched ? B : 1) * n * sizeof(double), st));
-    HIPDRT_CHECK(dL.alloc((size_t)B * qp_scratch_doubles(n, G) * sizeof(double)));
+    HIPDRT_CHECK(dL.alloc((size_t)B * qp_scratch_doubles(n, G, ctx->qp_u_outside) * sizeof(double)));
     HIPDRT_CHECK(dx.alloc((size_t)B * n * sizeof(double)));
     HIPDRT_CHECK(dit.alloc((size_t)B * sizeof(int)));
     HIPDRT_CHECK(dpc.alloc((size_t)B * sizeof(double)));
@@ -335,11 +335,12 @@
     QpArgs a{};
     a.B = B; a.n = n; a.P = dP.d(); a.p_stride = p_batched ? (long long)n * ldp : 0; a.ldp = ldp;
     a.q = dq.d(); a.h = dh.d(); a.h_stride = h_batched ? n : 0;
-    a.L = dL.d(); a.ldl = ldl; a.l_stride = (long long)qp_scratch_doubles(n, G);
+    a.L = dL.d(); a.ldl = ldl; a.l_stride = (long long)qp_scratch_doubles(n, G, ctx->qp_u_outside);
     a.x = dx.d(); a.iters = dit.i(); a.pcost = dpc.d(); a.status = dst.i();
     a.active = nullptr; a.iters_accum = nullptr;
     a.G = G;
     a.waves = ctx->qp_waves;
+    a.u_outside = ctx->qp_u_outside;
     if (G >= 1) {
         HIPDRT_CHECK(dgs.alloc((size_t)B * qp_gsync_ints() * sizeof(int)));
         a.gsync = dgs.i();
diff --git a/hybrid-drt_amd/csrc/plan.hip b/hybrid-drt_amd/csrc/plan.hip
--- a/hybrid-drt_amd/csrc/plan.hip
+++ b/hybrid-drt_amd/csrc/plan.hip
@@ -3,7 +3,7 @@
 
 #include "plan.hpp"
 
-struct SpecDims { size_t n, m, nf; int qp_G; };
+struct SpecDims { size_t n, m, nf; int qp_G, qp_gu; };
 struct PerSpectrumBuf {
     DevBuf hipdrt_plan::*buf;
     size_t (*bytes)(const SpecDims&);
@@ -30,7 +30,7 @@
     {&hipdrt_plan::qp_iters_total, [](const SpecDims&) { return sizeof(int); }},
     {&hipdrt_plan::qp_status, [](const SpecDims&) { return sizeof(int); }},
     {&hipdrt_plan::qp_iters, [](const SpecDims&) { return sizeof(int); }},
-    {&hipdrt_plan::L, [](const SpecDims& d) { return qp_scratch_doubles((int)d.n, d.qp_G) * sizeof(double); }},
+    {&hipdrt_plan::L, [](const SpecDims& d) { return qp_scratch_doubles((int)d.n, d.qp_G, d.qp_gu) * sizeof(double); }},
     {&hipdrt_plan::qpstate, [](const SpecDims& d) { return (d.qp_G > 1 ? d.qp_G : 1) * qp_state_doubles((int)d.n) * sizeof(double); }},
     {&hipdrt_plan::gsync, [](const SpecDims&) { return qp_gsync_ints() * sizeof(int); }},
     {&hipdrt_plan::Ppk, [](const SpecDims& d) { return qp_ppk_doubles((int)d.n) * sizeof(double); }},
@@ -39,7 +39,7 @@
 };
 
 static SpecDims spec_dims(const hipdrt_plan* p) {
-    return {(size_t)p->n, (size_t)p->m, (size_t)(p->nf > 0 ? p->nf : 1), p->qp_G};
+    return {(size_t)p->n, (size_t)p->m, (size_t)(p->nf > 0 ? p->nf : 1), p->qp_G, p->qp_gu};
 }
 
 namespace hipdrt {
@@ -126,6 +126,7 @@
     const size_t cap = (size_t)p->capacity;
     const int n = p->n, m = p->m;
     p->qp_G = qp_group_size(p->capacity, n, p->ctx->qp_force_group);
+    p->qp_gu = p->ctx->qp_u_outside;
     HIPDRT_REQUIRE(p->qp_G >= 0, "n too large for the QP kernels");
     const SpecDims d = spec_dims(p);
     for (const PerSpectrumBuf& e : kPerSpectrum)
diff --git a/hybrid-drt_amd/csrc/plan.hpp b/hybrid-drt_amd/csrc/plan.hpp
--- a/hybrid-drt_amd/csrc/plan.hpp
+++ b/hybrid-drt_amd/csrc/plan.hpp
@@ -90,6 +90,7 @@
     int toep_maxd = -1;
     int spec_zero = 0;
     int qp_G = 0;
+    int qp_gu = 0;
 };
 
 struct hipdrt_plan : PlanShape {
@@ -121,13 +122,14 @@
         int G = qp_group_size(B, n, ctx ? ctx->qp_force_group : -1);
         const size_t have_l = L.bytes / sizeof(double), have_s = qpstate.bytes / sizeof(double);
         if (G >= 1 && G != qp_G) {
-            const bool fits = gsync.p && (size_t)B * qp_scratch_doubles(n, G) <= have_l &&
+            const bool fits = gsync.p && (size_t)B * qp_scratch_doubles(n, G, qp_gu) <= have_l &&
                               (size_t)B * G * qp_state_doubles(n) <= have_s && (size_t)B * qp_gsync_ints() * sizeof(int) <= gsync.bytes;
             if (!fits) G = qp_G;
         } else if (G < 1) {
             G = qp_G;
         }
-        qa.G = G; qa.gsync = gsync.i(); qa.l_stride = (long long)qp_scratch_doubles(n, G);
+        qa.G = G; qa.gsync = gsync.i(); qa.l_stride = (long long)qp_scratch_doubles(n, G, qp_gu);
+        qa.u_outside = qp_gu;
         qa.waves = ctx ? ctx->qp_waves : -1;
     }
     int hist_b = -1, hist_cap = 0;
diff --git a/hybrid-drt_amd/csrc/qp.hip b/hybrid-drt_amd/csrc/qp.hip
--- a/hybrid-drt_amd/csrc/qp.hip
+++ b/hybrid-drt_amd/csrc/qp.hip
@@ -11,9 +11,9 @@
 
 size_t qp_scratch_ld(int n) { return (size_t)round_up(n, 16); }
 
-size_t qp_scratch_doubles(int n, int G) {
+size_t qp_scratch_doubles(int n, int G, int u_outside) {
     if (G >= 1) return group_scratch_doubles(n, G);
-    return n <= RNP_MAX ? resident_l_doubles(n) : resident_gu_doubles(n);
+    return n <= RNP_MAX && !u_outside ? resident_l_doubles(n) : resident_gu_doubles(n);
 }
 size_t qp_gsync_ints() { return GRP_WORDS; }
 
@@ -112,7 +112,7 @@
 static int launch_qp_resident(hipStream_t st, const QpArgs& a) {
     const int NP = round_up(a.n, 32);
     if (!a.Ppk) { set_error("qp resident: packed copy of P missing"); return HIPDRT_E_INVALID; }
-    const bool gu = a.n > RNP_MAX;
+    const bool gu = a.n > RNP_MAX || a.u_outside;
     if (!gu && a.waves == 4)
         return launch_lds(qp_kernel_resident<false, 256, 1, 2>, "qp fat", dim3(a.B), dim3(256), qp_resident_lds_bytes<false, 256, 2>(NP),
                           st, a, NP);
@@ -133,7 +133,7 @@
 
 size_t dist_var_scratch_doubles(int n, int nex) {
     const size_t nch = (size_t)round_up(n, 32) / 16;
-    return (nch + (size_t)nex) * nch * TSZ + (n > RNP_MAX ? (size_t)round_up(n, 32) * PLD : 0);
+    return (nch + (size_t)nex) * nch * TSZ + (n > RNP_MAX ? ULayout<true>::size(round_up(n, 32)) : 0);
 }
 
 int qp_occupancy(int threads, int n) {
@@ -148,6 +148,36 @@
         e = hipOccupancyMaxActiveBlocksPerMultiprocessor(&nb, qp_kernel_resident<false, 512>, 512, qp_resident_lds_bytes<false>(NP));
     }
     return e == hipSuccess ? nb : -1;
+}
+
+template <bool GU>
+static void u_layout_offsets(int NP, int* offsets) {
+    using UL = ULayout<GU>;
+    for (int jb = 0; jb < NP / NB; ++jb)
+        for (int r = 0; r < NB; ++r)
+            for (int c = 0; c < NB; ++c) {
+                const int j0 = jb * NB;
+                long long o = -1;
+                if (r < 16 && c < 16) o = (long long)UL::m11(j0, r, c);
+                else if (r >= 16 && c < 16) o = (long long)UL::m21(j0, r - 16, c);
+                else if (r >= 16) o = (long long)UL::m22(j0, r - 16, c - 16);
+                else if (GU) o = (long long)UL::row(j0, r) + c;
+                if ((o >= 0) != UL::stored(r, c) || (o >= 0 && o != (long long)UL::at(j0, r, c))) o = -2;
+                offsets[(jb * NB + r) * NB + c] = (int)o;
+            }
+}
+void qp_u_layout(int n, int u_outside, int* offsets, long long* vec_offsets, long long* info) {
+    const int NP = round_up(n, 32);
+    const bool gu = n > RNP_MAX || u_outside;
+    using S8 = ResSmemT<false, 512, true>;
+    using S4 = ResSmemT<false, 256, true, 2>;
+    if (gu) u_layout_offsets<true>(NP, offsets); else u_layout_offsets<false>(NP, offsets);
+    for (int k = 0; k < 8; ++k) vec_offsets[k] = gu ? -1 : (long long)(ULayout<false>::size(NP) + (size_t)k * NP);
+    info[0] = (long long)(gu ? ULayout<true>::size(NP) : ULayout<false>::size(NP));
+    info[1] = gu ? -1 : (long long)S8::FIXED;
+    info[2] = (long long)(gu ? qp_resident_lds_bytes<true>(NP) : qp_resident_lds_bytes<false>(NP));
+    info[3] = gu ? 0 : (long long)qp_resident_lds_bytes<false, 256, 2>(NP);
+    static_assert(S8::FIXED == S4::FIXED && S8::NLV == 8 && S4::NLV == 8, "both LDS forms carve U and the vectors at the same place");
 }
 
 static int launch_qp_group(hipStream_t st, const QpArgs& a, int G) {
diff --git a/hybrid-drt_amd/csrc/qp_common.hpp b/hybrid-drt_amd/csrc/qp_common.hpp
--- a/hybrid-drt_amd/csrc/qp_common.hpp
+++ b/hybrid-drt_amd/csrc/qp_common.hpp
@@ -24,8 +24,12 @@
     atomicAdd(&g_qp_prof[slot], _n - _pt); atomicAdd(&g_qp_prof[slot2], _n - _pt); _pt = _n; } else { _pt = 0; } } while (0)
 #define PROFW(slot) do { if ((threadIdx.x & 63) == 0 && blockIdx.x == 0) { unsigned long long _n = __builtin_amdgcn_s_memtime(); \
     atomicAdd(&g_qp_prof[slot], _n - _pt); _pt = _n; } else { _pt = 0; } } while (0)
+#define PROF_SPAN_BEGIN const unsigned long long _sp0 = __builtin_amdgcn_s_memtime();
+#define PROF_SPAN_END(slot) do { if (threadIdx.x == 0 && blockIdx.x == 0) atomicAdd(&g_qp_prof[slot], __builtin_amdgcn_s_memtime() - _sp0); } while (0)
 #else
 static constexpr int QP_PROF_SLOTS = 48;
+#define PROF_SPAN_BEGIN
+#define PROF_SPAN_END(slot)
 #define PROF_DECL
 #define PROF(slot)
 #define PROF2(slot, slot2)
@@ -36,6 +40,35 @@
 
 static constexpr int NB = 32;
 static constexpr int PLD = 33;
+
+template <bool GU>
+struct ULayout {
+    static constexpr int LD1 = GU ? PLD : 17;
+    static constexpr int LD2 = PLD;
+    static constexpr int LOW = 16 * LD1;
+    static constexpr int BLK = 16 * LD1 + 16 * LD2;
+    __host__ __device__ static constexpr size_t base(int j0) { return GU ? (size_t)j0 * PLD : (size_t)((j0 >> 5) * BLK); }
+    __host__ __device__ static constexpr size_t m11(int j0, int i, int j) {
+        return GU ? (size_t)(j0 + i) * PLD + j : (size_t)((j0 >> 5) * BLK + i * LD1 + j);
+    }
+    __host__ __device__ static constexpr size_t m21(int j0, int i, int j) {
+        return GU ? (size_t)(j0 + 16 + i) * PLD + j : (size_t)((j0 >> 5) * BLK + LOW + i * LD2 + j);
+    }
+    __host__ __device__ static constexpr size_t m22(int j0, int i, int j) {
+        return GU ? (size_t)(j0 + 16 + i) * PLD + 16 + j : (size_t)((j0 >> 5) * BLK + LOW + i * LD2 + 16 + j);
+    }
+    __host__ __device__ static constexpr size_t row(int j0, int r) {
+        return GU ? (size_t)(j0 + r) * PLD : (size_t)((j0 >> 5) * BLK + (r < 16 ? r * LD1 : LOW + (r - 16) * LD2));
+    }
+    __host__ __device__ static constexpr int cols(int r) { return (GU || r >= 16) ? NB : 16; }
+    __host__ __device__ static constexpr size_t zrow(int j0, int r) { return (GU || r >= 16) ? row(j0, r) + 16 : base(j0) + 1; }
+    __host__ __device__ static constexpr int zcol(int r) { return (GU || r < 16) ? r : 16; }
+    __host__ __device__ static constexpr bool stored(int r, int c) { return c < cols(r); }
+    __host__ __device__ static constexpr size_t at(int j0, int r, int c) { return row(j0, r) + c; }
+    __host__ __device__ static constexpr size_t size(int NP) { return (size_t)(NP >> 5) * BLK; }
+};
+static_assert(ULayout<true>::BLK == NB * PLD && ULayout<true>::m22(64, 3, 5) == (64 + 16 + 3) * PLD + 16 + 5, "");
+static_assert(ULayout<false>::BLK == 800 && ULayout<false>::m21(32, 0, 0) == 800 + 272 && ULayout<false>::row(0, 31) + 32 == 799, "");
 
 __device__ __forceinline__ unsigned opaque_u32(unsigned v) {
     asm volatile("" : "+v"(v));
@@ -156,6 +189,7 @@
     template <int N>
     __device__ __forceinline__ void sum(double (&v)[VT][N]) {
         static_assert(N <= 4, "");
+        PROF_SPAN_BEGIN
         double* s = buf + (slot & (SLOTS - 1)) * NWV * 4;
         ++slot;
 #pragma unroll
@@ -176,10 +210,12 @@
             for (int w = 0; w < NWV; ++w) t += s[w * 4 + i];
             v[0][i] = t;
         }
+        PROF_SPAN_END(47);
     }
     template <int N>
     __device__ __forceinline__ void max(double (&v)[VT][N]) {
         static_assert(N <= 4, "");
+        PROF_SPAN_BEGIN
         double* s = buf + (slot & (SLOTS - 1)) * NWV * 4;
         ++slot;
 #pragma unroll
@@ -200,6 +236,7 @@
             for (int w = 1; w < NWV; ++w) t = fmax(t, s[w * 4 + i]);
             v[0][i] = t;
         }
+        PROF_SPAN_END(47);
     }
 };
 
@@ -208,6 +245,8 @@
     double* vec;
     double* dvec;
     double* red;
+    double* lvec = nullptr;
+    int lld = 0;
 };
 
 template <int THREADS, int EPT, class Ops, int VT = 1>
@@ -233,10 +272,12 @@
     double* const S_ = a.state + (size_t)(slot >= 0 ? slot : b) * a.state_stride;
     const int sld = a.state_ld;
 #define SV(k) (S_ + (size_t)(k) * sld)
-    double* const x = SV(0); double* const z = SV(1); double* const s = SV(2); double* const d = SV(3);
-    double* const di = SV(4); double* const lm = SV(5); double* const qv = SV(6); double* const hv = SV(7);
-    double* const rx = SV(8); double* const rz = SV(9); double* const dx = SV(10); double* const ds = SV(11);
-    double* const dz = SV(12); double* const ws3 = SV(13); double* const zz = SV(14); double* const sv = SV(15);
+    constexpr bool kLV = Ops::kLdsState;
+#define LSV(l, k) (kLV ? sm.lvec + (size_t)(l) * sm.lld : SV(k))
+    double* const x = SV(0); double* const z = SV(1); double* const s = SV(2); double* const d = LSV(4, 3);
+    double* const di = LSV(0, 4); double* const lm = LSV(1, 5); double* const qv = SV(6); double* const hv = SV(7);
+    double* const rx = LSV(2, 8); double* const rz = LSV(3, 9); double* const dx = SV(10); double* const ds = SV(11);
+    double* const dz = SV(12); double* const ws3 = LSV(7, 13); double* const zz = LSV(5, 14); double* const sv = LSV(6, 15);
     double* const px = SV(16);
 #define FOR_E _Pragma("unroll") for (unsigned v_ = 0; v_ < (unsigned)VT; ++v_) \
         _Pragma("unroll EUNR") for (unsigned e_ = 0, i = opaque_u32(tid) + v_ * THREADS; e_ < (unsigned)EPT; ++e_, i += THREADS * VT)
@@ -265,8 +306,10 @@
                 FOR_E if (VALID) sm.vec[i] = x[i];
                 __syncthreads();
                 { PROF_DECL
+                PROF_SPAN_BEGIN
                 ops.matvec();
                 __syncthreads();
+                PROF_SPAN_END(0);
                 PROF(9); }
                 if (kRecurPx) {
                     FOR_E if (VALID) px[i] = sm.dvec[i];
@@ -340,19 +383,25 @@
         FOR_E if (VALID) sm.dvec[i] = di[i] * di[i];
         set_rhs(0);
         __syncthreads();
+        { PROF_SPAN_BEGIN
         if (!ops.factor()) {
             status = (start || iters == 0) ? HIPDRT_QP_SINGULAR : HIPDRT_QP_SINGULAR_LATE;
             break;
         }
+        PROF_SPAN_END(0); }
 
 #pragma nounroll
         for (int pc = 0; pc < nsolve; ++pc) {
             if (pc == 0) {
+                PROF_SPAN_BEGIN
                 ops.backward();
+                PROF_SPAN_END(0);
             } else {
                 set_rhs(pc);
                 __syncthreads();
+                PROF_SPAN_BEGIN
                 ops.solve();
+                PROF_SPAN_END(0);
             }
             if (start) {
                 double st[VT][2] = {}, mx[VT][2];
@@ -481,6 +530,7 @@
     }
 #undef FOR_E
 #undef VALID
+#undef LSV
 #undef SV
 }
 
diff --git a/hybrid-drt_amd/csrc/qp_group.hpp b/hybrid-drt_amd/csrc/qp_group.hpp
--- a/hybrid-drt_amd/csrc/qp_group.hpp
+++ b/hybrid-drt_amd/csrc/qp_group.hpp
@@ -396,14 +396,14 @@
             asm volatile("" ::: "memory");
             PROF(2);
             TS(1);
-            bool ok = cholinv16_dsc(j0, 0);
+            bool ok = cholinv16_dsc<0>(j0);
             TS(2);
             const v4d d21 = img21[lane];
             v4d d22 = img22[lane];
             v4d x21 = (v4d){0, 0, 0, 0};
 #pragma unroll
             for (int s_ = 0; s_ < 4; ++s_)
-                x21 = __builtin_amdgcn_mfma_f64_16x16x4f64(-U[(size_t)(j0 + li) * PLD + 4 * s_ + kq], d21[s_], x21, 0, 0, 0);
+                x21 = __builtin_amdgcn_mfma_f64_16x16x4f64(-U[UL::m11(j0, li, 4 * s_ + kq)], d21[s_], x21, 0, 0, 0);
 #pragma unroll
             for (int rg = 0; rg < 4; ++rg) sm.t21[li * DLD + kq + 4 * rg] = x21[rg];
             {
@@ -415,7 +415,7 @@
 #pragma unroll
             for (int s_ = 0; s_ < 4; ++s_)
                 d22 = __builtin_amdgcn_mfma_f64_16x16x4f64(sm.t21[li * DLD + 4 * s_ + kq], x21[s_], d22, 0, 0, 0);
-            ok = cholinv16(d22, j0 + 16, 16) && ok;
+            ok = cholinv16<1>(d22, j0) && ok;
             PROF(12);
             TS(5);
             if (lane == 0) sm.flag[0] = ok ? 0 : 1;
@@ -427,16 +427,16 @@
 #pragma unroll
             for (int s_ = 0; s_ < 4; ++s_)
                 y = __builtin_amdgcn_mfma_f64_16x16x4f64(sm.t21[li * DLD + 4 * s_ + kq],
-                                                         U[(size_t)(j0 + 4 * s_ + kq) * PLD + li], y, 0, 0, 0);
+                                                         U[UL::m11(j0, 4 * s_ + kq, li)], y, 0, 0, 0);
             v4d w21 = (v4d){0, 0, 0, 0};
 #pragma unroll
             for (int s_ = 0; s_ < 4; ++s_)
-                w21 = __builtin_amdgcn_mfma_f64_16x16x4f64(-U[(size_t)(j0 + 16 + li) * PLD + 16 + 4 * s_ + kq], y[s_], w21, 0, 0, 0);
-#pragma unroll
-            for (int rg = 0; rg < 4; ++rg) U[(size_t)(j0 + 16 + kq + 4 * rg) * PLD + li] = w21[rg];
+                w21 = __builtin_amdgcn_mfma_f64_16x16x4f64(-U[UL::m22(j0, li, 4 * s_ + kq)], y[s_], w21, 0, 0, 0);
+#pragma unroll
+            for (int rg = 0; rg < 4; ++rg) U[UL::m21(j0, kq + 4 * rg, li)] = w21[rg];
             __builtin_amdgcn_wave_barrier();
             const int r = lane & 31;
-            const double* Mr = U + (size_t)(j0 + r) * PLD;
+            const double* Mr = U + UL::row(j0, r);
             double s0 = 0.0, s1 = 0.0, s2 = 0.0, s3 = 0.0;
 #pragma unroll
             for (int c = 0; c < NB; c += 4) {
@@ -577,9 +577,9 @@
                 double wn1[4], l21[4], wn2[4];
 #pragma unroll
                 for (int s_ = 0; s_ < 4; ++s_) {
-                    wn1[s_] = -U[(size_t)(j0 + li) * PLD + 4 * s_ + kq];
+                    wn1[s_] = -U[UL::m11(j0, li, 4 * s_ + kq)];
                     l21[s_] = sm.t21[li * DLD + 4 * s_ + kq];
-                    wn2[s_] = -U[(size_t)(j0 + 16 + li) * PLD + 16 + 4 * s_ + kq];
+                    wn2[s_] = -U[UL::m22(j0, li, 4 * s_ + kq)];
                 }
                 v4d x20 = (v4d){0, 0, 0, 0}, x30 = x20, x21_ = x20, x31 = x20;
 #pragma unroll
@@ -707,8 +707,8 @@
                     double wn1[4], l21[4], wn2[4];
 #pragma unroll
                     for (int s_ = 0; s_ < 4; ++s_) {
-                        wn1[s_] = -U[(size_t)(j0 + li) * PLD + 4 * s_ + kq];
-                        wn2[s_] = -U[(size_t)(j0 + 16 + li) * PLD + 16 + 4 * s_ + kq];
+                        wn1[s_] = -U[UL::m11(j0, li, 4 * s_ + kq)];
+                        wn2[s_] = -U[UL::m22(j0, li, 4 * s_ + kq)];
                     }
                     if (ps == 0) {
 #pragma unroll
@@ -767,7 +767,7 @@
 
 static size_t group_scratch_doubles(int n, int G) {
     const size_t NP = (size_t)round_up(n, 32);
-    return NP * NP + (size_t)G * NP * PLD + (NP / NB) * (size_t)GRP_LA_SLOT;
+    return NP * NP + (size_t)G * ULayout<true>::size((int)NP) + (NP / NB) * (size_t)GRP_LA_SLOT;
 }
 
 __global__ __launch_bounds__(512, 2) void qp_kernel_group(QpArgs a, int NP, int G) {
@@ -795,10 +795,10 @@
     ops.lacnt = reinterpret_cast<int*>(ops.latile + 7 * 256);
     ops.sm.vec = ops.latile + 7 * 256 + 8;
     ops.sm.dvec = ops.sm.vec + NP + 64;
-    ops.sm.U = ops.L + (size_t)NP * NP + (size_t)g * NP * PLD;
-    ops.labuf = ops.L + (size_t)NP * NP + (size_t)G * NP * PLD;
+    ops.sm.U = ops.L + (size_t)NP * NP + (size_t)g * ULayout<true>::size(NP);
+    ops.labuf = ops.L + (size_t)NP * NP + (size_t)G * ULayout<true>::size((int)NP);
     ops.build_owner();
-    for (int i = threadIdx.x; i < NP * PLD; i += RT) ops.sm.U[i] = 0.0;
+    for (int i = threadIdx.x; i < (int)ULayout<true>::size(NP); i += RT) ops.sm.U[i] = 0.0;
     for (int i = threadIdx.x; i < NP + 64; i += RT) { ops.sm.vec[i] = 0.0; ops.sm.dvec[i] = 0.0; }
     if (G > 1) {
         int& xcc_mask = ops.sm.flag[2];
diff --git a/hybrid-drt_amd/csrc/qp_resident.hpp b/hybrid-drt_amd/csrc/qp_resident.hpp
--- a/hybrid-drt_amd/csrc/qp_resident.hpp
+++ b/hybrid-drt_amd/csrc/qp_resident.hpp
@@ -17,6 +17,7 @@
 template <bool GU, int RTT = 512, bool P64 = false, int VT = 1>
 struct ResSmemT {
     double* U;
+    double* lvec;
     double* vec;
     double* dvec;
     double* red;
@@ -33,6 +34,10 @@
     static constexpr int RED = (P64 ? 2 : 4) * (RTT / 64) * VT * 4;
     static constexpr int T21 = P64 ? 2 * 256 : 16 * 17;
     static constexpr int FIXED = RED + T21 + 16 * 17 + 8 + 512 + SCHED + VEC + DVEC;
+    static constexpr int NLV = (!GU && P64) ? 8 : 0;
+    using UL = ULayout<GU>;
+    static constexpr size_t doubles(int NP) { return (size_t)FIXED + (GU ? 0 : UL::size(NP) + (size_t)NLV * NP); }
+    __device__ __forceinline__ void carve_lvec(int NP) { lvec = NLV ? U + UL::size(NP) : nullptr; }
     __device__ __forceinline__ void carve(double* smem) {
         red = smem;
         t21 = red + RED;
@@ -43,10 +48,12 @@
         vec = img + 512 + SCHED;
         dvec = vec + VEC;
         U = dvec + DVEC;
+        lvec = nullptr;
     }
 };
-static_assert((ResSmemT<false, 512, true>::FIXED + 544 * 33) * 8 <= 160 * 1024, "n = 514 must fit one CU's LDS");
-static_assert((ResSmemT<false, 256, true, 2>::FIXED + 544 * 33) * 8 <= 160 * 1024, "n = 514 must fit one CU's LDS (fat form)");
+static_assert(ResSmemT<false, 512, true>::doubles(544) * 8 <= 160 * 1024, "n = 514 must fit one CU's LDS");
+static_assert(ResSmemT<false, 256, true, 2>::doubles(544) * 8 <= 160 * 1024, "n = 514 must fit one CU's LDS (fat form)");
+static_assert(ResSmemT<false, 512, true>::doubles(544) == ResSmemT<false, 512, true>::FIXED + 544 * 33, "U's zero quarters hold exactly the eight vectors");
 static_assert((ResSmemT<false, 512, true>::RED + ResSmemT<false, 512, true>::T21 + 16 * 17 + 8) % 4 == 0, "img must be 32-byte aligned");
 
 template <bool GU, int RTT = 512, bool P64 = false, int VT = 1>
@@ -56,6 +63,8 @@
     using Smem = ResSmemT<GU, RTT, P64, VT>;
     static constexpr int kVT = VT;
     static constexpr int kRedSlots = P64 ? 2 : 4;
+    using UL = ULayout<GU>;
+    static constexpr bool kLdsState = Smem::NLV > 0;
     double* L; int nch; int n; Smem sm;
     const double* Ppk; int nchp;
     int nex = 0; const double* Bex = nullptr;
@@ -75,18 +84,21 @@
 #pragma unroll
         for (int rg = 0; rg < 4; ++rg) sm.dsc[li * DLD + kq + 4 * rg] = -at[rg];
     }
-    __device__ __forceinline__ bool cholinv16(const v4d& at, int r0, int c0) const {
+    template <int H>
+    __device__ __forceinline__ bool cholinv16(const v4d& at, int j0) const {
         stage_dsc(at);
         __builtin_amdgcn_wave_barrier();
-        return cholinv16_dsc(r0, c0);
-    }
-    __device__ __forceinline__ bool cholinv16_dsc(int r0, int c0) const { return cholinv16_blocked(r0, c0); }
+        return cholinv16_dsc<H>(j0);
+    }
+    template <int H>
+    __device__ __forceinline__ bool cholinv16_dsc(int j0) const { return cholinv16_blocked<H>(j0); }
     static __device__ __forceinline__ double rsq_pivot(double x) {
         const double y0 = __builtin_amdgcn_rsq(x);
         const double e = __builtin_fma(y0 * -x, y0, 1.0);
         return __builtin_fma(y0 * e, __builtin_fma(e, 0.375, 0.5), y0);
     }
-    __device__ __forceinline__ bool cholinv16_blocked(int r0, int c0) const {
+    template <int H>
+    __device__ __forceinline__ bool cholinv16_blocked(int j0) const {
         const int lane = fresh_lane(), li = lane & 15, kq = lane >> 4;
         const double* D = sm.dsc;
         v4d aA, aW;
@@ -126,7 +138,7 @@
             const v4d z4 = (v4d){0, 0, 0, 0};
             const v4d X = __builtin_amdgcn_mfma_f64_16x16x4f64(wsel, tA, z4, 0, 0, 0);
             const v4d Y = __builtin_amdgcn_mfma_f64_16x16x4f64(wsel, tW, z4, 0, 0, 0);
-            sm.U[(size_t)(r0 + 4 * k + kq) * PLD + c0 + li] = (li <= 4 * k + kq) ? Y[0] : 0.0;
+            sm.U[(H ? UL::m22(j0, 4 * k + kq, li) : UL::m11(j0, 4 * k + kq, li))] = (li <= 4 * k + kq) ? Y[0] : 0.0;
             if (k < 3) {
                 const double pan = (li > 4 * k + 3) ? -X[0] : 0.0;
                 aA = __builtin_amdgcn_mfma_f64_16x16x4f64(pan, X[0], aA, 0, 0, 0);
@@ -217,14 +229,14 @@
         for (int jb = 0; jb < nblk; ++jb) {
             const int j0 = jb * NB;
             PROF_DECL
-            bool ok = cholinv16_dsc(j0, 0);
+            bool ok = cholinv16_dsc<0>(j0);
             PROF(12);
             const v4d d21 = img21[lane];
             v4d d22 = img22[lane];
             v4d x21 = (v4d){0, 0, 0, 0};
 #pragma unroll
             for (int s_ = 0; s_ < 4; ++s_)
-                x21 = __builtin_amdgcn_mfma_f64_16x16x4f64(-U[(size_t)(j0 + li) * PLD + 4 * s_ + kq], d21[s_], x21, 0, 0, 0);
+                x21 = __builtin_amdgcn_mfma_f64_16x16x4f64(-U[UL::m11(j0, li, 4 * s_ + kq)], d21[s_], x21, 0, 0, 0);
 #pragma unroll
             for (int rg = 0; rg < 4; ++rg) sm.t21[li * DLD + kq + 4 * rg] = x21[rg];
             __builtin_amdgcn_wave_barrier();
@@ -232,7 +244,7 @@
             for (int s_ = 0; s_ < 4; ++s_)
                 d22 = __builtin_amdgcn_mfma_f64_16x16x4f64(sm.t21[li * DLD + 4 * s_ + kq], x21[s_], d22, 0, 0, 0);
             PROF(14);
-            ok = cholinv16(d22, j0 + 16, 16) && ok;
+            ok = cholinv16<1>(d22, j0) && ok;
             PROF(15);
             if (lane == 0) sm.flag[0] = ok ? 0 : 1;
             __syncthreads();
@@ -242,13 +254,13 @@
 #pragma unroll
             for (int s_ = 0; s_ < 4; ++s_)
                 y = __builtin_amdgcn_mfma_f64_16x16x4f64(sm.t21[li * DLD + 4 * s_ + kq],
-                                                         U[(size_t)(j0 + 4 * s_ + kq) * PLD + li], y, 0, 0, 0);
+                                                         U[UL::m11(j0, 4 * s_ + kq, li)], y, 0, 0, 0);
             v4d w21 = (v4d){0, 0, 0, 0};
 #pragma unroll
             for (int s_ = 0; s_ < 4; ++s_)
-                w21 = __builtin_amdgcn_mfma_f64_16x16x4f64(-U[(size_t)(j0 + 16 + li) * PLD + 16 + 4 * s_ + kq], y[s_], w21, 0, 0, 0);
-#pragma unroll
-            for (int rg = 0; rg < 4; ++rg) U[(size_t)(j0 + 16 + kq + 4 * rg) * PLD + li] = w21[rg];
+                w21 = __builtin_amdgcn_mfma_f64_16x16x4f64(-U[UL::m22(j0, li, 4 * s_ + kq)], y[s_], w21, 0, 0, 0);
+#pragma unroll
+            for (int rg = 0; rg < 4; ++rg) U[UL::m21(j0, kq + 4 * rg, li)] = w21[rg];
             PROF(3);
             __syncthreads();
             PROF(4);
@@ -338,9 +350,9 @@
                 double wn1[4], l21[4], wn2[4];
 #pragma unroll
                 for (int s_ = 0; s_ < 4; ++s_) {
-                    wn1[s_] = -U[(size_t)(j0 + li) * PLD + 4 * s_ + kq];
+                    wn1[s_] = -U[UL::m11(j0, li, 4 * s_ + kq)];
                     l21[s_] = sm.t21[li * DLD + 4 * s_ + kq];
-                    wn2[s_] = -U[(size_t)(j0 + 16 + li) * PLD + 16 + 4 * s_ + kq];
+                    wn2[s_] = -U[UL::m22(j0, li, 4 * s_ + kq)];
                 }
                 v4d x20 = (v4d){0, 0, 0, 0}, x30 = x20, x21_ = x20, x31 = x20;
 #pragma unroll
@@ -509,9 +521,9 @@
                     double wn1[4], l21[4], wn2[4];
 #pragma unroll
                     for (int s_ = 0; s_ < 4; ++s_) {
-                        wn1[s_] = -U[(size_t)(j0 + li) * PLD + 4 * s_ + kq];
+                        wn1[s_] = -U[UL::m11(j0, li, 4 * s_ + kq)];
                         l21[s_] = sm.t21[li * DLD + 4 * s_ + kq];
-                        wn2[s_] = -U[(size_t)(j0 + 16 + li) * PLD + 16 + 4 * s_ + kq];
+                        wn2[s_] = -U[UL::m22(j0, li, 4 * s_ + kq)];
                     }
                     v4d x1[RMAXT], x2[RMAXT];
 #pragma unroll
@@ -627,8 +639,8 @@
         const double* U = sm.U;
 #pragma unroll
         for (int s_ = 0; s_ < 4; ++s_) {
-            wn1[s_] = -U[(size_t)(j0 + li) * PLD + 4 * s_ + kq];
-            wn2[s_] = -U[(size_t)(j0 + 16 + li) * PLD + 16 + 4 * s_ + kq];
+            wn1[s_] = -U[UL::m11(j0, li, 4 * s_ + kq)];
+            wn2[s_] = -U[UL::m22(j0, li, 4 * s_ + kq)];
         }
     }
     __device__ __forceinline__ void wait_y(int word) const {
@@ -686,23 +698,31 @@
         v4d y = (v4d){0, 0, 0, 0};
 #pragma unroll
         for (int s_ = 0; s_ < 4; ++s_)
-            y = __builtin_amdgcn_mfma_f64_16x16x4f64(x21[s_], U[(size_t)(j0 + 4 * s_ + kq) * PLD + li], y, 0, 0, 0);
+            y = __builtin_amdgcn_mfma_f64_16x16x4f64(x21[s_], U[UL::m11(j0, 4 * s_ + kq, li)], y, 0, 0, 0);
         v4d w21 = (v4d){0, 0, 0, 0};
 #pragma unroll
         for (int s_ = 0; s_ < 4; ++s_)
-            w21 = __builtin_amdgcn_mfma_f64_16x16x4f64(-U[(size_t)(j0 + 16 + li) * PLD + 16 + 4 * s_ + kq], y[s_], w21, 0, 0, 0);
-#pragma unroll
-        for (int rg = 0; rg < 4; ++rg) U[(size_t)(j0 + 16 + kq + 4 * rg) * PLD + li] = w21[rg];
+            w21 = __builtin_amdgcn_mfma_f64_16x16x4f64(-U[UL::m22(j0, li, 4 * s_ + kq)], y[s_], w21, 0, 0, 0);
+#pragma unroll
+        for (int rg = 0; rg < 4; ++rg) U[UL::m21(j0, kq + 4 * rg, li)] = w21[rg];
         __builtin_amdgcn_wave_barrier();
         const int r = lane & 31;
-        const double* Mr = U + (size_t)(j0 + r) * PLD;
+        const double* Mr = U + UL::row(j0, r);
+        const double* Mz = U + UL::zrow(j0, r);
         double s0 = 0.0, s1 = 0.0, s2 = 0.0, s3 = 0.0;
 #pragma unroll
-        for (int c = 0; c < NB; c += 4) {
+        for (int c = 0; c < 16; c += 4) {
             s0 += Mr[c] * sm.vec[j0 + c];
             s1 += Mr[c + 1] * sm.vec[j0 + c + 1];
             s2 += Mr[c + 2] * sm.vec[j0 + c + 2];
             s3 += Mr[c + 3] * sm.vec[j0 + c + 3];
+        }
+#pragma unroll
+        for (int c = 16; c < NB; c += 4) {
+            s0 += Mz[c - 16] * sm.vec[j0 + c];
+            s1 += Mz[c - 16 + 1] * sm.vec[j0 + c + 1];
+            s2 += Mz[c - 16 + 2] * sm.vec[j0 + c + 2];
+            s3 += Mz[c - 16 + 3] * sm.vec[j0 + c + 3];
         }
         const double yv = (s0 + s1) + (s2 + s3);
         __builtin_amdgcn_wave_barrier();
@@ -797,7 +817,7 @@
             const unsigned long long _jt0 = __builtin_amdgcn_s_memtime();
 #endif
             TL(0, J, 0);
-            bool ok = cholinv16_dsc(j0a, 0);
+            bool ok = cholinv16_dsc<0>(j0a);
             PROF(12);
             {
                 const v4d d21 = img21[lane];
@@ -805,14 +825,14 @@
                 v4d x21 = (v4d){0, 0, 0, 0};
 #pragma unroll
                 for (int s_ = 0; s_ < 4; ++s_)
-                    x21 = __builtin_amdgcn_mfma_f64_16x16x4f64(-U[(size_t)(j0a + li) * PLD + 4 * s_ + kq], d21[s_], x21, 0, 0, 0);
+                    x21 = __builtin_amdgcn_mfma_f64_16x16x4f64(-U[UL::m11(j0a, li, 4 * s_ + kq)], d21[s_], x21, 0, 0, 0);
 #pragma unroll
                 for (int rg = 0; rg < 4; ++rg) sm.t21[rg * 64 + lane] = x21[rg];
 #pragma unroll
                 for (int s_ = 0; s_ < 4; ++s_)
                     d22 = __builtin_amdgcn_mfma_f64_16x16x4f64(x21[s_], x21[s_], d22, 0, 0, 0);
                 PROF(14);
-                ok = cholinv16(d22, j0a + 16, 16) && ok;
+                ok = cholinv16<1>(d22, j0a) && ok;
                 PROF(15);
                 TL(0, J, 4);
             }
@@ -868,17 +888,17 @@
                 }
                 PROF(41);
                 TL(0, J, 6);
-                ok = cholinv16(e11, j0b, 0) && ok;
+                ok = cholinv16<0>(e11, j0b) && ok;
                 v4d xb = (v4d){0, 0, 0, 0};
 #pragma unroll
                 for (int s_ = 0; s_ < 4; ++s_)
-                    xb = __builtin_amdgcn_mfma_f64_16x16x4f64(-U[(size_t)(j0b + li) * PLD + 4 * s_ + kq], e21[s_], xb, 0, 0, 0);
+                    xb = __builtin_amdgcn_mfma_f64_16x16x4f64(-U[UL::m11(j0b, li, 4 * s_ + kq)], e21[s_], xb, 0, 0, 0);
 #pragma unroll
                 for (int rg = 0; rg < 4; ++rg) sm.t21[256 + rg * 64 + lane] = xb[rg];
 #pragma unroll
                 for (int s_ = 0; s_ < 4; ++s_)
                     e22 = __builtin_amdgcn_mfma_f64_16x16x4f64(xb[s_], xb[s_], e22, 0, 0, 0);
-                ok = cholinv16(e22, j0b + 16, 16) && ok;
+                ok = cholinv16<1>(e22, j0b) && ok;
                 PROF(42);
             }
             if (lane == 0) sm.flag[0] = ok ? 0 : 1;
@@ -1424,7 +1444,7 @@
             double mr[NB];
             if (GU) {
 #pragma unroll
-                for (int c = 0; c < NB; ++c) mr[c] = U[(size_t)r * PLD + c];
+                for (int c = 0; c < NB; ++c) mr[c] = U[UL::row(0, r) + c];
             }
             const int l4 = lane & 3, g4 = lane >> 2;
             auto ucount = [&](int jb) {
@@ -1460,15 +1480,23 @@
             upre(ub, 1);
             auto dstep = [&](int jb) {
                 const int j0 = jb * NB;
-                const double* Mr = U + (size_t)(j0 + r) * PLD;
+                const double* Mr = U + UL::row(j0, r);
+                const double* Mz = U + UL::zrow(j0, r);
                 PROF(6);
                 double s0 = 0.0, s1 = 0.0, s2 = 0.0, s3 = 0.0;
 #pragma unroll
-                for (int c = 0; c < NB; c += 4) {
+                for (int c = 0; c < 16; c += 4) {
                     s0 += (GU ? mr[c] : Mr[c]) * vec[j0 + c];
                     s1 += (GU ? mr[c + 1] : Mr[c + 1]) * vec[j0 + c + 1];
                     s2 += (GU ? mr[c + 2] : Mr[c + 2]) * vec[j0 + c + 2];
                     s3 += (GU ? mr[c + 3] : Mr[c + 3]) * vec[j0 + c + 3];
+                }
+#pragma unroll
+                for (int c = 16; c < NB; c += 4) {
+                    s0 += (GU ? mr[c] : Mz[c - 16]) * vec[j0 + c];
+                    s1 += (GU ? mr[c + 1] : Mz[c - 16 + 1]) * vec[j0 + c + 1];
+                    s2 += (GU ? mr[c + 2] : Mz[c - 16 + 2]) * vec[j0 + c + 2];
+                    s3 += (GU ? mr[c + 3] : Mz[c - 16 + 3]) * vec[j0 + c + 3];
                 }
                 const double y = (s0 + s1) + (s2 + s3);
                 __builtin_amdgcn_wave_barrier();
@@ -1477,7 +1505,7 @@
                 PROF(5);
                 if (GU && jb + 1 < nblk) {
 #pragma unroll
-                    for (int c = 0; c < NB; ++c) mr[c] = Mr[(size_t)NB * PLD + c];
+                    for (int c = 0; c < NB; ++c) mr[c] = Mr[UL::BLK + c];
                 }
             };
             for (int jb = 0; jb < nblk; jb += 2) {
@@ -1575,7 +1603,7 @@
             double mc[NB];
             if (GU) {
 #pragma unroll
-                for (int q = 0; q < NB; ++q) mc[q] = U[((size_t)(nblk - 1) * NB + q) * PLD + r];
+                for (int q = 0; q < NB; ++q) mc[q] = U[UL::row((nblk - 1) * NB, q) + r];
             }
             const int l4 = lane & 3, g4 = lane >> 2;
             auto ucount = [&](int jb) { return jb > 0 ? 2 : 0; };
@@ -1610,15 +1638,23 @@
             upre(ub, nblk - 2);
             auto dstep = [&](int jb) {
                 const int j0 = jb * NB;
-                const double* Mc = U + (size_t)j0 * PLD + r;
+                const double* Mc = U + UL::row(j0, 0) + r;
+                const double* Mt = U + UL::row(j0, 0) + UL::zcol(r);
                 PROF(8);
                 double s0 = 0.0, s1 = 0.0, s2 = 0.0, s3 = 0.0;
 #pragma unroll
-                for (int q = 0; q < NB; q += 4) {
-                    s0 += (GU ? mc[q] : Mc[(size_t)q * PLD]) * vec[j0 + q];
-                    s1 += (GU ? mc[q + 1] : Mc[(size_t)(q + 1) * PLD]) * vec[j0 + q + 1];
-                    s2 += (GU ? mc[q + 2] : Mc[(size_t)(q + 2) * PLD]) * vec[j0 + q + 2];
-                    s3 += (GU ? mc[q + 3] : Mc[(size_t)(q + 3) * PLD]) * vec[j0 + q + 3];
+                for (int q = 0; q < 16; q += 4) {
+                    s0 += (GU ? mc[q] : Mt[UL::row(0, q)]) * vec[j0 + q];
+                    s1 += (GU ? mc[q + 1] : Mt[UL::row(0, q + 1)]) * vec[j0 + q + 1];
+                    s2 += (GU ? mc[q + 2] : Mt[UL::row(0, q + 2)]) * vec[j0 + q + 2];
+                    s3 += (GU ? mc[q + 3] : Mt[UL::row(0, q + 3)]) * vec[j0 + q + 3];
+                }
+#pragma unroll
+                for (int q = 16; q < NB; q += 4) {
+                    s0 += (GU ? mc[q] : Mc[UL::row(0, q)]) * vec[j0 + q];
+                    s1 += (GU ? mc[q + 1] : Mc[UL::row(0, q + 1)]) * vec[j0 + q + 1];
+                    s2 += (GU ? mc[q + 2] : Mc[UL::row(0, q + 2)]) * vec[j0 + q + 2];
+                    s3 += (GU ? mc[q + 3] : Mc[UL::row(0, q + 3)]) * vec[j0 + q + 3];
                 }
                 const double xv = (s0 + s1) + (s2 + s3);
                 __builtin_amdgcn_wave_barrier();
@@ -1627,7 +1663,7 @@
                 PROF(7);
                 if (GU && jb > 0) {
 #pragma unroll
-                    for (int q = 0; q < NB; ++q) mc[q] = U[((size_t)(j0 - NB) + q) * PLD + r];
+                    for (int q = 0; q < NB; ++q) mc[q] = U[UL::row(j0 - NB, q) + r];
                 }
             };
             for (int jb = nblk - 1; jb >= 0; jb -= 2) {
@@ -1820,7 +1856,7 @@
     constexpr int VEC = ResSmemT<GU, RTT>::VEC;
     ops.sm.carve(smem);
     if (GU) ops.sm.U = ops.L + (size_t)(NP / 16 + a.nex) * (NP / 16) * TSZ;
-    for (int i = threadIdx.x; i < NP * PLD; i += RT) ops.sm.U[i] = 0.0;
+    for (int i = threadIdx.x; i < (int)ULayout<GU>::size(NP); i += RT) ops.sm.U[i] = 0.0;
     for (int i = threadIdx.x; i < VEC; i += RT) { ops.sm.vec[i] = 0.0; ops.sm.dvec[i] = 0.0; }
     __syncthreads();
     const bool ok = ops.factor();
@@ -1856,25 +1892,26 @@
     ops.sm.carve(smem);
     if (GU) ops.sm.U = resident_u_ptr<GU>(ops.L, NP);
     ops.build_schedule64();
-    for (int i = threadIdx.x; i < NP * PLD; i += RT) ops.sm.U[i] = 0.0;
+    ops.sm.carve_lvec(NP);
+    for (int i = threadIdx.x; i < (int)ULayout<GU>::size(NP); i += RT) ops.sm.U[i] = 0.0;
     for (int i = threadIdx.x; i < NP + 32; i += RT) ops.sm.vec[i] = 0.0;
     __syncthreads();
-    IpmSmem is{ops.sm.vec, ops.sm.dvec, ops.sm.red};
+    IpmSmem is{ops.sm.vec, ops.sm.dvec, ops.sm.red, ops.sm.lvec, NP};
     constexpr int VTH = RT * VT;
     ipm_solve<RT, GU ? (2048 + VTH - 1) / VTH : (RNP_MAX + VTH - 1) / VTH, decltype(ops), VT>(a, b, ops, is);
 }
 
 template <bool GU, int RTT = 512, int VT = 1>
 static size_t qp_resident_lds_bytes(int NP) {
-    return ((GU ? 0 : (size_t)NP * PLD) + ResSmemT<GU, RTT, true, VT>::FIXED) * sizeof(double);
+    return ResSmemT<GU, RTT, true, VT>::doubles(NP) * sizeof(double);
 }
 template <bool GU>
 static size_t cov_lds_bytes(int NP) {
-    return ((GU ? 0 : (size_t)NP * PLD) + ResSmemT<GU, 512, false>::FIXED) * sizeof(double);
+    return ResSmemT<GU, 512, false>::doubles(NP) * sizeof(double);
 }
 static size_t resident_gu_doubles(int n) {
     const size_t NP = (size_t)round_up(n, 32);
-    return NP * NP + NP * PLD;
+    return NP * NP + ULayout<true>::size((int)NP);
 }
 
 static size_t resident_l_doubles(int n) {
diff --git a/include/hipdrt_debug.h b/include/hipdrt_debug.h
--- a/include/hipdrt_debug.h
+++ b/include/hipdrt_debug.h
@@ -11,6 +11,8 @@
 int hipdrt_debug_qp_occupancy(hipdrt_ctx* ctx, int threads, int n);
 int hipdrt_debug_qp_group(hipdrt_ctx* ctx, int members);
 int hipdrt_debug_qp_waves(hipdrt_ctx* ctx, int waves);
+int hipdrt_debug_qp_u_outside(hipdrt_ctx* ctx, int on);
+int hipdrt_debug_qp_u_layout(hipdrt_ctx* ctx, int n, int u_outside, int* offsets, long long* vec_offsets, long long* info);
 int hipdrt_debug_exact_zero_shortcuts(hipdrt_ctx* ctx, int on);
 int hipdrt_debug_stream_pool(hipdrt_ctx* ctx, int cap, void** streams, int* holders, int* running, int* size);
 
```
